# vpc-ccg/circminer

Hardware: AMD Instinct MI355X
Metric: paired reads/sec (whole node), hg38 k=20, 2x150 bp; circ_report bit-exact (higher is better)
Workload: dtype int32/u8 (chain scores f64)

## Files before the change

circminer_amd/_build.py:

```python
from __future__ import annotations

import os
import subprocess
import sys

HERE = os.path.dirname(os.path.abspath(__file__))
CSRC = os.path.join(HERE, "csrc")
INC = os.path.join(HERE, "..", "include")
OUT = os.path.join(CSRC, "libcmhot.so")
SOURCES = ["cm_hot.hip", "cm_dispatch.cpp", "host_index.cpp", "host_annot.cpp", "host_index_io.cpp", "host_fastq.cpp", "host_mapping.cpp", "host_circ.cpp",
           "host_circ_call.cpp"]
DEPS = SOURCES + sorted(f for f in os.listdir(CSRC) if f.endswith(".h")) + [os.path.join("..", "..", "include", "circminer_hot.h")]
KERNEL_EXPORTS = ['cm_create', 'cm_destroy', 'cm_last_error', 'cm_load_contig', 'cm_load_contig_raw', 'cm_build_contig', 'cm_index_download', 'cm_load_annotation', 'cm_unload_contig', 'cm_reads_upload', 'cm_reads_stage', 'cm_reads_swap', 'cm_map_rounds', 'cm_map_round', 'cm_sync', 'cm_reads_reset', 'cm_collect_active', 'cm_collect_records', 'cm_collect_records_device', 'cm_host_alloc', 'cm_host_free', 'cm_host_register', 'cm_host_unregister', 'cm_type_histogram', 'cm_reads_download', 'cm_map_batch', 'cm_seed_batch', 'cm_chain_batch', 'cm_debug_lane_clk', 'cm_debug_counters', 'cm_prof_enable', 'cm_prof_reset', 'cm_prof_get', 'cm_prof_counters', 'cm_ctx', 'cm_chain']
VARIANTS = (("k16", []), ("k24", ["-DCM_MAX_CHAIN_FRAGS=24"]))


def needs_build(out: str = OUT) -> bool:
    if not os.path.exists(out):
        return True
    t = os.path.getmtime(out)
    return any(os.path.getmtime(os.path.join(CSRC, d)) > t for d in DEPS)


def build(force: bool = False, verbose: bool = False, tag: str = "", flags=()) -> str:
    OUT = os.path.join(CSRC, f"libcmhot_{tag}.so") if tag else globals()["OUT"]
    if not force and not needs_build(OUT):
        return OUT
    hipcc = os.environ.get("HIPCC", "/opt/rocm/bin/hipcc")
    extra = os.environ.get("CM_EXTRA_FLAGS", "").split() + list(flags)
    sfx = ("_" + tag) if tag else ""
    objs = []
    jobs = []
    for s in SOURCES:
        base = [hipcc, "-c", "-O3", "-std=c++17", "-fPIC", "-ffp-contract=off", *extra, "-I", INC, "-I", CSRC]
        if s.endswith(".hip"):
            arch = ["--offload-arch=gfx950", "-Rpass-analysis=kernel-resource-usage"] if verbose else ["--offload-arch=gfx950"]
            for vtag, vflags in VARIANTS:
                o = os.path.join(CSRC, s.rsplit(".", 1)[0] + "_" + vtag + sfx + ".o")
                ren = [f"-D{n}={n}_{vtag}" for n in KERNEL_EXPORTS + ["cmc"]]
                jobs.append((s + " [" + vtag + "]", [base[0]] + arch + base[1:] + vflags + ren + [os.path.join(CSRC, s), "-o", o]))
                objs.append(o)
        else:
            o = os.path.join(CSRC, s.rsplit(".", 1)[0] + sfx + ".o")
            jobs.append((s, [base[0], "-x", "c++"] + base[1:] + [os.path.join(CSRC, s), "-o", o]))
            objs.append(o)
    procs = [(name, subprocess.Popen(cmd, stdout=subprocess.PIPE, stderr=subprocess.STDOUT, text=True)) for name, cmd in jobs]
    failed = []
    for name, pr in procs:
        out, _ = pr.communicate()
        if verbose or pr.returncode != 0:
            sys.stderr.write(out)
        if pr.returncode != 0:
            failed.append(name)
    if failed:
        raise RuntimeError(f"hipcc failed on {failed}")
    r = subprocess.run([hipcc, "--offload-arch=gfx950", "-shared", "-fPIC", "-o", OUT] + objs + ["-lpthread", "-lz"],
                       capture_output=True, text=True)
    if r.returncode != 0:
        sys.stderr.write(r.stdout + r.stderr)
        raise RuntimeError("link failed")
    return OUT


if __name__ == "__main__":
    print(build(force="--force" in sys.argv, verbose="-v" in sys.argv))
```

circminer_amd/csrc/cm_dispatch.cpp:

```cpp
#include <cstdlib>

#include "circminer_hot.h"

struct cm_ctx {
    int wide;
    void *inner;
};

#define CM_VARIANTS(ret, name, params) extern "C" ret name##_k16 params; extern "C" ret name##_k24 params;
CM_VARIANTS(int, cm_create, (const cm_params *, void **))
CM_VARIANTS(void, cm_destroy, (void *))
CM_VARIANTS(const char *, cm_last_error, (const void *))
CM_VARIANTS(int, cm_load_contig, (void *, int, const cm_index_view *))
CM_VARIANTS(int, cm_load_annotation, (void *, int, const cm_annot_view *))
CM_VARIANTS(int, cm_unload_contig, (void *, int))
CM_VARIANTS(int, cm_reads_upload, (void *, const cm_reads *, const cm_mapped_read *))
CM_VARIANTS(int, cm_reads_stage, (void *, const cm_reads *, const cm_mapped_read *))
CM_VARIANTS(int, cm_reads_swap, (void *))
CM_VARIANTS(int, cm_map_rounds, (void *, const int *, int, int))
CM_VARIANTS(int, cm_map_round, (void *, int, int))
CM_VARIANTS(int, cm_sync, (void *))
CM_VARIANTS(int, cm_reads_reset, (void *))
CM_VARIANTS(int, cm_collect_active, (void *, uint64_t, uint64_t *, cm_mapped_read *, uint64_t *))
CM_VARIANTS(int, cm_collect_records, (void *, uint64_t, uint64_t, cm_record *, uint64_t *))
CM_VARIANTS(int, cm_collect_records_device, (void *, uint64_t, uint64_t, void *, uint64_t *))
CM_VARIANTS(int, cm_host_alloc, (void *, uint64_t, void **))
CM_VARIANTS(int, cm_host_free, (void *, void *))
CM_VARIANTS(int, cm_load_contig_raw, (void *, int, const cm_index_raw *))
CM_VARIANTS(int, cm_build_contig, (void *, int, int32_t, const uint8_t *, uint32_t, cm_build_stats *))
CM_VARIANTS(int, cm_index_download, (void *, int, uint32_t *, uint16_t *, uint32_t *, uint64_t, uint64_t *))
CM_VARIANTS(int, cm_host_register, (void *, void *, uint64_t))
CM_VARIANTS(int, cm_host_unregister, (void *, void *))
CM_VARIANTS(int, cm_type_histogram, (void *, uint64_t *))
CM_VARIANTS(int, cm_reads_download, (void *, cm_mapped_read *, int32_t *, uint8_t *))
CM_VARIANTS(int, cm_map_batch, (void *, int, int, const cm_reads *, const cm_mapped_read *, cm_mapped_read *, int32_t *))
CM_VARIANTS(int, cm_seed_batch, (void *, int, uint32_t *, uint32_t *, uint32_t *, uint32_t, uint32_t *))
CM_VARIANTS(int, cm_chain_batch, (void *, int, void *, int32_t *, int32_t *))
CM_VARIANTS(int, cm_debug_lane_clk, (void *, unsigned long long *))
CM_VARIANTS(int, cm_debug_counters, (void *, unsigned long long *))
CM_VARIANTS(int, cm_prof_enable, (void *, int))
CM_VARIANTS(int, cm_prof_reset, (void *))
CM_VARIANTS(int, cm_prof_get, (void *, double *, uint64_t *))
CM_VARIANTS(int, cm_prof_counters, (void *, uint64_t *))

#define GO(name, ...) (ctx->wide ? name##_k24(ctx->inner, ##__VA_ARGS__) : name##_k16(ctx->inner, ##__VA_ARGS__))

extern "C" {

int cm_create(const cm_params *p, cm_ctx **out) {
    if (!p || !out) return CM_EINVAL;
    *out = nullptr;
    if (p->kmer < CM_WINDOW_SIZE) return CM_EINVAL;
    const int seeds = p->max_read_len / p->kmer;
    cm_ctx *c = new cm_ctx{seeds > 16 ? 1 : 0, nullptr};
    const int rc = c->wide ? cm_create_k24(p, &c->inner) : cm_create_k16(p, &c->inner);
    if (rc != CM_OK) {
        delete c;
        return rc;
    }
    *out = c;
    return CM_OK;
}
void cm_destroy(cm_ctx *ctx) {
    if (!ctx) return;
    if (ctx->wide) cm_destroy_k24(ctx->inner);
    else cm_destroy_k16(ctx->inner);
    delete ctx;
}
const char *cm_last_error(const cm_ctx *ctx) { return !ctx ? "null context" : (ctx->wide ? cm_last_error_k24(ctx->inner) : cm_last_error_k16(ctx->inner)); }
int cm_load_contig(cm_ctx *ctx, int slot, const cm_index_view *iv) { return ctx ? GO(cm_load_contig, slot, iv) : CM_EINVAL; }
int cm_load_annotation(cm_ctx *ctx, int slot, const cm_annot_view *av) { return ctx ? GO(cm_load_annotation, slot, av) : CM_EINVAL; }
int cm_unload_contig(cm_ctx *ctx, int slot) { return ctx ? GO(cm_unload_contig, slot) : CM_EINVAL; }
int cm_reads_upload(cm_ctx *ctx, const cm_reads *r, const cm_mapped_read *prior) { return ctx ? GO(cm_reads_upload, r, prior) : CM_EINVAL; }
int cm_reads_stage(cm_ctx *ctx, const cm_reads *r, const cm_mapped_read *prior) { return ctx ? GO(cm_reads_stage, r, prior) : CM_EINVAL; }
int cm_reads_swap(cm_ctx *ctx) { return ctx ? GO(cm_reads_swap) : CM_EINVAL; }
int cm_map_rounds(cm_ctx *ctx, const int *slots, int n, int last) { return ctx ? GO(cm_map_rounds, slots, n, last) : CM_EINVAL; }
int cm_map_round(cm_ctx *ctx, int slot, int is_last) { return ctx ? GO(cm_map_round, slot, is_last) : CM_EINVAL; }
int cm_sync(cm_ctx *ctx) { return ctx ? GO(cm_sync) : CM_EINVAL; }
int cm_reads_reset(cm_ctx *ctx) { return ctx ? GO(cm_reads_reset) : CM_EINVAL; }
int cm_collect_active(cm_ctx *ctx, uint64_t cap, uint64_t *idx, cm_mapped_read *st, uint64_t *n) { return ctx ? GO(cm_collect_active, cap, idx, st, n) : CM_EINVAL; }
int cm_collect_records(cm_ctx *ctx, uint64_t base, uint64_t cap, cm_record *out, uint64_t *n) { return ctx ? GO(cm_collect_records, base, cap, out, n) : CM_EINVAL; }
int cm_collect_records_device(cm_ctx *ctx, uint64_t base, uint64_t cap, void *d_out, uint64_t *n) {
    return ctx ? GO(cm_collect_records_device, base, cap, d_out, n) : CM_EINVAL;
}
int cm_host_alloc(cm_ctx *ctx, uint64_t bytes, void **out) { return ctx ? GO(cm_host_alloc, bytes, out) : CM_EINVAL; }
int cm_host_free(cm_ctx *ctx, void *p) { return ctx ? GO(cm_host_free, p) : CM_EINVAL; }
int cm_load_contig_raw(cm_ctx *ctx, int slot, const cm_index_raw *raw) { return ctx ? GO(cm_load_contig_raw, slot, raw) : CM_EINVAL; }
int cm_build_contig(cm_ctx *ctx, int slot, int32_t contig_num, const uint8_t *genome, uint32_t ref_len, cm_build_stats *stats) {
    return ctx ? GO(cm_build_contig, slot, contig_num, genome, ref_len, stats) : CM_EINVAL;
}
int cm_index_download(cm_ctx *ctx, int slot, uint32_t *bucket_off, uint16_t *checksum, uint32_t *pos, uint64_t cap, uint64_t *n) {
    return ctx ? GO(cm_index_download, slot, bucket_off, checksum, pos, cap, n) : CM_EINVAL;
}
int cm_host_register(cm_ctx *ctx, void *p, uint64_t bytes) { return ctx ? GO(cm_host_register, p, bytes) : CM_EINVAL; }
int cm_host_unregister(cm_ctx *ctx, void *p) { return ctx ? GO(cm_host_unregister, p) : CM_EINVAL; }
int cm_type_histogram(cm_ctx *ctx, uint64_t out[14]) { return ctx ? GO(cm_type_histogram, out) : CM_EINVAL; }
int cm_reads_download(cm_ctx *ctx, cm_mapped_read *st, int32_t *cat, uint8_t *act) { return ctx ? GO(cm_reads_download, st, cat, act) : CM_EINVAL; }
int cm_map_batch(cm_ctx *ctx, int slot, int is_last, const cm_reads *reads, const cm_mapped_read *prior, cm_mapped_read *st, int32_t *cat) {
    return ctx ? GO(cm_map_batch, slot, is_last, reads, prior, st, cat) : CM_EINVAL;
}
int cm_seed_batch(cm_ctx *ctx, int slot, uint32_t *a, uint32_t *b, uint32_t *c, uint32_t cap, uint32_t *n_slots) {
    return ctx ? GO(cm_seed_batch, slot, a, b, c, cap, n_slots) : CM_EINVAL;
}
int cm_chain_batch(cm_ctx *ctx, int slot, cm_chain *out, int32_t *nchain, int32_t *high) {
    if (!ctx) return CM_EINVAL;
    if (ctx->wide) return CM_ELIMIT;
    return cm_chain_batch_k16(ctx->inner, slot, out, nchain, high);
}
int cm_debug_lane_clk(cm_ctx *ctx, unsigned long long *out) { return ctx ? GO(cm_debug_lane_clk, out) : CM_EINVAL; }
int cm_debug_counters(cm_ctx *ctx, unsigned long long *out) { return ctx ? GO(cm_debug_counters, out) : CM_EINVAL; }
int cm_prof_enable(cm_ctx *ctx, int on) { return ctx ? GO(cm_prof_enable, on) : CM_EINVAL; }
int cm_prof_reset(cm_ctx *ctx) { return ctx ? GO(cm_prof_reset) : CM_EINVAL; }
int cm_prof_get(cm_ctx *ctx, double ms[8], uint64_t launches[8]) { return ctx ? GO(cm_prof_get, ms, launches) : CM_EINVAL; }
int cm_prof_counters(cm_ctx *ctx, uint64_t c[8]) { return ctx ? GO(cm_prof_counters, c) : CM_EINVAL; }

}
```

circminer_amd/csrc/cm_hot.hip:

```cpp
#include <chrono>
#include <hip/hip_runtime.h>
#include <rocprim/device/device_radix_sort.hpp>

#include <algorithm>
#include <atomic>
#include <cstdarg>
#include <cstdio>
#include <cstdlib>
#include <cstring>
#include <string>
#include <functional>
#include <thread>
#include <vector>

#include "circminer_hot.h"
#include "cm_core.h"
#include "cm_aos.h"
#include "cm_index_build.h"

using cmc::Core;
using cmc::KCore;

namespace {

// ... 275 lines not shown
    if (lane_clk) lane_clk[slot] = ((wall_clock64() - it0) & 0xFFFFFFFFull) | ((unsigned long long)t << 32);
#endif
    }
}


__global__ void __launch_bounds__(BLK_PAIR, CM_PAIR_WAVES) k_pair(KCore kc, ReadsDev rd, uint64_t pair0, uint32_t n_tile, const cm_chain *chains, const int32_t *nchain,
                                                   const int32_t *high, cm_mapped_read *state, uint8_t *active, int32_t *cat, int is_last,
                                                   int *err, unsigned long long *counters, int str_cap, unsigned long long *lane_clk,
                                                   const uint32_t *perm, const unsigned int *n_light, unsigned int *next_chunk,
                                                   RetryArgs ra) {
    pair_kernel<true>(kc, rd, pair0, n_tile, chains, nchain, high, state, active, cat, is_last, err, counters, str_cap, lane_clk, perm, n_light, next_chunk, ra);
}
__global__ void __launch_bounds__(BLK_PAIR, CM_PAIR_WAVES) k_pair_rerun(KCore kc, ReadsDev rd, uint64_t pair0, uint32_t n_tile, const cm_chain *chains,
                                                         const int32_t *nchain, const int32_t *high, cm_mapped_read *state, uint8_t *active, int32_t *cat,
                                                         int is_last, int *err, unsigned long long *counters, int str_cap,
                                                         unsigned long long *lane_clk, const uint32_t *perm, const unsigned int *n_light,
                                                         unsigned int *next_chunk, RetryArgs ra) {
    pair_kernel<false>(kc, rd, pair0, n_tile, chains, nchain, high, state, active, cat, is_last, err, counters, str_cap, lane_clk, perm, n_light, next_chunk, ra);
}

template <class T> __device__ inline T wave_excl_scan(T v, int lane, T &total) {
    T x = v;
    for (int o = 1; o < 64; o <<= 1) {
        const T y = __shfl_up(x, o);
        if (lane >= o) x += y;
    }
    total = __shfl(x, 63);
    return x - v;
}
struct HeavyChainCtx {
#if defined(CM_CHAIN_DIAG)
    unsigned long long *tk;
#endif
    const Core *c;
    CM_L const uint32_t *LP;
    CM_L const uint32_t *NB;
    const uint32_t *base, *cnt;
    int kc, seq_len;
    CM_G double *dps;
    CM_G int32_t *dpp;
};
__device__ inline uint32_t heavy_cell(const HeavyChainCtx &h, int ii, uint32_t i, CM_G cmc::Event *ev, double &out_score, int32_t &out_prev,
                                     double &e0, double &e1) {
    const Core &c = *h.c;
    const int kmer = c.P.kmer;
    const uint32_t read_remain = (uint32_t)(h.seq_len - ii * kmer - kmer);
    const int32_t cur_info = (int32_t)h.LP[h.base[ii] + i];
    const uint32_t seg_start = (uint32_t)cur_info, seg_end = (uint32_t)cur_info + kmer - 1;
    uint32_t max_lpos_lim = cmc::MAXUB, max_exon_end = 0;
    int ol = -1;
    double my_score = (double)kmer;
    int32_t my_prev = -1;
    uint32_t n = 0;
    const uint32_t cell = h.base[ii] + i;
    const bool near = (h.NB[cell >> 5] >> (cell & 31)) & 1u;
    uint2 parked = make_uint2(0u, 0u);
    int parked_ol = -1;
    if (near) {
        parked = *(CM_G const uint2 *)(h.dps + cell);
        parked_ol = h.dpp[cell];
    }
#if defined(CM_CHAIN_DIAG)
    if (!ev) h.tk[3] += 1;
#define CD_T0 const unsigned long long cd_t = wall_clock64()
#define CD_ADD(k) h.tk[k] += wall_clock64() - cd_t
#else
#define CD_T0
#define CD_ADD(k)
#endif
    for (int jj = ii + 1; jj < h.kc; ++jj) {
        const uint32_t pcn = h.cnt[jj];
        if (pcn == 0) continue;
        CM_L const uint32_t *pp = h.LP + h.base[jj];
        uint32_t lo = 0, hi = pcn;
        {
            CD_T0;
            while (lo < hi) {
                const uint32_t mid = (lo + hi) >> 1;
                if ((int32_t)pp[mid] <= cur_info) lo = mid + 1;
                else hi = mid;
            }
            CD_ADD(0);
        }
        if (lo >= pcn) continue;
        if (cur_info + c.P.max_intron < (int32_t)pp[lo]) continue;
        if (max_lpos_lim == cmc::MAXUB) {
            CD_T0;
            if (near) {
                max_lpos_lim = parked.x;
                max_exon_end = parked.y;
                ol = parked_ol;
            } else {
                max_exon_end = 0;
                ol = -1;
                max_lpos_lim = seg_start + read_remain + (uint32_t)c.P.max_ed;
            }
            CD_ADD(1);
        }
        const int distr = (jj - ii) * kmer - kmer;
        CD_T0;
        for (uint32_t j = lo; j < pcn && pp[j] <= max_lpos_lim; ++j) {
#if defined(CM_CHAIN_DIAG)
            if (!ev) h.tk[4] += 1;
#endif
            const uint32_t pinfo = pp[j];
            int genome_dist, distt, trans_dist;
            if (max_exon_end == 0 || (pinfo + kmer - 1) <= max_exon_end) genome_dist = (int)(pinfo - seg_end - 1);
            else genome_dist = cmc::INF_I;
            if (cmc::cabs(genome_dist - distr) <= c.P.max_ed) distt = genome_dist;
            else if (cmc::check_junction(c, seg_start, pinfo, ol, kmer, distr, trans_dist)) distt = trans_dist;
            else continue;
            const int maxd = distr < distt ? distt : distr, mind = distr < distt ? distr : distt;
            const double beta = 0.1 * (double)(maxd - mind);
            const double alpha = 2e4 * (double)kmer;
            const double t1 = h.dps[h.base[jj] + j] + alpha;
            const double temp_score = t1 - beta;
            if (temp_score > my_score) {
                my_score = temp_score;
                my_prev = (int32_t)(((uint32_t)jj << 16) | j);
                if (ev) {
                    ev[n].score = temp_score;
                    ev[n].cell = ((uint32_t)ii << 16) | i;
                }
                if (n == 0) e0 = temp_score;
                else if (n == 1) e1 = temp_score;
                ++n;
            }
        }
        CD_ADD(2);
    }
    out_score = my_score;
    out_prev = my_prev;
    return n;
}

struct HeavyBackTrack {
    uint32_t base[cmc::MAX_SEEDS + 1];
    uint32_t cand[CM_BESTCHAINLIM + 2];
    uint16_t cidx[CM_BESTCHAINLIM][CM_MAX_CHAIN_FRAGS];
    uint8_t cbl[CM_BESTCHAINLIM][CM_MAX_CHAIN_FRAGS];
    uint8_t clen[CM_BESTCHAINLIM + 2];
    uint8_t emit[CM_BESTCHAINLIM + 2];
    uint32_t rep[CM_BESTCHAINLIM * (CM_MAX_CHAIN_FRAGS - 1)];
};

#ifndef CM_CHEAVY_WAVES
#define CM_CHEAVY_WAVES 3
#endif
__global__ void __launch_bounds__(64, CM_CHEAVY_WAVES) k_chain_heavy(KCore kc_, ReadsDev rd, uint64_t pair0, int S, const uint32_t *sstart, const uint32_t *scnt,
                                                    const unsigned long long *celloff, double *dp_score, int32_t *dp_prev, uint8_t *pool,
                                                    unsigned long long pool_bytes, unsigned long long *pool_cursor, cm_chain *chains, int32_t *nchain,
                                                    int *err, uint16_t *resid, const uint32_t *perm, const unsigned int *n_perm, unsigned int *next_problem,
                                                    unsigned long long *counters) {
    extern __shared__ uint32_t lds_words[];
    CM_L uint32_t *LP = (CM_L uint32_t *)lds_words;
    __shared__ HeavyBackTrack BT;
    const int lane = threadIdx.x;
    const Core c = cmc::to_core(kc_);
    const int kmer = c.P.kmer;
    const uint32_t max_best = (uint32_t)c.P.max_chain_len;
    const unsigned int n_heavy = *n_perm;
    auto take = [&]() { return (unsigned int)__shfl((int)(lane == 0 ? atomicAdd(next_problem, 1u) : 0u), 0); };
    for (unsigned int hidx = take(); hidx < n_heavy; hidx = take()) {
        const uint32_t r = perm[hidx];
        const uint64_t p = pair0 + (r >> 2);
        const int mate = (int)((r >> 1) & 1u);
        const int len = (int)(mate ? rd.off2[p + 1] - rd.off2[p] : rd.off1[p + 1] - rd.off1[p]);
#if defined(CM_CHAIN_DIAG)
        const unsigned long long dg0 = wall_clock64();
#endif
        uint32_t st[cmc::MAX_SEEDS], cn[cmc::MAX_SEEDS], base[cmc::MAX_SEEDS + 1];
        int kc = S;
        for (int s = 0; s < S; ++s) {
            st[s] = sstart[(uint64_t)r * S + s];
            cn[s] = scnt[(uint64_t)r * S + s];
        }
        while (kc >= 1 && cn[kc - 1] == 0) --kc;
        base[0] = 0;
        for (int s = 0; s < kc; ++s) base[s + 1] = base[s] + cn[s];
        const uint32_t ncell = base[kc];
        CM_G double *dps = (CM_G double *)(dp_score + celloff[r]);
        CM_G int32_t *dpp = (CM_G int32_t *)(dp_prev + celloff[r]);
        for (int s = 0; s < kc; ++s)
            for (uint32_t i = lane; i < cn[s]; i += 64) LP[base[s] + i] = c.X.pos[st[s] + i];
        for (uint32_t x = lane; x < ncell; x += 64) {
            dps[x] = (double)kmer;
            dpp[x] = -1;
        }
        __threadfence_block();
        __syncthreads();
        CM_L uint32_t *NB = LP + ncell;
        CM_L uint16_t *Q = (CM_L uint16_t *)(NB + 2 * ((ncell + 63) >> 6));
        {
            const uint32_t n_pre = kc >= 1 ? base[kc - 1] : 0u;
            const unsigned long long lt = (1ull << lane) - 1ull;
            uint32_t qn = 0;
            auto look_up = [&](uint32_t cnt) {
                if ((uint32_t)lane < cnt) {
                    const uint32_t x = Q[lane];
                    int ii = 0;
                    for (int s = 1; s < kc; ++s) ii += x >= base[s] ? 1 : 0;
                    const uint32_t read_remain = (uint32_t)(len - ii * kmer - kmer);
                    uint32_t mx = 0;
                    int ol = -1;
                    const uint32_t lim = cmc::upper_bound_lookup(c, LP[x], (uint32_t)kmer, read_remain, mx, ol);
                    *(CM_G uint2 *)(dps + x) = make_uint2(lim, mx);
                    dpp[x] = ol;
                }
            };
            for (uint32_t x0 = 0; x0 < n_pre; x0 += 256) {
                bool nr[4];
#pragma unroll
                for (int u = 0; u < 4; ++u) {
                    const uint32_t x = x0 + 64 * u + lane;
                    nr[u] = x < n_pre && cmc::bit_at(c.A.near_border_bits, c.A.n_bits, LP[x]);
                }
#pragma unroll
                for (int u = 0; u < 4; ++u) {
                    const uint32_t xb = x0 + 64 * u;
                    if (xb >= n_pre) break;
                    const unsigned long long m = __ballot(nr[u]);
                    if (lane == 0) NB[xb >> 5] = (uint32_t)m;
                    if (lane == 32) NB[(xb >> 5) + 1] = (uint32_t)(m >> 32);
                    if (nr[u]) Q[qn + __popcll(m & lt)] = (uint16_t)(xb + lane);
                    qn += (uint32_t)__popcll(m);
                }
                __syncthreads();
                while (qn >= 64) {
                    look_up(64);
                    uint16_t keep[4];
#pragma unroll
                    for (int u = 0; u < 4; ++u) keep[u] = 64u * u + (uint32_t)lane < qn - 64 ? Q[64 + 64 * u + lane] : (uint16_t)0;
                    __syncthreads();
#pragma unroll
                    for (int u = 0; u < 4; ++u)
                        if (64u * u + (uint32_t)lane < qn - 64) Q[64 * u + lane] = keep[u];
                    qn -= 64;
                    __syncthreads();
                }
            }
            if (qn) look_up(qn);
        }
        __threadfence_block();
        __syncthreads();
#if defined(CM_CHAIN_DIAG)
        const unsigned long long dg1 = wall_clock64();
#endif
#if defined(CM_CHAIN_DIAG)
        unsigned long long tk[5] = {0, 0, 0, 0, 0};
        unsigned long long wv[4] = {0, 0, 0, 0};
        HeavyChainCtx H{tk, &c, LP, NB, base, cn, kc, len, dps, dpp};
#else
        HeavyChainCtx H{&c, LP, NB, base, cn, kc, len, dps, dpp};
#endif
        CM_G cmc::Event *ev = nullptr;
        uint32_t n_ev = 0, cap_ev = 0;
        bool lost = false;
        for (int ii = kc - 2; ii >= 0; --ii) {
            for (uint32_t i0 = 0; i0 < cn[ii]; i0 += 64) {
                const uint32_t i = i0 + lane;
                const bool on = i < cn[ii];
                double sc = 0, e0 = 0, e1 = 0;
                int32_t pv = -1;
#if defined(CM_CHAIN_DIAG)
                const unsigned long long w0 = wall_clock64();
#endif
                const uint32_t mine = on ? heavy_cell(H, ii, i, (CM_G cmc::Event *)nullptr, sc, pv, e0, e1) : 0u;
#if defined(CM_CHAIN_DIAG)
                const unsigned long long w1 = wall_clock64();
#endif
                uint32_t total;
                const uint32_t off = wave_excl_scan(mine, lane, total);
                if (n_ev + total > cap_ev && !lost) {
                    uint32_t ncap = cap_ev ? cap_ev : 256u;
                    while (ncap < n_ev + total) ncap *= 4u;
                    const unsigned long long bytes = (unsigned long long)ncap * sizeof(cmc::Event);
                    unsigned long long o = 0;
                    if (lane == 0) o = atomicAdd(pool_cursor, bytes);
                    o = ((unsigned long long)__shfl((unsigned int)(o >> 32), 0) << 32) | (unsigned long long)__shfl((unsigned int)o, 0);
                    if (o + bytes > pool_bytes) {
                        lost = true;
                        if (lane == 0) atomicOr(err, cmc::ERR_POOL);
                    } else {
                        CM_G cmc::Event *ne = (CM_G cmc::Event *)((CM_G uint8_t *)pool + o);
                        for (uint32_t q = lane; q < n_ev; q += 64) ne[q] = ev[q];
                        ev = ne;
                        cap_ev = ncap;
                    }
                }
                if (on) {
                    if (mine && !lost) {
                        CM_G cmc::Event *dst = ev + n_ev + off;
                        if (mine <= 2) {
                            dst[0].score = e0;
                            dst[0].cell = ((uint32_t)ii << 16) | i;
                            if (mine == 2) {
                                dst[1].score = e1;
                                dst[1].cell = ((uint32_t)ii << 16) | i;
                            }
                        } else heavy_cell(H, ii, i, dst, sc, pv, e0, e1);
                    }
                    dps[base[ii] + i] = sc;
                    dpp[base[ii] + i] = pv;
                }
                if (!lost) n_ev += total;
#if defined(CM_CHAIN_DIAG)
                const unsigned long long w3 = wall_clock64();
                wv[0] += w1 - w0;
                wv[2] += w3 - w1;
#endif
            }
#if defined(CM_CHAIN_DIAG)
            const unsigned long long w4 = wall_clock64();
#endif
            __threadfence_block();
            __syncthreads();
#if defined(CM_CHAIN_DIAG)
            wv[3] += wall_clock64() - w4;
#endif
        }
#if defined(CM_CHAIN_DIAG)
        for (int k = 0; k < 5; ++k) atomicAdd(&counters[8 + k], tk[k]);
        if (lane == 0)
            for (int k = 0; k < 4; ++k) atomicAdd(&counters[16 + k], wv[k]);
#endif
        CM_G cm_chain *out = (CM_G cm_chain *)(chains + (uint64_t)r * CM_BESTCHAINLIM);
        uint32_t best_count = 0;
        int first_q0 = 0, first_qlast = 0;
        if (lane <= kc) BT.base[lane] = base[lane];
        __threadfence_block();
        __syncthreads();
#if defined(CM_CHAIN_DIAG)
        const unsigned long long dg2 = wall_clock64();
#endif
        if (n_ev > 0) {
            double best_score = -1.0;
            for (uint32_t q = lane; q < n_ev; q += 64) best_score = ev[q].score > best_score ? ev[q].score : best_score;
            for (int o = 32; o >= 1; o >>= 1) {
                const double u = __shfl_xor(best_score, o);
                best_score = u > best_score ? u : best_score;
            }
            double cur = best_score;
            bool have = true;
            uint32_t n_rep = 0;
#if defined(CM_CHAIN_DIAG)
            unsigned long long dg_levels = 0;
#endif
            while (have && best_count < max_best) {
#if defined(CM_CHAIN_DIAG)
                ++dg_levels;
#endif
                uint32_t n_c = 0;
                double nxt = -1.0;
                bool hv = false;
                for (uint32_t q0 = 0; q0 < n_ev; q0 += 64) {
                    const uint32_t q = q0 + lane;
                    const double v = q < n_ev ? ev[q].score : 0.0;
                    const bool hit = q < n_ev && v == cur;
                    if (q < n_ev && v < cur && (!hv || v > nxt)) {
                        nxt = v;
                        hv = true;
                    }
                    const unsigned long long m = __ballot(hit);
                    if (m && n_c < max_best) {
                        const uint32_t rank = n_c + (uint32_t)__popcll(m & ((1ull << lane) - 1ull));
                        if (hit && rank < max_best) BT.cand[rank] = ev[q].cell;
                        n_c += (uint32_t)__popcll(m);
                        if (n_c > max_best) n_c = max_best;
// ... 591 lines not shown
                        if (cmc::fold_task(c, r1, r2, res[y - b0].is_left != 0, res[y - b0].ok != 0, res[y - b0].row, res[y - b0].pair_type, r1_fwd, mr)) {
                            early = true;
                            S[lane].done = 1;
                            break;
                        }
                        min_ret1 = r1.type < min_ret1 ? r1.type : min_ret1;
                        min_ret2 = r2.type < min_ret2 ? r2.type : min_ret2;
                        g1 = (r1.exons_spos >= 0) || (r1.exons_epos >= 0);
                        g2 = (r2.exons_spos >= 0) || (r2.exons_epos >= 0);
                    }
                }
                __syncthreads();
                CM_TICK(sm, 31);
            }
            int a = -1;
            bool do_f = false, do_b = false;
            if (on) {
                CM_L HSlot &s = S[lane];
                if (early) a = CM_CONCRD;
                else if (mr.type == CM_CONCRD || mr.type == CM_DISCRD || mr.type == CM_CHIORF || mr.type == CM_CHIBSJ || mr.type == CM_CHI2BSJ) a = mr.type;
                else {
                    const uint32_t fun = ~s.fp & (s.nf >= 32 ? 0xffffffffu : ((1u << s.nf) - 1u));
                    const uint32_t bun = ~s.bp & (s.nb >= 32 ? 0xffffffffu : ((1u << s.nb) - 1u));
                    do_f = min_ret1 != CM_CONCRD && fun != 0;
                    do_b = min_ret2 != CM_CONCRD && bun != 0;
                    if (!cmc::leftovers_matter(mr.type, min_ret1, do_f, min_ret2, do_b)) a = mr.type;
                    else {
                        s.fun = fun;
                        s.bun = bun;
                        s.nfu = (int16_t)(do_f ? __popc(fun) : 0);
                        s.nbu = (int16_t)(do_b ? __popc(bun) : 0);
                        s.exf = 99;
                        s.exb = 99;
                        s.gf = 0;
                        s.gb = 0;
                    }
                }
            }
            __syncthreads();
            pre[0] = 0;
#pragma unroll
            for (int g = 0; g < HG; ++g) pre[g + 1] = pre[g] + S[g].nfu + S[g].nbu;
            for (int x = lane; x < pre[HG]; x += 64) {
                int g, u;
                locate(pre, x, g, u);
                CM_L HSlot &s = S[g];
                const bool back = u >= s.nfu;
                const int k = back ? u - s.nfu : u;
                const int ci = nth_set_bit(back ? s.bun : s.fun, k);
                const cmc::CH ch{(back ? slot_bch(s, chains) : slot_fch(s, chains)) + ci, kmer};
                const cmc::Read frd{s.fseq, s.flen, 0}, brd{s.bseq, s.blen, 1};
                cmc::MM m = cmc::mm_init(c);
                sm.err = slot_perr(s, ra.pair_err);
                const int ex = ext.chain_both_sides(ch, back ? brd : frd, m, back ? -1 : 1);
                atomicMin((int *)(back ? &s.exb : &s.exf), ex);
                if (k == 0) {
                    cmc::overlap_to_spos(c, m);
                    cmc::overlap_to_epos(c, m);
                    (back ? s.gb : s.gf) = (int8_t)((m.exons_spos >= 0) || (m.exons_epos >= 0));
                }
            }
            __syncthreads();
            CM_TICK(sm, 15);
            if (on) {
                if (a < 0) {
                    CM_L HSlot &s = S[lane];
                    if (do_f) {
                        min_ret1 = s.exf < min_ret1 ? s.exf : min_ret1;
                        g1 = s.gf;
                    }
                    if (do_b) {
                        min_ret2 = s.exb < min_ret2 ? s.exb : min_ret2;
                        g2 = s.gb;
                    }
                    cmc::mr_update_type(mr, cmc::leftover_type(min_ret1, min_ret2, g1 != 0, g2 != 0));
                    a = mr.type;
                }
                if (c.P.scan_level == 0 && a == CM_CONCRD) st = CM_CONCRD;
            }
            __syncthreads();
        }
        __threadfence_block();
        if (owner) {
            if (st < 0) st = mr.type;
            if (__hip_atomic_load(ra.pair_err + t, __ATOMIC_RELAXED, __HIP_MEMORY_SCOPE_AGENT) != 0u) {
                ra.list[atomicAdd(ra.count, 1u)] = t;
                active[p] = 1;
            } else {
                uint8_t act = 1;
                cmc::finish_round(c, st, is_last, len1, len2, mr, act);
                state[p] = mr;
                active[p] = act;
                cat[p] = st;
                atomicAdd(&counters[3], 1ull);
            }
        }
        __syncthreads();
        CM_TICK(sm, 13);
    }
#if defined(CM_DIAG)
    if (dbg_rows && lane == 0)
        for (int i = 0; i < 64; ++i) dbg_rows[(size_t)blockIdx.x * 64 + i] = tick_w[1 + i];
#endif
}

#include "cm_heavy_pipe.h"

__global__ void __launch_bounds__(BLK) k_active_cls(const uint8_t *active, uint64_t n, int8_t *cls) {
    const uint64_t i = (uint64_t)blockIdx.x * BLK + threadIdx.x;
    if (i < n) cls[i] = active[i] ? 0 : -2;
}
__global__ void __launch_bounds__(BLK) k_gather_active(const uint32_t *perm, const unsigned int *count, unsigned long long cap, const cm_mapped_read *state,
                                                       unsigned long long *out_idx, cm_mapped_read *out_state) {
    const uint64_t i = (uint64_t)blockIdx.x * BLK + threadIdx.x;
    if (i >= *count || i >= cap) return;
    const uint32_t p = perm[i];
    out_idx[i] = p;
    out_state[i] = state[p];
}

__global__ void __launch_bounds__(BLK) k_gather_records(const uint32_t *perm, const unsigned int *count, unsigned long long cap, const cm_mapped_read *state,
                                                        unsigned long long index_base, cm_record *out) {
    const uint64_t i = (uint64_t)blockIdx.x * BLK + threadIdx.x;
    if (i >= *count || i >= cap) return;
    const uint32_t p = perm[i];
    out[i].pair = index_base + p;
    out[i].state = state[p];
}

__global__ void __launch_bounds__(BLK) k_type_hist(const cm_mapped_read *state, uint64_t n, unsigned long long *hist) {
    __shared__ unsigned int h[16];
    if (threadIdx.x < 16) h[threadIdx.x] = 0;
    __syncthreads();
    for (uint64_t i = (uint64_t)blockIdx.x * BLK + threadIdx.x; i < n; i += (uint64_t)gridDim.x * BLK) {
        const int t = state[i].type;
        if (t >= 0 && t < 14) atomicAdd(&h[t], 1u);
    }
    __syncthreads();
    if (threadIdx.x < 14 && h[threadIdx.x]) atomicAdd(&hist[threadIdx.x], (unsigned long long)h[threadIdx.x]);
}
__global__ void k_err_clear(int *err, int mask) {
    if (threadIdx.x == 0 && blockIdx.x == 0) atomicAnd(err, ~mask);
}
__global__ void __launch_bounds__(BLK) k_build_desc(const uint32_t *bucket_off, const uint16_t *checksum, uint64_t n_buckets, int kmer, uint32_t *desc) {
    const uint64_t hv = (uint64_t)blockIdx.x * BLK + threadIdx.x;
    if (hv >= n_buckets) return;
    const uint32_t b0 = bucket_off[hv], n = bucket_off[hv + 1] - b0;
    uint32_t out[cmc::DESC_WORDS];
    cmc::desc_pack(b0, n, [&](uint32_t i) { return (uint32_t)checksum[b0 + i]; }, kmer, out);
    uint4 v;
    v.x = out[0]; v.y = out[1]; v.z = out[2]; v.w = out[3];
    ((uint4 *)desc)[hv] = v;
}
constexpr int S32_T = 1024, S32_E = 8, S32_B = S32_T * S32_E;
__global__ void __launch_bounds__(S32_T) k_scan32_a(const uint32_t *in, uint64_t n, uint32_t *out, uint32_t *bsum, uint32_t add, int inclusive) {
    __shared__ uint32_t wsum[S32_T / 64];
    const uint64_t base = (uint64_t)blockIdx.x * S32_B + (uint64_t)threadIdx.x * S32_E;
    uint32_t v[S32_E], run = 0;
#pragma unroll
    for (int k = 0; k < S32_E; ++k) {
        const uint64_t i = base + k;
        v[k] = i < n ? in[i] + add : 0u;
        run += v[k];
    }
    const int lane = threadIdx.x & 63, wave = threadIdx.x >> 6;
    uint32_t incl = run;
    for (int o = 1; o < 64; o <<= 1) {
        const uint32_t y = __shfl_up(incl, o);
        if (lane >= o) incl += y;
    }
    if (lane == 63) wsum[wave] = incl;
    __syncthreads();
    uint32_t wbase = 0;
    for (int w = 0; w < wave; ++w) wbase += wsum[w];
    uint32_t pre = wbase + incl - run;
#pragma unroll
    for (int k = 0; k < S32_E; ++k) {
        const uint64_t i = base + k;
        if (i < n) out[i] = inclusive ? pre + v[k] : pre;
        pre += v[k];
    }
    if (threadIdx.x == S32_T - 1) bsum[blockIdx.x] = pre;
}
__global__ void __launch_bounds__(1024) k_scan32_b(uint32_t *bsum, uint32_t nb) {
    __shared__ uint32_t part[1024];
    const uint32_t t = threadIdx.x, chunk = (nb + 1023u) / 1024u;
    const uint32_t a = t * chunk, b = (a + chunk < nb) ? a + chunk : nb;
    uint32_t sum = 0;
    for (uint32_t i = a; i < b; ++i) sum += bsum[i];
    part[t] = sum;
    __syncthreads();
    for (uint32_t d = 1; d < 1024; d <<= 1) {
        const uint32_t v = (t >= d) ? part[t - d] : 0u;
        __syncthreads();
        part[t] += v;
        __syncthreads();
    }
    uint32_t run = t ? part[t - 1] : 0u;
    for (uint32_t i = a; i < b; ++i) {
        const uint32_t x = bsum[i];
        bsum[i] = run;
        run += x;
    }
}
__global__ void __launch_bounds__(S32_T) k_scan32_c(uint32_t *out, uint64_t n, const uint32_t *bsum) {
    const uint32_t add = bsum[blockIdx.x];
    const uint64_t base = (uint64_t)blockIdx.x * S32_B + (uint64_t)threadIdx.x * S32_E;
    if (add)
#pragma unroll
        for (int k = 0; k < S32_E; ++k)
            if (base + k < n) out[base + k] += add;
}
struct RawEntry { uint16_t checksum, pad; int32_t info; };
__global__ void __launch_bounds__(BLK) k_raw_counts(const RawEntry *tab, const uint32_t *start, const uint32_t *hv, const uint32_t *cnt14, uint32_t n_b,
                                                   uint64_t n_buckets_all, uint32_t *counts, int *bad) {
    const uint32_t i = blockIdx.x * BLK + threadIdx.x;
    if (i >= n_b) return;
    const int32_t c = tab[start[i]].info;
    if (c < 0 || (uint32_t)c > cnt14[i] || (uint64_t)hv[i] >= n_buckets_all || (i && hv[i] <= hv[i - 1])) {
        atomicOr(bad, 1);
        return;
    }
    counts[hv[i] + 1] = (uint32_t)c;
}
__global__ void __launch_bounds__(BLK) k_raw_scatter(const RawEntry *tab, const uint32_t *start, const uint32_t *hv, uint32_t n_b, const uint32_t *bucket_off,
                                                    uint16_t *checksum, uint32_t *pos) {
    const uint32_t i = blockIdx.x * BLK + threadIdx.x;
    if (i >= n_b) return;
    const uint32_t h = hv[i], w = bucket_off[h], c = bucket_off[h + 1] - w;
    const RawEntry *e = tab + start[i] + 1;
    for (uint32_t k = 0; k < c; ++k) {
        const RawEntry x = e[k];
        checksum[w + k] = x.checksum;
        pos[w + k] = (uint32_t)x.info;
    }
}

constexpr int IB_PER = 8, IB_TILE = BLK * IB_PER;
constexpr int IB_HALO = CM_WINDOW_SIZE + 8 - 1;
static_assert(cmc::CM_STAGE_PAD >= 4, "k_ib_positions reads whole words up to 3 bytes past the contig");
template <bool SCATTER>
__global__ void __launch_bounds__(BLK) k_ib_positions(const uint8_t *genome, uint32_t ref_len, uint32_t n_pos, int k, int c, uint32_t *cursor,
                                                      uint16_t *checksum, uint32_t *pos) {
    __shared__ uint8_t codes[IB_TILE + IB_HALO + 3];
    const uint64_t t0 = (uint64_t)blockIdx.x * IB_TILE;
    if (t0 >= n_pos) return;
    const uint32_t tile_pos = (uint32_t)(n_pos - t0 < (uint64_t)IB_TILE ? n_pos - t0 : (uint64_t)IB_TILE);
    const uint32_t n_codes = tile_pos + (uint32_t)k - 1;
    const uint32_t *gw = (const uint32_t *)(genome + t0);
    for (uint32_t w = threadIdx.x; w * 4 < n_codes; w += BLK) {
        const uint32_t x = gw[w];
#pragma unroll
        for (int b = 0; b < 4; ++b) codes[w * 4 + b] = (uint8_t)cmib::base_code((uint8_t)(x >> (8 * b)));
    }
    __syncthreads();
    const uint32_t first = threadIdx.x * IB_PER;
    if (first >= tile_pos) return;
    const uint32_t mine = tile_pos - first < (uint32_t)IB_PER ? tile_pos - first : (uint32_t)IB_PER;
    cmib::scan_positions(codes + first, n_codes - first, mine, k, c, [&](uint32_t j, uint32_t hv, uint32_t ck) {
        if (SCATTER) {
            const uint32_t at = atomicSub(&cursor[hv], 1u) - 1u;
            checksum[at] = (uint16_t)ck;
            pos[at] = (uint32_t)(t0 + first + j) + 1u;
        } else {
            atomicAdd(&cursor[hv], 1u);
        }
    });
}
enum { IB_ST_PATH = 0, IB_ST_MAX = 3, IB_ST_NMED = 4, IB_ST_NOVER = 5, IB_ST_WORDS = 6 };
__global__ void __launch_bounds__(BLK) k_ib_order_lane(const uint32_t *bucket_off, uint64_t n_buckets, uint16_t *checksum, uint32_t *pos, uint32_t lane_max,
                                                       uint32_t wg_max, uint32_t *med_list, uint32_t *over_list, unsigned long long *st) {
    __shared__ unsigned int cnt[4];
    if (threadIdx.x < 4) cnt[threadIdx.x] = 0;
    __syncthreads();
    const uint64_t hv = (uint64_t)blockIdx.x * BLK + threadIdx.x;
    if (hv < n_buckets) {
        const uint32_t b0 = bucket_off[hv], n = bucket_off[hv + 1] - b0;
        const int path = cmib::bucket_path(n, lane_max, wg_max);
        if (path >= 0) {
            atomicAdd(&cnt[path], 1u);
            atomicMax(&cnt[3], n);
            if (path == 0) cmib::lane_sort(checksum + b0, pos + b0, n);
            else if (path == 1) med_list[atomicAdd(&st[IB_ST_NMED], 1ull)] = (uint32_t)hv;
            else over_list[atomicAdd(&st[IB_ST_NOVER], 1ull)] = (uint32_t)hv;
        }
    }
    __syncthreads();
    if (threadIdx.x < 3 && cnt[threadIdx.x]) atomicAdd(&st[IB_ST_PATH + threadIdx.x], (unsigned long long)cnt[threadIdx.x]);
    if (threadIdx.x == 3 && cnt[3]) atomicMax(&st[IB_ST_MAX], (unsigned long long)cnt[3]);
}
constexpr uint32_t IB_WG_CAP = cmib::WG_MAX;
__global__ void __launch_bounds__(BLK) k_ib_order_wg(const uint32_t *bucket_off, const uint32_t *list, uint32_t n_list, uint16_t *checksum, uint32_t *pos) {
    __shared__ uint64_t keys[IB_WG_CAP];
    for (uint32_t b = blockIdx.x; b < n_list; b += gridDim.x) {
        const uint32_t hv = list[b], b0 = bucket_off[hv], n = bucket_off[hv + 1] - b0;
        if (n > IB_WG_CAP) continue;
        const uint32_t np2 = cmib::pow2_at_least(n);
        for (uint32_t i = threadIdx.x; i < np2; i += BLK) keys[i] = i < n ? cmib::pack_key(checksum[b0 + i], pos[b0 + i]) : ~0ull;
        __syncthreads();
        for (uint32_t size = 2; size <= np2; size <<= 1)
            for (uint32_t stride = size >> 1; stride > 0; stride >>= 1) {
                for (uint32_t i = threadIdx.x; i < np2; i += BLK) cmib::bitonic_step(keys, i, size, stride);
                __syncthreads();
            }
        for (uint32_t i = threadIdx.x; i < n; i += BLK) {
            checksum[b0 + i] = cmib::key_checksum(keys[i]);
            pos[b0 + i] = cmib::key_pos(keys[i]);
        }
        __syncthreads();
    }
}
__global__ void __launch_bounds__(BLK) k_ib_over_sizes(const uint32_t *bucket_off, const uint32_t *list, uint32_t n_list, uint32_t *sizes) {
    const uint32_t i = blockIdx.x * BLK + threadIdx.x;
    if (i < n_list) sizes[i] = bucket_off[list[i] + 1] - bucket_off[list[i]];
}
__global__ void __launch_bounds__(BLK) k_ib_over_pack(const uint32_t *bucket_off, const uint32_t *list, const uint32_t *start, uint32_t r0, uint32_t r1,
                                                      const uint16_t *checksum, const uint32_t *pos, uint64_t *keys) {
    const uint32_t base = start[r0];
    for (uint32_t r = r0 + blockIdx.x; r < r1; r += gridDim.x) {
        const uint32_t b0 = bucket_off[list[r]], n = start[r + 1] - start[r], at = start[r] - base;
        for (uint32_t i = threadIdx.x; i < n; i += BLK) keys[at + i] = cmib::over_key(r - r0, checksum[b0 + i], pos[b0 + i]);
    }
}
__global__ void __launch_bounds__(BLK) k_ib_over_unpack(const uint32_t *bucket_off, const uint32_t *list, const uint32_t *start, uint32_t r0, uint32_t r1,
                                                        const uint64_t *keys, uint16_t *checksum, uint32_t *pos) {
    const uint32_t base = start[r0];
    for (uint32_t r = r0 + blockIdx.x; r < r1; r += gridDim.x) {
        const uint32_t b0 = bucket_off[list[r]], n = start[r + 1] - start[r], at = start[r] - base;
        for (uint32_t i = threadIdx.x; i < n; i += BLK) {
            const uint64_t x = keys[at + i];
            checksum[b0 + i] = cmib::key_checksum(x);
            pos[b0 + i] = cmib::key_pos(x);
        }
    }
}

__global__ void k_init_state(KCore kc, cm_mapped_read *state, uint8_t *active, int32_t *cat, uint64_t n) {
    const uint64_t i = (uint64_t)blockIdx.x * BLK + threadIdx.x;
    if (i >= n) return;
    Core c;
    c.P = kc.P;
    cmc::default_mr(c, state[i]);
    active[i] = 1;
    cat[i] = -1;
}

struct Slot {
    bool loaded = false, has_annot = false;
    uint64_t gen = 0;
    uint32_t *d_desc = nullptr;
    bool chain_parallel_ok = false;
    cm_index_view X{};
    cmc::AnnotDev A{};
    std::vector<void *> idx_allocs, ann_allocs;
};

struct ProfRec { hipEvent_t a, b; int cls; };

enum Life { BATCH = 0, CONTEXT = 1 };
struct DevMem {
    void *p = nullptr;
    size_t cap = 0;
    std::vector<DevMem *> *listed = nullptr;
    DevMem() = default;
    DevMem(const DevMem &) = delete;
    DevMem &operator=(const DevMem &) = delete;
};
inline void swap(DevMem &a, DevMem &b) {
    std::swap(a.p, b.p);
    std::swap(a.cap, b.cap);
    if (!a.listed && b.listed) (a.listed = b.listed)->push_back(&a);
    if (!b.listed && a.listed) (b.listed = a.listed)->push_back(&b);
}
template <class T, Life L>
struct DevBuf : DevMem {
    operator T *() const { return (T *)p; }
};
template <class T> using BatchBuf = DevBuf<T, BATCH>;
template <class T> using CtxBuf = DevBuf<T, CONTEXT>;

struct ReadBufs {
    BatchBuf<uint8_t> seq1_base, seq2_base;
    BatchBuf<uint64_t> off1, off2;
};
inline void swap(ReadBufs &a, ReadBufs &b) {
    swap(a.seq1_base, b.seq1_base);
    swap(a.seq2_base, b.seq2_base);
    swap(a.off1, b.off1);
    swap(a.off2, b.off2);
}

struct SeedSet {
    BatchBuf<uint32_t> sstart, scnt, sraw;
    BatchBuf<unsigned long long> celloff, bsum;
    BatchBuf<unsigned int> bmax;
    BatchBuf<int8_t> cls4;
    BatchBuf<unsigned int> cblk, cctr;
    BatchBuf<uint32_t> perm4;
    BatchBuf<int32_t> thigh;
    bool cls_deferred = false;
};
struct ChainRecs {
    BatchBuf<cm_chain> chains;
    BatchBuf<int32_t> nchain, high;
    BatchBuf<uint16_t> resid;
};
struct PairSet {
    uint32_t *perm = nullptr, *hlist = nullptr;
    unsigned int *cls_ctr = nullptr;
    uint32_t *pair_err = nullptr, *retry_list = nullptr;
    unsigned int *retry_ctr = nullptr;
    uint32_t *hp_fall = nullptr;
    unsigned int *hp_fallctr = nullptr;
};
struct PairSetMem {
    BatchBuf<uint32_t> perm, hlist;
    BatchBuf<unsigned int> cls_ctr;
    BatchBuf<uint32_t> pair_err, retry_list;
    BatchBuf<unsigned int> retry_ctr;
    BatchBuf<uint32_t> hp_fall;
    BatchBuf<unsigned int> hp_fallctr;
};
struct PairSort {
    BatchBuf<int8_t> cls, sub, sub2;
    BatchBuf<uint32_t> perm1, perm0;
    BatchBuf<unsigned int> ctr2, ctr3, blk_cnt;
};
struct HeavyPipe {
    BatchBuf<HPair> pairs;
    BatchBuf<uint32_t> list2, q, q2;
    BatchBuf<HTask> T;
    BatchBuf<int8_t> tcls;
    BatchBuf<uint32_t> tperm;
    BatchBuf<unsigned int> tblk, tctr;
    BatchBuf<HUnp> U;
    BatchBuf<cmc::PreDP> pre, pre2;
    BatchBuf<HRes> res;
    BatchBuf<uint16_t> lists;
    BatchBuf<unsigned int> ctr;
    uint32_t tasks_cap = 0, unp_cap = 0;
};
struct ChainWork {
    BatchBuf<double> score;
    BatchBuf<int32_t> prev;
    unsigned long long cells_cap = 0;
    BatchBuf<uint8_t> pool;
    unsigned long long pool_bytes = 0;
};
struct Collect {
    BatchBuf<int8_t> cls;
    BatchBuf<uint32_t> perm;
    BatchBuf<unsigned int> blk, ctr;
    CtxBuf<unsigned long long> idx;
    CtxBuf<cm_mapped_read> st;
    CtxBuf<cm_record> rec;
};

struct Streams {
    hipStream_t B = nullptr;
    hipStream_t B2 = nullptr;
    hipStream_t C = nullptr;
    hipStream_t P = nullptr, P2 = nullptr;
    hipStream_t R = nullptr;
    hipStream_t O = nullptr;
    hipStream_t S = nullptr;
};
enum StreamKind { BLOCKING, NON_BLOCKING, NON_BLOCKING_LOWEST };
struct StreamDef {
    hipStream_t Streams::*st;
    const char *name;
    StreamKind kind;
};
constexpr StreamDef STREAMS[] = {
    {&Streams::B, "main", BLOCKING},           {&Streams::B2, "heavy chains", BLOCKING},     {&Streams::C, "copy", NON_BLOCKING},
    {&Streams::P, "pairs", NON_BLOCKING_LOWEST}, {&Streams::P2, "heavy pairs", NON_BLOCKING}, {&Streams::R, "re-run", NON_BLOCKING},
    {&Streams::O, "pair ordering", NON_BLOCKING}, {&Streams::S, "seeding", NON_BLOCKING},
};
struct Events {
    hipEvent_t fork = nullptr, join = nullptr;
    hipEvent_t join_p = nullptr, tail = nullptr;
    hipEvent_t flags = nullptr;
    hipEvent_t staged = nullptr, retired = nullptr;
    hipEvent_t order[2] = {nullptr, nullptr};
    hipEvent_t seed[2] = {nullptr, nullptr};
    hipEvent_t first[2] = {nullptr, nullptr};
    hipEvent_t prep[2] = {nullptr, nullptr}, pair[2] = {nullptr, nullptr};
    hipEvent_t *begin() { return &fork; }
    hipEvent_t *end() { return begin() + sizeof(Events) / sizeof(hipEvent_t); }
};
static_assert(sizeof(Events) == 17 * sizeof(hipEvent_t), "Events holds events only");

}

struct cm_ctx {
    cm_params P{};
    unsigned id = 0;
    int teardown_errors = 0;
    Streams st;
    Events ev;
    std::vector<DevMem *> bufs[2];
    struct Rerun {
        bool deferred = false;
        cmc::KCore core;
// ... 99 lines not shown
    for (void *p : v) report_hip(ctx, "hipFree", hipFree(p));
    v.clear();
}
void dfree(cm_ctx *c, DevMem &m) {
    if (m.p) report_hip(c, "hipFree", hipFree(m.p));
    m.p = nullptr;
    m.cap = 0;
}
template <class T, Life L>
hipError_t ensure(cm_ctx *c, DevBuf<T, L> &m, size_t bytes) {
    if (m.p && m.cap >= bytes) return hipSuccess;
    dfree(c, m);
    const hipError_t e = hipMalloc(&m.p, bytes ? bytes : 1);
    if (e != hipSuccess) return e;
    m.cap = bytes;
    if (!m.listed) (m.listed = &c->bufs[L])->push_back(&m);
    return e;
}
void release(cm_ctx *c, Life l) {
    for (DevMem *m : c->bufs[l]) {
        dfree(c, *m);
        m->listed = nullptr;
    }
    c->bufs[l].clear();
}

void free_reads(cm_ctx *c) {
    if (c->st.C) report_hip(c, "hipStreamSynchronize(copy stream)", hipStreamSynchronize(c->st.C));
    release(c, BATCH);
    c->pset[0] = c->pset[1] = PairSet{};
    c->ones_cap = 0;
    c->pre_launched = c->pre_ready = false;
    c->staged = false;
    c->st_n_pairs = 0;
    c->n_pairs = 0;
    c->tile = 0;
}

static hipEvent_t take_event(cm_ctx *c) {
    hipEvent_t e = nullptr;
    if (!c->ev_free.empty()) {
        e = c->ev_free.back();
        c->ev_free.pop_back();
    } else (void)hipEventCreate(&e);
    return e;
}
struct Timer {
    cm_ctx *c;
    int cls;
    ProfRec r{};
    bool on;
    hipStream_t st;
    Timer(cm_ctx *ctx, int k, hipStream_t stream = nullptr) : c(ctx), cls(k), on(ctx->prof), st(stream ? stream : ctx->st.B) {
        if (on) {
            r.a = take_event(c);
            r.b = take_event(c);
            r.cls = cls;
            (void)hipEventRecord(r.a, st);
        }
    }
    ~Timer() {
        if (on) {
            (void)hipEventRecord(r.b, st);
            c->recs.push_back(r);
        }
    }
};

KCore make_core(const cm_ctx *c, const Slot &s) {
    KCore k;
    k.P = c->P;
    k.X = s.X;
    k.A = s.A;
    k.desc = s.d_desc;
    return k;
}

int check_slot(cm_ctx *ctx, int slot, bool need_annot) {
    if (slot < 0 || slot >= MAX_SLOTS) return fail(ctx, CM_EINVAL, "slot %d out of range", slot);
    if (!ctx->slots[slot].loaded) return fail(ctx, CM_ESTATE, "contig slot %d not loaded", slot);
    if (need_annot && !ctx->slots[slot].has_annot) return fail(ctx, CM_ESTATE, "annotation of slot %d not loaded", slot);
    return CM_OK;
}

ReadsDev reads_dev(const ReadBufs &r) { return ReadsDev{r.seq1_base + cmc::CM_STAGE_PAD, r.seq2_base + cmc::CM_STAGE_PAD, r.off1, r.off2}; }
ReadsDev current_reads(const cm_ctx *ctx) { return reads_dev(ctx->rd); }

constexpr unsigned HP_PLAN_GRID = 2048;
static bool heavy_pipeline() {
    static const bool v = !(getenv("CM_HEAVY_PIPELINE") && getenv("CM_HEAVY_PIPELINE")[0] == '0');
    return v;
}
static unsigned long long chain_light_w() {
    static const unsigned long long v = getenv("CM_CHAIN_LIGHT_W") ? strtoull(getenv("CM_CHAIN_LIGHT_W"), nullptr, 10) : 256ull;
    return v;
}
static unsigned int chain_light_cells() {
    static const unsigned int v = getenv("CM_CHAIN_LIGHT_CELLS") ? (unsigned)atoi(getenv("CM_CHAIN_LIGHT_CELLS")) : 96u;
    return v;
}

static int seed_classes(cm_ctx *ctx, uint64_t pair0, uint32_t n_tile, const uint8_t *act, int s, hipStream_t st, const ChainRecs *rb, bool defer = false) {
    const int S = ctx->n_seeds;
    const uint32_t n_prob = n_tile * 4u;
    if ((uint64_t)n_prob * (uint64_t)S == 0) return CM_OK;
    const SeedSet &sb = ctx->seed[s];
    Timer t(ctx, 5, st);
    const uint32_t nbk = (n_prob + CLS_T - 1) / CLS_T;
    hipLaunchKernelGGL(k_chain_cls, dim3((n_prob + BLK - 1) / BLK), dim3(BLK), 0, st, sb.scnt, sb.sraw, S, n_prob, sb.cls4, defer ? sb.thigh : rb->high,
                       chain_light_w(), chain_light_cells(), defer ? (int32_t *)nullptr : rb->nchain, defer ? (uint16_t *)nullptr : rb->resid, act, pair0);
    ctx->seed[s].cls_deferred = defer;
    hipLaunchKernelGGL(k_cls_hist, dim3(nbk), dim3(CLS_W), 0, st, sb.cls4, n_prob, sb.cblk, nbk, (const uint32_t *)nullptr,
                       (const unsigned int *)nullptr);
    hipLaunchKernelGGL(k_cls_scan, dim3(1), dim3(SCAN_CLS_T), 0, st, sb.cblk, nbk, sb.cctr, -1, N_CLS);
    hipLaunchKernelGGL(k_cls_place, dim3(nbk), dim3(CLS_W), 0, st, sb.cls4, n_prob, sb.cblk, nbk, sb.cctr, sb.perm4,
                       (uint32_t *)nullptr, (const uint32_t *)nullptr, (const unsigned int *)nullptr);
    ctx->launches[5] += 4;
    HIPCHK(ctx, hipMemsetAsync(ctx->pool_cursor(s), 0, sizeof(unsigned long long), st));
    HIPCHK(ctx, hipMemsetAsync(sb.cctr + 48, 0, sizeof(unsigned int), st));
    HIPCHK(ctx, hipGetLastError());
    return CM_OK;
}
int run_seed_tile(cm_ctx *ctx, const KCore &core, const ReadsDev &rd, uint64_t pair0, uint32_t n_tile, const uint8_t *act, int s, hipStream_t st,
                  const ChainRecs *rb, bool defer_rb = false) {
    const int S = ctx->n_seeds;
    const uint64_t total = (uint64_t)n_tile * 4u * (uint64_t)S;
    if (total == 0) return CM_OK;
    const SeedSet &sb = ctx->seed[s];
    {
        Timer t(ctx, 0, st);
        hipLaunchKernelGGL(k_seed, dim3((unsigned)((total + BLK - 1) / BLK)), dim3(BLK), 0, st, core, rd, act, pair0, n_tile, S,
                           sb.sstart, sb.scnt, sb.sraw, ctx->d_counters);
        ++ctx->launches[0];
    }
    const uint32_t n_prob = n_tile * 4u;
    {
        Timer t(ctx, 3, st);
        const uint32_t nb = (n_prob + SCAN_ELEMS - 1) / SCAN_ELEMS;
        hipLaunchKernelGGL(k_scan_a, dim3(nb), dim3(SCAN_T), 0, st, sb.scnt, S, n_prob, sb.celloff, sb.bsum, sb.bmax);
        hipLaunchKernelGGL(k_scan_b, dim3(1), dim3(1024), 0, st, sb.bsum, nb, sb.celloff + n_prob, (const unsigned int *)sb.bmax);
        hipLaunchKernelGGL(k_scan_c, dim3((n_prob + SCAN_T - 1) / SCAN_T), dim3(SCAN_T), 0, st, sb.celloff, sb.bsum, n_prob);
        ctx->launches[3] += 3;
    }
    HIPCHK(ctx, hipMemcpyAsync(ctx->h_pin + 8 + 2 * s, sb.celloff + n_prob, 2 * sizeof(unsigned long long), hipMemcpyDeviceToHost, st));
    if (rb) {
        const int rc = seed_classes(ctx, pair0, n_tile, act, s, st, rb, defer_rb);
        if (rc) return rc;
    }
    HIPCHK(ctx, hipEventRecord(ctx->ev.seed[s], st));
    HIPCHK(ctx, hipGetLastError());
    return CM_OK;
}

int run_chain_tile(cm_ctx *ctx, const KCore &core, const ReadsDev &rd, uint64_t pair0, uint32_t n_tile, bool parallel_ok, const uint8_t *act,
                   const ChainRecs &rb, int s, const std::function<int()> &after_launch = {}) {
    const int S = ctx->n_seeds;
    const uint32_t n_prob = n_tile * 4u;
    if (n_prob == 0 || S == 0) return after_launch ? after_launch() : CM_OK;
    const SeedSet &sb = ctx->seed[s];
    HIPCHK(ctx, hipStreamWaitEvent(ctx->st.B, ctx->ev.seed[s], 0));
    HIPCHK(ctx, hipEventSynchronize(ctx->ev.seed[s]));
    if (ctx->seed[s].cls_deferred) {
        hipLaunchKernelGGL(k_chain_apply, dim3((n_prob + BLK - 1) / BLK), dim3(BLK), 0, ctx->st.B, n_prob, (const int8_t *)sb.cls4, (const int32_t *)sb.thigh,
                           rb.high, rb.nchain, rb.resid);
        ctx->seed[s].cls_deferred = false;
    }
    const unsigned long long total = ctx->h_pin[8 + 2 * s];
    const unsigned long long max_cells = ctx->h_pin[9 + 2 * s];
    std::vector<std::pair<uint32_t, uint32_t>> ranges;
    if (total <= ctx->dp.cells_cap) {
        ranges.push_back({0u, n_prob});
    } else {
        ctx->h_celloff.resize((size_t)n_prob + 1);
        HIPCHK(ctx, hipMemcpyAsync(ctx->h_celloff.data(), sb.celloff, ((size_t)n_prob + 1) * sizeof(unsigned long long), hipMemcpyDeviceToHost,
                                   ctx->st.B));
        HIPCHK(ctx, hipStreamSynchronize(ctx->st.B));
        uint32_t a = 0;
        while (a < n_prob) {
            uint32_t b = a;
            while (b < n_prob && ctx->h_celloff[b + 1] - ctx->h_celloff[a] <= ctx->dp.cells_cap) ++b;
            if (b == a) return fail(ctx, CM_ELIMIT, "one chaining problem needs %llu DP cells (> workspace %llu)",
                                    ctx->h_celloff[a + 1] - ctx->h_celloff[a], ctx->dp.cells_cap);
            ranges.push_back({a, b});
            a = b;
        }
    }
    const size_t lds_extra = ((size_t)max_cells / 64 + 2) * 8 + 640;
    const size_t heavy_lds = std::min<size_t>((size_t)S * (size_t)ctx->P.seed_lim * sizeof(uint32_t),
                                              ((size_t)max_cells * sizeof(uint32_t) + 2047) / 2048 * 2048 + 2048) + (lds_extra + 255) / 256 * 256;
    const bool split = ranges.size() == 1 && parallel_ok && heavy_lds <= 152u * 1024u;
    bool fresh = true;
    auto launch_group = [&](uint32_t a, uint32_t b, unsigned long long base, bool use_split) -> int {
        const uint32_t n = b - a;
        if (!fresh) {
            HIPCHK(ctx, hipMemsetAsync(ctx->pool_cursor(s), 0, sizeof(unsigned long long), ctx->st.B));
            HIPCHK(ctx, hipMemsetAsync(sb.cctr + 48, 0, sizeof(unsigned int), ctx->st.B));
        }
        fresh = false;
        if (use_split) {
            HIPCHK(ctx, hipEventRecord(ctx->ev.fork, ctx->st.B));
            HIPCHK(ctx, hipStreamWaitEvent(ctx->st.B2, ctx->ev.fork, 0));
            {
            Timer t(ctx, 6, ctx->st.B2);
            static std::atomic<size_t> heavy_attr{64u * 1024u};
            if (heavy_lds > heavy_attr.load()) {
                HIPCHK(ctx, hipFuncSetAttribute((const void *)k_chain_heavy, hipFuncAttributeMaxDynamicSharedMemorySize, (int)heavy_lds));
                heavy_attr.store(heavy_lds);
            }
            const uint32_t hb = n < 8192u ? n : 8192u;
            hipLaunchKernelGGL(k_chain_heavy, dim3(hb), dim3(64), heavy_lds, ctx->st.B2, core, rd, pair0, S, sb.sstart, sb.scnt, sb.celloff,
                               ctx->dp.score, ctx->dp.prev, ctx->dp.pool, ctx->dp.pool_bytes, ctx->pool_cursor(s), rb.chains, rb.nchain, ctx->d_err,
                               rb.resid, sb.perm4, sb.cctr + CTR_BASE + CHAIN_LIGHT_CLS - 1, sb.cctr + 48, ctx->d_counters);
            ++ctx->launches[6];
            }
            HIPCHK(ctx, hipEventRecord(ctx->ev.join, ctx->st.B2));
        }
        Timer t(ctx, 1);
        hipLaunchKernelGGL(k_chain, dim3((n + BLK_CHAIN - 1) / BLK_CHAIN), dim3(BLK_CHAIN), 0, ctx->st.B, core, rd, act, pair0, a, b, S,
                           sb.sstart, sb.scnt, sb.sraw, sb.celloff, base, ctx->dp.score, ctx->dp.prev, ctx->dp.pool,
                           ctx->dp.pool_bytes, ctx->pool_cursor(s), rb.chains, rb.nchain, rb.high, ctx->d_err, rb.resid,
                           use_split ? sb.perm4 : (const uint32_t *)nullptr, sb.cctr + CTR_BASE + CHAIN_LIGHT_CLS - 1, sb.cctr + CTR_SUM);
        if (use_split) HIPCHK(ctx, hipStreamWaitEvent(ctx->st.B, ctx->ev.join, 0));
        ++ctx->launches[1];
        HIPCHK(ctx, hipGetLastError());
        return CM_OK;
    };
    auto pool_lost = [&](bool *lost) -> int {
        HIPCHK(ctx, hipMemcpyAsync(ctx->h_pin + 2, ctx->d_err, sizeof(int), hipMemcpyDeviceToHost, ctx->st.B));
        HIPCHK(ctx, hipStreamSynchronize(ctx->st.B));
        const int e = *(const int *)(ctx->h_pin + 2);
        *lost = (e & cmc::ERR_POOL) != 0;
        if (*lost) {
            hipLaunchKernelGGL(k_err_clear, dim3(1), dim3(64), 0, ctx->st.B, ctx->d_err, (int)cmc::ERR_POOL);
            HIPCHK(ctx, hipStreamSynchronize(ctx->st.B));
        }
        return CM_OK;
    };
    const unsigned long long pool_max = getenv("CM_POOL_MAX") ? strtoull(getenv("CM_POOL_MAX"), nullptr, 10) : (48ull << 30);
    bool told = false;
    for (auto &rg : ranges) {
        unsigned long long base = 0;
        if (rg.first != 0) base = ctx->h_celloff[rg.first];
        int rc = launch_group(rg.first, rg.second, base, split);
        if (rc) return rc;
        if (!told && after_launch && (rc = after_launch())) return rc;
        told = true;
        bool lost = false;
        if ((rc = pool_lost(&lost))) return rc;
        while (lost && ctx->dp.pool_bytes < pool_max) {
            unsigned long long want = ctx->dp.pool_bytes * 4ull;
            if (want > pool_max) want = pool_max;
            HIPCHK(ctx, hipStreamSynchronize(ctx->st.B2));
            if (ensure(ctx, ctx->dp.pool, want) != hipSuccess) {
                (void)hipGetLastError();
                HIPCHK(ctx, ensure(ctx, ctx->dp.pool, ctx->dp.pool_bytes));
                break;
            }
            ctx->dp.pool_bytes = want;
            if ((rc = launch_group(rg.first, rg.second, base, split))) return rc;
            if ((rc = pool_lost(&lost))) return rc;
        }
        if (lost) {
            std::vector<std::pair<uint32_t, uint32_t>> todo{{rg.first, rg.second}};
            while (!todo.empty()) {
                const auto pc = todo.back();
                todo.pop_back();
                if ((rc = launch_group(pc.first, pc.second, base, false))) return rc;
                if ((rc = pool_lost(&lost))) return rc;
                if (!lost) continue;
                if (pc.second - pc.first <= 1)
                    return fail(ctx, CM_ELIMIT, "one chaining problem's improvement log does not fit %llu bytes", ctx->dp.pool_bytes);
                const uint32_t mid = pc.first + (pc.second - pc.first) / 2;
                todo.push_back({mid, pc.second});
                todo.push_back({pc.first, mid});
            }
        }
    }
    return CM_OK;
}

int check_dev_err(cm_ctx *ctx) {
    HIPCHK(ctx, hipMemcpyAsync(ctx->h_pin, ctx->d_err, sizeof(int), hipMemcpyDeviceToHost, ctx->st.B));
    HIPCHK(ctx, hipStreamSynchronize(ctx->st.B));
    const int e = *(const int *)ctx->h_pin;
    if (e) {
        (void)hipMemsetAsync(ctx->d_err, 0, sizeof(int), ctx->st.B);
        return fail(ctx, CM_ELIMIT, "device capacity limit hit:%s%s%s", (e & cmc::ERR_POOL) ? " chain improvement-log pool exhausted;" : "",
                    (e & (cmc::ERR_SEEDS | cmc::ERR_BAND)) ? " DP string longer than the staging buffer;" : "",
                    (e & cmc::ERR_MEMO) ? " extension memo overflowed where the reference's memo would have served a colliding key" : "");
    }
    return CM_OK;
}

}

extern "C" {

int cm_create(const cm_params *p, cm_ctx **out) {
    if (!p || !out) return CM_EINVAL;
    *out = nullptr;
    const int c = p->kmer - CM_WINDOW_SIZE;
    if (p->kmer < CM_WINDOW_SIZE || c > 8) return CM_EINVAL;
    if (p->max_chain_len < 1 || p->max_chain_len > CM_BESTCHAINLIM) return CM_EINVAL;
    if (p->band < 0 || p->band > cmc::MAX_BAND) return CM_EINVAL;
    if (p->seed_lim < 1 || p->seed_lim > 65535) return CM_EINVAL;
    if (p->max_ed < 0 || p->max_sc < 0 || p->max_read_len < p->kmer) return CM_EINVAL;
    const char *hwq = getenv("GPU_MAX_HW_QUEUES");
    const bool hwq_low = !hwq || atoi(hwq) < 16;
    setenv("GPU_MAX_HW_QUEUES", "16", 0);
    int ndev = 0;
    if (hipGetDeviceCount(&ndev) != hipSuccess || ndev <= 0) return CM_ENODEV;
    if (p->device < 0 || p->device >= ndev) return CM_ENODEV;
    if (hipSetDevice(p->device) != hipSuccess) return CM_ENODEV;
    cm_ctx *ctx = new cm_ctx();
    ctx->P = *p;
    {
        static std::atomic<unsigned> serial{0};
        ctx->id = ++serial;
    }
    int prio_lo = 0, prio_hi = 0;
    (void)hipDeviceGetStreamPriorityRange(&prio_lo, &prio_hi);
    for (const StreamDef &d : STREAMS) {
        hipStream_t *st = &(ctx->st.*d.st);
        if ((d.kind == BLOCKING              ? hipStreamCreate(st)
             : d.kind == NON_BLOCKING_LOWEST ? hipStreamCreateWithPriority(st, hipStreamNonBlocking, prio_lo)
                                             : hipStreamCreateWithFlags(st, hipStreamNonBlocking)) != hipSuccess) {
            cm_destroy(ctx);
            return CM_EHIP;
        }
    }
    for (hipEvent_t &e : ctx->ev)
        if (hipEventCreateWithFlags(&e, hipEventDisableTiming) != hipSuccess) {
            cm_destroy(ctx);
            return CM_EHIP;
        }
    if (ensure(ctx, ctx->d_pool_cursor, 2 * sizeof(unsigned long long)) != hipSuccess ||
        ensure(ctx, ctx->d_err, sizeof(int)) != hipSuccess ||
        ensure(ctx, ctx->d_counters, 32 * sizeof(unsigned long long)) != hipSuccess ||
        hipHostMalloc((void **)&ctx->h_pin, 128, hipHostMallocDefault) != hipSuccess) {
        cm_destroy(ctx);
        return CM_ENOMEM;
    }
    memset(ctx->h_pin, 0, 128);
    (void)hipMemsetAsync(ctx->d_err, 0, sizeof(int), ctx->st.B);
    (void)hipMemsetAsync(ctx->d_counters, 0, 32 * sizeof(unsigned long long), ctx->st.B);
    if (hwq_low) {
        ctx->err = "note: GPU_MAX_HW_QUEUES was " + std::string(hwq ? hwq : "unset") +
                   " when this context was created; if HIP was initialised earlier in this process the seven streams of a context share the "
                   "default 4 hardware queues (pipelined rounds run slower). Export GPU_MAX_HW_QUEUES=16 before the first HIP call.";
        static std::atomic<bool> said{false};
        if (hwq && !said.exchange(true) && !getenv("CM_QUIET")) fprintf(stderr, "[cmhot] %s\n", ctx->err.c_str());
    }
    *out = ctx;
    return CM_OK;
}

void cm_destroy(cm_ctx *ctx) {
    if (!ctx) return;
    report_hip(ctx, "hipSetDevice", hipSetDevice(ctx->P.device));
    for (const StreamDef &d : STREAMS)
        if (ctx->st.*d.st) report_hip(ctx, (std::string("hipStreamSynchronize(") + d.name + ")").c_str(), hipStreamSynchronize(ctx->st.*d.st));
    report_hip(ctx, "hipGetLastError at teardown", hipGetLastError());
    for (auto e : ctx->ev_free) report_hip(ctx, "hipEventDestroy", hipEventDestroy(e));
    ctx->ev_free.clear();
    for (auto &r : ctx->recs) {
        report_hip(ctx, "hipEventDestroy", hipEventDestroy(r.a));
        report_hip(ctx, "hipEventDestroy", hipEventDestroy(r.b));
    }
    ctx->recs.clear();
    free_reads(ctx);
    for (auto &s : ctx->slots) {
        free_all(ctx, s.idx_allocs);
        free_all(ctx, s.ann_allocs);
    }
    release(ctx, CONTEXT);
    if (ctx->h_pin) report_hip(ctx, "hipHostFree", hipHostFree(ctx->h_pin));
    for (hipEvent_t e : ctx->ev)
        if (e) report_hip(ctx, "hipEventDestroy", hipEventDestroy(e));
    for (const StreamDef &d : STREAMS)
        if (ctx->st.*d.st) report_hip(ctx, "hipStreamDestroy", hipStreamDestroy(ctx->st.*d.st));
    delete ctx;
}

const char *cm_last_error(const cm_ctx *ctx) { return ctx ? ctx->err.c_str() : "null context"; }

static int finish_contig(cm_ctx *ctx, Slot &s) {
    const size_t nb = ((size_t)1 << (2 * CM_WINDOW_SIZE)) + 1;
    s.d_desc = nullptr;
    static const bool use_desc = !(getenv("CM_SEED_DESC") && getenv("CM_SEED_DESC")[0] == '0');
    if (use_desc) {
        const uint64_t n_buckets = nb - 1;
        uint32_t *d = nullptr;
        if (hipMalloc((void **)&d, n_buckets * cmc::DESC_WORDS * sizeof(uint32_t)) == hipSuccess) {
            s.idx_allocs.push_back(d);
            hipLaunchKernelGGL(k_build_desc, dim3((unsigned)((n_buckets + BLK - 1) / BLK)), dim3(BLK), 0, ctx->st.B, s.X.bucket_off, s.X.checksum, n_buckets,
                               ctx->P.kmer, d);
            HIPCHK(ctx, hipGetLastError());
            s.d_desc = d;
        } else (void)hipGetLastError();
    }
    HIPCHK(ctx, hipStreamSynchronize(ctx->st.B));
    s.loaded = true;
    return CM_OK;
}

int cm_load_contig(cm_ctx *ctx, int slot, const cm_index_view *iv) {
    if (!ctx || !iv) return CM_EINVAL;
    if (slot < 0 || slot >= MAX_SLOTS) return fail(ctx, CM_EINVAL, "slot %d out of range", slot);
    if (!iv->genome || !iv->bucket_off || !iv->checksum || !iv->pos) return fail(ctx, CM_EINVAL, "null index array");
    HIPCHK(ctx, hipSetDevice(ctx->P.device));
    Slot &s = ctx->slots[slot];
    free_all(ctx, s.idx_allocs);
    s.d_desc = nullptr;
    s.loaded = false;
    ++s.gen;
    const size_t nb = ((size_t)1 << (2 * CM_WINDOW_SIZE)) + 1;
    s.X = *iv;
    int rc;
    {
        uint8_t *g = nullptr;
        const size_t pad = cmc::CM_STAGE_PAD;
        HIPCHK(ctx, hipMalloc((void **)&g, (size_t)iv->ref_len + 2 * pad));
        s.idx_allocs.push_back(g);
        HIPCHK(ctx, hipMemsetAsync(g, 0, (size_t)iv->ref_len + 2 * pad, ctx->st.B));
        HIPCHK(ctx, hipMemcpyAsync(g + pad, iv->genome, (size_t)iv->ref_len, hipMemcpyHostToDevice, ctx->st.B));
        s.X.genome = g + pad;
    }
    if ((rc = up(ctx, s.idx_allocs, iv->bucket_off, nb, &s.X.bucket_off))) return rc;
    if ((rc = up(ctx, s.idx_allocs, iv->checksum, (size_t)iv->n_entries, &s.X.checksum))) return rc;
    if ((rc = up(ctx, s.idx_allocs, iv->pos, (size_t)iv->n_entries, &s.X.pos))) return rc;
    return finish_contig(ctx, s);
}

static int scan32(cm_ctx *ctx, const uint32_t *in, uint64_t n, uint32_t *out, uint32_t *tmp, uint32_t add, int inclusive) {
    const uint32_t nb = (uint32_t)((n + S32_B - 1) / S32_B);
    if (nb == 0) return CM_OK;
    hipLaunchKernelGGL(k_scan32_a, dim3(nb), dim3(S32_T), 0, ctx->st.B, in, n, out, tmp, add, inclusive);
    hipLaunchKernelGGL(k_scan32_b, dim3(1), dim3(1024), 0, ctx->st.B, tmp, nb);
    hipLaunchKernelGGL(k_scan32_c, dim3(nb), dim3(S32_T), 0, ctx->st.B, out, n, (const uint32_t *)tmp);
    HIPCHK(ctx, hipGetLastError());
    return CM_OK;
}

int cm_load_contig_raw(cm_ctx *ctx, int slot, const cm_index_raw *raw) {
    if (!ctx || !raw) return CM_EINVAL;
    if (slot < 0 || slot >= MAX_SLOTS) return fail(ctx, CM_EINVAL, "slot %d out of range", slot);
    if (!raw->genome || (raw->n_buckets && (!raw->hv || !raw->count14 || !raw->table))) return fail(ctx, CM_EINVAL, "null array in the raw record");
    if (raw->table_slots > 0xffffffffull) return fail(ctx, CM_ELIMIT, "table of %llu slots", (unsigned long long)raw->table_slots);
    HIPCHK(ctx, hipSetDevice(ctx->P.device));
    Slot &s = ctx->slots[slot];
    free_all(ctx, s.idx_allocs);
    s.d_desc = nullptr;
    s.loaded = false;
    ++s.gen;
    const uint64_t n_all = (uint64_t)1 << (2 * CM_WINDOW_SIZE);
    const uint32_t n_b = raw->n_buckets;
    s.X = cm_index_view{};
    s.X.contig_num = raw->contig_num;
    s.X.ref_len = raw->ref_len;
    int rc;
    {
        uint8_t *g = nullptr;
        const size_t pad = cmc::CM_STAGE_PAD;
        HIPCHK(ctx, hipMalloc((void **)&g, (size_t)raw->ref_len + 2 * pad));
        s.idx_allocs.push_back(g);
        HIPCHK(ctx, hipMemsetAsync(g, 0, (size_t)raw->ref_len + 2 * pad, ctx->st.B));
        HIPCHK(ctx, hipMemcpyAsync(g + pad, raw->genome, (size_t)raw->ref_len, hipMemcpyHostToDevice, ctx->st.B));
        s.X.genome = g + pad;
    }
    std::vector<void *> tmp;
    struct FreeTmp {
        cm_ctx *c;
        std::vector<void *> &v;
        ~FreeTmp() { free_all(c, v); }
    } free_tmp{ctx, tmp};
    const RawEntry *d_tab = nullptr;
    const uint32_t *d_hv = nullptr, *d_cnt = nullptr;
    if ((rc = up(ctx, tmp, (const RawEntry *)raw->table, (size_t)raw->table_slots, &d_tab))) return rc;
    if ((rc = up(ctx, tmp, raw->hv, (size_t)n_b, &d_hv))) return rc;
    if ((rc = up(ctx, tmp, raw->count14, (size_t)n_b, &d_cnt))) return rc;
    uint32_t *d_start = nullptr, *d_bs = nullptr, *d_off = nullptr;
    int *d_bad = nullptr;
    HIPCHK(ctx, hipMalloc((void **)&d_start, ((size_t)n_b + 1) * sizeof(uint32_t)));
    tmp.push_back(d_start);
    HIPCHK(ctx, hipMalloc((void **)&d_bs, ((size_t)(n_all / S32_B) + 4) * sizeof(uint32_t)));
    tmp.push_back(d_bs);
    HIPCHK(ctx, hipMalloc((void **)&d_bad, sizeof(int)));
    tmp.push_back(d_bad);
    HIPCHK(ctx, hipMemsetAsync(d_bad, 0, sizeof(int), ctx->st.B));
    HIPCHK(ctx, hipMalloc((void **)&d_off, (n_all + 1) * sizeof(uint32_t)));
    s.idx_allocs.push_back(d_off);
    HIPCHK(ctx, hipMemsetAsync(d_off, 0, (n_all + 1) * sizeof(uint32_t), ctx->st.B));
    if ((rc = scan32(ctx, d_cnt, n_b, d_start, d_bs, 1u, 0))) return rc;
    if (n_b) {
        hipLaunchKernelGGL(k_raw_counts, dim3((n_b + BLK - 1) / BLK), dim3(BLK), 0, ctx->st.B, d_tab, (const uint32_t *)d_start, d_hv, d_cnt, n_b, n_all, d_off, d_bad);
        HIPCHK(ctx, hipGetLastError());
    }
    if ((rc = scan32(ctx, d_off, n_all + 1, d_off, d_bs, 0u, 1))) return rc;
    unsigned long long landing[2] = {0, 0};
    HIPCHK(ctx, hipMemcpyAsync(&landing[0], d_off + n_all, sizeof(uint32_t), hipMemcpyDeviceToHost, ctx->st.B));
    HIPCHK(ctx, hipMemcpyAsync(&landing[1], d_bad, sizeof(int), hipMemcpyDeviceToHost, ctx->st.B));
    HIPCHK(ctx, hipStreamSynchronize(ctx->st.B));
    if ((int)landing[1]) return fail(ctx, CM_EINVAL, "malformed index table: a bucket header is out of range");
    const uint64_t total = (uint32_t)landing[0];
    uint16_t *d_cs = nullptr;
    uint32_t *d_ps = nullptr;
    HIPCHK(ctx, hipMalloc((void **)&d_cs, (total ? total : 1) * sizeof(uint16_t)));
    s.idx_allocs.push_back(d_cs);
    HIPCHK(ctx, hipMalloc((void **)&d_ps, (total ? total : 1) * sizeof(uint32_t)));
    s.idx_allocs.push_back(d_ps);
    if (n_b) {
        hipLaunchKernelGGL(k_raw_scatter, dim3((n_b + BLK - 1) / BLK), dim3(BLK), 0, ctx->st.B, d_tab, (const uint32_t *)d_start, d_hv, n_b, (const uint32_t *)d_off, d_cs, d_ps);
        HIPCHK(ctx, hipGetLastError());
    }
    s.X.bucket_off = d_off;
    s.X.checksum = d_cs;
    s.X.pos = d_ps;
    s.X.n_entries = total;
    return finish_contig(ctx, s);
}

static int ib_order(cm_ctx *ctx, const uint32_t *d_off, uint16_t *d_cs, uint32_t *d_ps, uint64_t total, uint32_t *d_bs, std::vector<void *> &tmp,
                    unsigned long long st_host[IB_ST_WORDS], size_t *tmp_bytes) {
    const uint64_t n_all = (uint64_t)1 << (2 * CM_WINDOW_SIZE);
    static const uint32_t wg_lim = std::max<uint32_t>(1u, std::min<uint32_t>(getenv("CM_IB_WG_MAX") ? (uint32_t)atoi(getenv("CM_IB_WG_MAX")) : cmib::WG_MAX, IB_WG_CAP));
    static const uint32_t lane_max = std::max<uint32_t>(1u, std::min<uint32_t>(getenv("CM_IB_LANE_MAX") ? (uint32_t)atoi(getenv("CM_IB_LANE_MAX")) : cmib::LANE_MAX, wg_lim));
    unsigned long long *d_st = nullptr;
    uint32_t *d_med = nullptr, *d_over = nullptr;
    const size_t med_cap = (size_t)(total / ((uint64_t)lane_max + 1)) + 1, over_cap = (size_t)(total / ((uint64_t)wg_lim + 1)) + 1;
    HIPCHK(ctx, hipMalloc((void **)&d_st, IB_ST_WORDS * sizeof(unsigned long long)));
    tmp.push_back(d_st);
    HIPCHK(ctx, hipMalloc((void **)&d_med, med_cap * sizeof(uint32_t)));
    tmp.push_back(d_med);
    HIPCHK(ctx, hipMalloc((void **)&d_over, over_cap * sizeof(uint32_t)));
    tmp.push_back(d_over);
    *tmp_bytes += (med_cap + over_cap) * sizeof(uint32_t);
    HIPCHK(ctx, hipMemsetAsync(d_st, 0, IB_ST_WORDS * sizeof(unsigned long long), ctx->st.B));
    hipLaunchKernelGGL(k_ib_order_lane, dim3((unsigned)(n_all / BLK)), dim3(BLK), 0, ctx->st.B, d_off, n_all, d_cs, d_ps, lane_max, wg_lim, d_med, d_over, d_st);
    HIPCHK(ctx, hipGetLastError());
    HIPCHK(ctx, hipMemcpyAsync(st_host, d_st, IB_ST_WORDS * sizeof(unsigned long long), hipMemcpyDeviceToHost, ctx->st.B));
    HIPCHK(ctx, hipStreamSynchronize(ctx->st.B));
    const uint32_t n_med = (uint32_t)st_host[IB_ST_NMED], n_over = (uint32_t)st_host[IB_ST_NOVER];
    if (n_med) {
        hipLaunchKernelGGL(k_ib_order_wg, dim3(std::min<uint32_t>(n_med, 1u << 16)), dim3(BLK), 0, ctx->st.B, d_off, (const uint32_t *)d_med, n_med, d_cs, d_ps);
        HIPCHK(ctx, hipGetLastError());
    }
    if (!n_over) return CM_OK;
    uint32_t *d_start = nullptr;
    HIPCHK(ctx, hipMalloc((void **)&d_start, ((size_t)n_over + 1) * sizeof(uint32_t)));
    tmp.push_back(d_start);
    HIPCHK(ctx, hipMemsetAsync(d_start + n_over, 0, sizeof(uint32_t), ctx->st.B));
    hipLaunchKernelGGL(k_ib_over_sizes, dim3((n_over + BLK - 1) / BLK), dim3(BLK), 0, ctx->st.B, d_off, (const uint32_t *)d_over, n_over, d_start);
    int rc;
    if ((rc = scan32(ctx, d_start, (uint64_t)n_over + 1, d_start, d_bs, 0u, 0))) return rc;
    std::vector<uint32_t> start((size_t)n_over + 1);
    HIPCHK(ctx, hipMemcpyAsync(start.data(), d_start, start.size() * sizeof(uint32_t), hipMemcpyDeviceToHost, ctx->st.B));
    HIPCHK(ctx, hipStreamSynchronize(ctx->st.B));
    auto rank_bits_of = [](uint32_t n_ranks) {
        unsigned b = 1;
        while ((1u << b) < n_ranks) ++b;
        return b;
    };
    uint64_t *d_k0 = nullptr, *d_k1 = nullptr;
    void *d_sort = nullptr;
    uint32_t largest = 0;
    size_t sort_bytes = 0;
    for (uint32_t r0 = 0; r0 < n_over; r0 += cmib::OVER_CHUNK) {
        const uint32_t r1 = std::min(n_over, r0 + cmib::OVER_CHUNK), m = start[r1] - start[r0];
        size_t need = 0;
        HIPCHK(ctx, rocprim::radix_sort_keys(nullptr, need, d_k0, d_k1, (size_t)m, 0u, 48u + rank_bits_of(r1 - r0), ctx->st.B));
        largest = std::max(largest, m);
        sort_bytes = std::max(sort_bytes, need);
    }
    HIPCHK(ctx, hipMalloc((void **)&d_k0, (size_t)largest * sizeof(uint64_t)));
    tmp.push_back(d_k0);
    HIPCHK(ctx, hipMalloc((void **)&d_k1, (size_t)largest * sizeof(uint64_t)));
    tmp.push_back(d_k1);
    HIPCHK(ctx, hipMalloc(&d_sort, sort_bytes ? sort_bytes : 1));
    tmp.push_back(d_sort);
    *tmp_bytes += 2 * (size_t)largest * sizeof(uint64_t) + sort_bytes + ((size_t)n_over + 1) * sizeof(uint32_t);
    for (uint32_t r0 = 0; r0 < n_over; r0 += cmib::OVER_CHUNK) {
        const uint32_t r1 = std::min(n_over, r0 + cmib::OVER_CHUNK), m = start[r1] - start[r0];
        const unsigned rank_bits = rank_bits_of(r1 - r0);
        size_t have = sort_bytes;
        const dim3 grid(std::min<uint32_t>(r1 - r0, 1u << 16));
        hipLaunchKernelGGL(k_ib_over_pack, grid, dim3(BLK), 0, ctx->st.B, d_off, (const uint32_t *)d_over, (const uint32_t *)d_start, r0, r1, (const uint16_t *)d_cs,
                           (const uint32_t *)d_ps, d_k0);
        HIPCHK(ctx, hipGetLastError());
        HIPCHK(ctx, rocprim::radix_sort_keys(d_sort, have, d_k0, d_k1, (size_t)m, 0u, 48u + rank_bits, ctx->st.B));
        hipLaunchKernelGGL(k_ib_over_unpack, grid, dim3(BLK), 0, ctx->st.B, d_off, (const uint32_t *)d_over, (const uint32_t *)d_start, r0, r1, (const uint64_t *)d_k1,
                           d_cs, d_ps);
        HIPCHK(ctx, hipGetLastError());
    }
    return CM_OK;
}

static int build_contig_arrays(cm_ctx *ctx, Slot &s, const uint8_t *genome, uint32_t ref_len, cm_build_stats *stats, hipEvent_t ev_a, hipEvent_t ev_b) {
    const uint64_t n_all = (uint64_t)1 << (2 * CM_WINDOW_SIZE);
    const int k = ctx->P.kmer, c = k - CM_WINDOW_SIZE;
    {
        uint8_t *g = nullptr;
        const size_t pad = cmc::CM_STAGE_PAD;
        HIPCHK(ctx, hipMalloc((void **)&g, (size_t)ref_len + 2 * pad));
        s.idx_allocs.push_back(g);
        HIPCHK(ctx, hipMemsetAsync(g, 0, (size_t)ref_len + 2 * pad, ctx->st.B));
        if (ref_len) HIPCHK(ctx, hipMemcpyAsync(g + pad, genome, (size_t)ref_len, hipMemcpyHostToDevice, ctx->st.B));
        s.X.genome = g + pad;
    }
    std::vector<void *> tmp;
    struct FreeTmp {
        cm_ctx *c;
        std::vector<void *> &v;
        ~FreeTmp() { free_all(c, v); }
    } free_tmp{ctx, tmp};
    size_t tmp_bytes = ((size_t)(n_all / S32_B) + 4) * sizeof(uint32_t);
    uint32_t *d_bs = nullptr, *d_off = nullptr;
    HIPCHK(ctx, hipMalloc((void **)&d_bs, tmp_bytes));
    tmp.push_back(d_bs);
    HIPCHK(ctx, hipMalloc((void **)&d_off, (n_all + 1) * sizeof(uint32_t)));
    s.idx_allocs.push_back(d_off);
    HIPCHK(ctx, hipEventRecord(ev_a, ctx->st.B));
    HIPCHK(ctx, hipMemsetAsync(d_off, 0, (n_all + 1) * sizeof(uint32_t), ctx->st.B));
    const uint32_t n_pos = ref_len >= (uint32_t)k ? ref_len - (uint32_t)k + 1u : 0u;
    const dim3 pgrid((unsigned)(((uint64_t)n_pos + IB_TILE - 1) / IB_TILE));
    if (n_pos) {
        hipLaunchKernelGGL(k_ib_positions<false>, pgrid, dim3(BLK), 0, ctx->st.B, s.X.genome, ref_len, n_pos, k, c, d_off, (uint16_t *)nullptr, (uint32_t *)nullptr);
        HIPCHK(ctx, hipGetLastError());
    }
    int rc;
    if ((rc = scan32(ctx, d_off, n_all + 1, d_off, d_bs, 0u, 1))) return rc;
    uint32_t total32 = 0;
    HIPCHK(ctx, hipMemcpyAsync(&total32, d_off + n_all, sizeof(uint32_t), hipMemcpyDeviceToHost, ctx->st.B));
    HIPCHK(ctx, hipStreamSynchronize(ctx->st.B));
    const uint64_t total = total32;
    if (total > (uint64_t)n_pos) return fail(ctx, CM_ELIMIT, "%llu entries from %u k-mer starts", (unsigned long long)total, n_pos);
    uint16_t *d_cs = nullptr;
    uint32_t *d_ps = nullptr;
    HIPCHK(ctx, hipMalloc((void **)&d_cs, (total ? total : 1) * sizeof(uint16_t)));
    s.idx_allocs.push_back(d_cs);
    HIPCHK(ctx, hipMalloc((void **)&d_ps, (total ? total : 1) * sizeof(uint32_t)));
    s.idx_allocs.push_back(d_ps);
    unsigned long long st[IB_ST_WORDS] = {0, 0, 0, 0, 0, 0};
    if (total) {
        hipLaunchKernelGGL(k_ib_positions<true>, pgrid, dim3(BLK), 0, ctx->st.B, s.X.genome, ref_len, n_pos, k, c, d_off, d_cs, d_ps);
        HIPCHK(ctx, hipGetLastError());
        if ((rc = ib_order(ctx, d_off, d_cs, d_ps, total, d_bs, tmp, st, &tmp_bytes))) return rc;
    }
    HIPCHK(ctx, hipEventRecord(ev_b, ctx->st.B));
    s.X.bucket_off = d_off;
    s.X.checksum = d_cs;
    s.X.pos = d_ps;
    s.X.n_entries = total;
    if ((rc = finish_contig(ctx, s))) return rc;
    if (stats) {
        float ms = 0.f;
        HIPCHK(ctx, hipEventElapsedTime(&ms, ev_a, ev_b));
        memset(stats, 0, sizeof *stats);
        stats->n_entries = total;
        stats->max_bucket = (uint32_t)st[IB_ST_MAX];
        stats->reserved = (uint32_t)std::min<size_t>(tmp_bytes >> 20, 0xffffffffu);
        for (int i = 0; i < 3; ++i) stats->buckets_by_path[i] = st[IB_ST_PATH + i];
        stats->ms_device = ms;
    }
    return CM_OK;
}

int cm_build_contig(cm_ctx *ctx, int slot, int32_t contig_num, const uint8_t *genome, uint32_t ref_len, cm_build_stats *stats) {
    if (!ctx) return CM_EINVAL;
    if (slot < 0 || slot >= MAX_SLOTS) return fail(ctx, CM_EINVAL, "slot %d out of range", slot);
    if (!genome && ref_len) return fail(ctx, CM_EINVAL, "null genome");
    HIPCHK(ctx, hipSetDevice(ctx->P.device));
    Slot &s = ctx->slots[slot];
    free_all(ctx, s.idx_allocs);
    s.d_desc = nullptr;
    s.loaded = false;
    ++s.gen;
    s.X = cm_index_view{};
    s.X.contig_num = contig_num;
    s.X.ref_len = ref_len;
    hipEvent_t ev_a = take_event(ctx), ev_b = take_event(ctx);
    if (!ev_a || !ev_b) return fail(ctx, CM_EHIP, "hipEventCreate failed");
    const int rc = build_contig_arrays(ctx, s, genome, ref_len, stats, ev_a, ev_b);
    if (rc != CM_OK) {
        (void)hipStreamSynchronize(ctx->st.B);
        (void)hipGetLastError();
        free_all(ctx, s.idx_allocs);
        s.d_desc = nullptr;
        s.loaded = false;
        s.X = cm_index_view{};
    }
    ctx->ev_free.push_back(ev_a);
    ctx->ev_free.push_back(ev_b);
    return rc;
}

int cm_index_download(cm_ctx *ctx, int slot, uint32_t *bucket_off, uint16_t *checksum, uint32_t *pos, uint64_t cap_entries, uint64_t *n_entries) {
    if (!ctx) return CM_EINVAL;
    int rc;
    if ((rc = check_slot(ctx, slot, false))) return rc;
    const Slot &s = ctx->slots[slot];
    const uint64_t n = s.X.n_entries;
    if (n_entries) *n_entries = n;
    if (!bucket_off && !checksum && !pos) return CM_OK;
    if ((checksum || pos) && cap_entries < n) return fail(ctx, CM_ELIMIT, "slot %d holds %llu entries, the buffers %llu", slot, (unsigned long long)n, (unsigned long long)cap_entries);
    HIPCHK(ctx, hipSetDevice(ctx->P.device));
    const size_t nb = ((size_t)1 << (2 * CM_WINDOW_SIZE)) + 1;
    if (bucket_off) HIPCHK(ctx, hipMemcpyAsync(bucket_off, s.X.bucket_off, nb * sizeof(uint32_t), hipMemcpyDeviceToHost, ctx->st.B));
    if (checksum && n) HIPCHK(ctx, hipMemcpyAsync(checksum, s.X.checksum, (size_t)n * sizeof(uint16_t), hipMemcpyDeviceToHost, ctx->st.B));
    if (pos && n) HIPCHK(ctx, hipMemcpyAsync(pos, s.X.pos, (size_t)n * sizeof(uint32_t), hipMemcpyDeviceToHost, ctx->st.B));
    HIPCHK(ctx, hipStreamSynchronize(ctx->st.B));
    return CM_OK;
}

int cm_load_annotation(cm_ctx *ctx, int slot, const cm_annot_view *av) {
    if (!ctx || !av) return CM_EINVAL;
    if (slot < 0 || slot >= MAX_SLOTS) return fail(ctx, CM_EINVAL, "slot %d out of range", slot);
    if (av->n_iv == 0 || av->n_chr == 0) return fail(ctx, CM_EINVAL, "annotation needs >= 1 interval and >= 1 chromosome");
    HIPCHK(ctx, hipSetDevice(ctx->P.device));
    Slot &s = ctx->slots[slot];
    free_all(ctx, s.ann_allocs);
    s.has_annot = false;
    ++s.gen;
    cmc::AnnotAosHost aos;
    cmc::build_annot_aos(*av, aos);
    cmc::AnnotDev &A = s.A;
    A = cmc::AnnotDev{};
    A.n_iv = av->n_iv; A.n_seg = av->n_seg; A.n_trans = av->n_trans; A.n_gene = av->n_gene; A.n_chr = av->n_chr; A.n_bits = av->n_bits;
    A.pair_reach = aos.pair_reach;
    int rc;
    auto &al = s.ann_allocs;
    if ((rc = up(ctx, al, aos.iv.data(), aos.iv.size(), &A.iv))) return rc;
    if ((rc = up(ctx, al, av->iv_seg, (size_t)av->iv_seg_off[av->n_iv], &A.iv_seg))) return rc;
    if ((rc = up(ctx, al, aos.seg.data(), aos.seg.size(), &A.seg))) return rc;
    if ((rc = up(ctx, al, av->seg_tid, (size_t)av->seg_tid_off[av->n_seg], &A.seg_tid))) return rc;
    if ((rc = up(ctx, al, aos.tr.data(), aos.tr.size(), &A.tr))) return rc;
    if ((rc = up(ctx, al, av->t2s, (size_t)av->t2s_off[av->n_trans], &A.t2s))) return rc;
    if ((rc = up(ctx, al, aos.gene.data(), aos.gene.size(), &A.gene))) return rc;
    if ((rc = up(ctx, al, av->near_border_bits, (size_t)(av->n_bits / 64), &A.near_border_bits))) return rc;
    if ((rc = up(ctx, al, av->intronic_bits, (size_t)(av->n_bits / 64), &A.intronic_bits))) return rc;
    if ((rc = up(ctx, al, av->chr_shift, (size_t)av->n_chr, &A.chr_shift))) return rc;
    if ((rc = up(ctx, al, av->chr_id, (size_t)av->n_chr, &A.chr_id))) return rc;
    if (av->iv_bucket && av->n_iv_bucket >= 2) {
        if ((rc = up(ctx, al, av->iv_bucket, (size_t)av->n_iv_bucket, &A.iv_bucket))) return rc;
        A.iv_bucket_shift = av->iv_bucket_shift;
        A.n_iv_bucket = av->n_iv_bucket;
    }
    HIPCHK(ctx, hipStreamSynchronize(ctx->st.B));
    {
        const long long mi = ctx->P.max_intron;
        bool ok = mi >= (long long)ctx->P.max_read_len + ctx->P.max_ed && mi < (1ll << 30);
        for (uint32_t i = 0; i < av->n_iv && ok; ++i) {
            if (av->iv_seg_off[i + 1] == av->iv_seg_off[i]) continue;
            const long long far = std::max<long long>((long long)av->iv_max_next_exon[i] + ctx->P.kmer, (long long)av->iv_max_end[i]);
            if (far - (long long)av->iv_spos[i] > mi) ok = false;
        }
        s.chain_parallel_ok = ok;
    }
    s.has_annot = true;
    return CM_OK;
}

int cm_unload_contig(cm_ctx *ctx, int slot) {
    if (!ctx || slot < 0 || slot >= MAX_SLOTS) return CM_EINVAL;
    (void)hipSetDevice(ctx->P.device);
    (void)hipStreamSynchronize(ctx->st.B);
    free_all(ctx, ctx->slots[slot].idx_allocs);
    free_all(ctx, ctx->slots[slot].ann_allocs);
    ctx->slots[slot].loaded = ctx->slots[slot].has_annot = false;
    ctx->slots[slot].d_desc = nullptr;
    ++ctx->slots[slot].gen;
    return CM_OK;
}

static int check_reads(cm_ctx *ctx, const cm_reads *rd, int *max_len_out) {
    const uint64_t n = rd->n_pairs;
    if (n > 0x3fffffffull) return fail(ctx, CM_ELIMIT, "more than 2^30 pairs in one batch");
    if (!rd->seq1 || !rd->seq2 || !rd->off1 || !rd->off2) return fail(ctx, CM_EINVAL, "null read arrays");
    int max_len = 0;
    const uint64_t lim = (uint64_t)ctx->P.max_read_len;
    uint64_t bad = 0, longest = 0;
    auto scan = [&](uint64_t lo, uint64_t hi, uint64_t *bad_o, uint64_t *long_o) {
        uint64_t bd = 0, lg = 0;
        for (uint64_t i = lo; i < hi; ++i) {
            const uint64_t l1 = rd->off1[i + 1] - rd->off1[i], l2 = rd->off2[i + 1] - rd->off2[i];
            const uint64_t m = l1 > l2 ? l1 : l2;
            if (m > lim && !bd) bd = i + 1;
            if (m > lg) lg = m;
        }
        *bad_o = bd;
        *long_o = lg;
    };
    const unsigned hw = std::thread::hardware_concurrency();
    const unsigned n_thr = n < (1u << 18) ? 1u : std::min(8u, hw ? hw : 1u);
    if (n_thr <= 1) {
        scan(0, n, &bad, &longest);
    } else {
        uint64_t bd[8] = {0}, lg[8] = {0};
        std::thread th[8];
        unsigned started = 1;
        try {
            for (; started < n_thr; ++started) th[started] = std::thread(scan, n * started / n_thr, n * (started + 1) / n_thr, &bd[started], &lg[started]);
        } catch (...) {
        }
        scan(0, n / n_thr, &bd[0], &lg[0]);
        for (unsigned k = started; k < n_thr; ++k) scan(n * k / n_thr, n * (k + 1) / n_thr, &bd[k], &lg[k]);
        for (unsigned k = 1; k < started; ++k) th[k].join();
        for (unsigned k = 0; k < n_thr; ++k) {
            if (bd[k] && !bad) bad = bd[k];
            if (lg[k] > longest) longest = lg[k];
        }
    }
    if (bad) {
        const uint64_t i = bad - 1;
        if (rd->off1[i + 1] < rd->off1[i] || rd->off2[i + 1] < rd->off2[i]) return fail(ctx, CM_EINVAL, "read offsets not monotone at pair %llu", (unsigned long long)i);
        return fail(ctx, CM_EINVAL, "pair %llu longer than max_read_len %d", (unsigned long long)i, ctx->P.max_read_len);
    }
    max_len = (int)longest;
    if (max_len / ctx->P.kmer > cmc::MAX_SEEDS) return fail(ctx, CM_ELIMIT, "%d seeds per read > %d supported", max_len / ctx->P.kmer, cmc::MAX_SEEDS);
    *max_len_out = max_len;
    return CM_OK;
}

static uint32_t tile_for(uint64_t n) {
    uint32_t tile_cap = TILE_PAIRS;
    if (n > 2ull * TILE_PAIRS) {
        const uint64_t half = ((n + 1) / 2 + 65535) / 65536 * 65536;
        tile_cap = (uint32_t)std::min<uint64_t>(half, TILE_PAIRS_MAX);
    }
    if (const char *e = getenv("CM_TILE_PAIRS")) {
        const long v = atol(e);
        if (v >= 64 && v <= (1l << 24)) tile_cap = (uint32_t)v;
    }
    return (uint32_t)(n < tile_cap ? n : tile_cap);
}

static int prepare_resident(cm_ctx *ctx, uint64_t n, int max_len) {
    ctx->n_seeds = max_len / ctx->P.kmer;
    ctx->max_len = max_len;
    HIPCHK(ctx, ensure(ctx, ctx->d_state, n * sizeof(cm_mapped_read)));
    HIPCHK(ctx, ensure(ctx, ctx->d_active, n));
    HIPCHK(ctx, ensure(ctx, ctx->d_active_b, n));
    HIPCHK(ctx, ensure(ctx, ctx->d_cat, n * sizeof(int32_t)));
    const uint32_t tile = tile_for(n);
    ctx->tile = tile;
    const size_t nprob = (size_t)tile * 4, nprobe = nprob * (size_t)(ctx->n_seeds ? ctx->n_seeds : 1);
    for (SeedSet &sd : ctx->seed) {
        HIPCHK(ctx, ensure(ctx, sd.sstart, nprobe * 4));
        HIPCHK(ctx, ensure(ctx, sd.scnt, nprobe * 4));
        HIPCHK(ctx, ensure(ctx, sd.sraw, nprobe * 4));
        HIPCHK(ctx, ensure(ctx, sd.celloff, (nprob + 2) * 8));
        HIPCHK(ctx, ensure(ctx, sd.bmax, (nprob / SCAN_ELEMS + 2) * 4));
        HIPCHK(ctx, ensure(ctx, sd.bsum, (nprob / SCAN_ELEMS + 2) * 8));
        HIPCHK(ctx, ensure(ctx, sd.cctr, CTR_WORDS * sizeof(unsigned int)));
        HIPCHK(ctx, ensure(ctx, sd.cblk, (size_t)N_CLS * (4 * (size_t)tile / CLS_T + 2) * sizeof(unsigned int)));
        HIPCHK(ctx, ensure(ctx, sd.cls4, (size_t)tile * 4));
        HIPCHK(ctx, ensure(ctx, sd.perm4, (size_t)tile * 4 * 4));
        HIPCHK(ctx, ensure(ctx, sd.thigh, (size_t)tile * 4 * sizeof(int32_t)));
    }
    for (ChainRecs &cr : ctx->rec) {
        HIPCHK(ctx, ensure(ctx, cr.chains, nprob * CM_BESTCHAINLIM * sizeof(cm_chain)));
        HIPCHK(ctx, ensure(ctx, cr.nchain, nprob * 4));
        HIPCHK(ctx, ensure(ctx, cr.high, nprob * 4));
        HIPCHK(ctx, ensure(ctx, cr.resid, (size_t)tile * 4 * sizeof(uint16_t)));
    }
    unsigned long long cap = (unsigned long long)nprob * 64ull;
    const unsigned long long worst = (unsigned long long)ctx->P.seed_lim * (unsigned long long)(ctx->n_seeds ? ctx->n_seeds : 1);
    if (cap < (8ull << 20)) cap = 8ull << 20;
    if (cap < worst) cap = worst;
    if (cap > ctx->dp.cells_cap || !ctx->dp.score) ctx->dp.cells_cap = cap;
    HIPCHK(ctx, ensure(ctx, ctx->dp.score, ctx->dp.cells_cap * sizeof(double)));
    HIPCHK(ctx, ensure(ctx, ctx->dp.prev, ctx->dp.cells_cap * sizeof(int32_t)));
    HIPCHK(ctx, ensure(ctx, ctx->sort.cls, (size_t)tile));
    PairSetMem &pm = ctx->pair_mem;
    HIPCHK(ctx, ensure(ctx, pm.perm, (size_t)tile * 4 * 2));
    HIPCHK(ctx, ensure(ctx, pm.hlist, (size_t)tile * 4 * 2));
    HIPCHK(ctx, ensure(ctx, ctx->d_hres, (size_t)HEAVY_GRID_MAX * (64 * sizeof(HRes) + HEAVY_SCRATCH)));
    if (heavy_pipeline()) {
        const size_t tc = getenv("CM_HP_TASKS_CAP") ? (size_t)std::max(1, atoi(getenv("CM_HP_TASKS_CAP"))) : std::max<size_t>((size_t)tile * 6, 4096);
        const size_t uc = getenv("CM_HP_UNP_CAP") ? (size_t)std::max(1, atoi(getenv("CM_HP_UNP_CAP"))) : std::max<size_t>((size_t)tile * 4, 4096);
        ctx->hp.tasks_cap = (uint32_t)tc;
        ctx->hp.unp_cap = (uint32_t)uc;
        HIPCHK(ctx, ensure(ctx, ctx->hp.pairs, (size_t)tile * sizeof(HPair)));
        HIPCHK(ctx, ensure(ctx, ctx->hp.list2, (size_t)tile * 4));
        HIPCHK(ctx, ensure(ctx, pm.hp_fall, (size_t)tile * 4 * 2));
        HIPCHK(ctx, ensure(ctx, pm.hp_fallctr, 2 * sizeof(unsigned int)));
        HIPCHK(ctx, ensure(ctx, ctx->hp.T, tc * sizeof(HTask)));
        HIPCHK(ctx, ensure(ctx, ctx->hp.tcls, tc));
        HIPCHK(ctx, ensure(ctx, ctx->hp.tperm, tc * 4));
        HIPCHK(ctx, ensure(ctx, ctx->hp.tblk, (size_t)N_CLS * (tc / CLS_T + 2) * sizeof(unsigned int)));
        HIPCHK(ctx, ensure(ctx, ctx->hp.tctr, CTR_WORDS * sizeof(unsigned int)));
        HIPCHK(ctx, ensure(ctx, ctx->hp.pre, tc * 4 * sizeof(cmc::PreDP)));
        HIPCHK(ctx, ensure(ctx, ctx->hp.q, tc * 4 * 4));
        HIPCHK(ctx, ensure(ctx, ctx->hp.res, tc * sizeof(HRes)));
        HIPCHK(ctx, ensure(ctx, ctx->hp.U, uc * sizeof(HUnp)));
        HIPCHK(ctx, ensure(ctx, ctx->hp.pre2, uc * 2 * sizeof(cmc::PreDP)));
        HIPCHK(ctx, ensure(ctx, ctx->hp.q2, uc * 2 * 4));
        HIPCHK(ctx, ensure(ctx, ctx->hp.lists, (size_t)HP_PLAN_GRID * HEAVY_LIST * 2));
        HIPCHK(ctx, ensure(ctx, ctx->hp.ctr, HC_WORDS * sizeof(unsigned int)));
    }
    {
        const uint32_t *before = pm.pair_err;
        HIPCHK(ctx, ensure(ctx, pm.pair_err, (size_t)tile * 4 * 2));
        if (pm.pair_err != before) HIPCHK(ctx, hipMemsetAsync(pm.pair_err, 0, (size_t)tile * 4 * 2, ctx->st.P));
    }
    HIPCHK(ctx, ensure(ctx, pm.retry_list, (size_t)tile * 4 * 2));
    HIPCHK(ctx, ensure(ctx, pm.retry_ctr, 4 * sizeof(unsigned int)));
    HIPCHK(ctx, ensure(ctx, ctx->d_heavy_load, sizeof(unsigned long long)));
    HIPCHK(ctx, ensure(ctx, ctx->d_spill, (size_t)RETRY_GRID * BLK_PAIR * RETRY_SPILL * sizeof(cmc::MemoSpill)));
    HIPCHK(ctx, ensure(ctx, pm.cls_ctr, 2 * CTR_WORDS * sizeof(unsigned int)));
    HIPCHK(ctx, ensure(ctx, ctx->sort.ctr2, CTR_WORDS * sizeof(unsigned int)));
    HIPCHK(ctx, ensure(ctx, ctx->sort.sub, (size_t)tile));
    HIPCHK(ctx, ensure(ctx, ctx->sort.perm1, (size_t)tile * 4));
    HIPCHK(ctx, ensure(ctx, ctx->sort.ctr3, CTR_WORDS * sizeof(unsigned int)));
    HIPCHK(ctx, ensure(ctx, ctx->sort.sub2, (size_t)tile));
    HIPCHK(ctx, ensure(ctx, ctx->sort.perm0, (size_t)tile * 4));
    HIPCHK(ctx, ensure(ctx, ctx->sort.blk_cnt, (size_t)N_CLS * (4 * (size_t)tile / CLS_T + 2) * sizeof(unsigned int)));
    if (getenv("CM_LANE_CLK")) {
#if defined(CM_DIAG)
        const size_t clk_words = 16 * 2 + 1;
#else
        const size_t clk_words = 1;
#endif
// ... 273 lines not shown
                                   (const int32_t *)rb.nchain, hp, pair_err, str_cap, (task_order && attempt == 0) ? (const uint32_t *)ctx->hp.tperm : (const uint32_t *)nullptr,
                                   (const unsigned int *)(ctx->hp.tctr + CTR_SUM));
                hipLaunchKernelGGL(k_hp_fold, dim3(pipe_grid), dim3(BLK_PAIR), 0, sp2, core, p0, (const uint32_t *)ctx->hp.list2, n_list2, n_heavy, attempt, hp,
                                   ctx->d_counters);
                hipLaunchKernelGGL(k_hp_unp_req, dim3(pipe_grid), dim3(BLK_PAIR), 0, sp2, core, rd, p0, attempt, (const cm_chain *)rb.chains, hp, str_cap);
                hipLaunchKernelGGL(k_hp_dp, dim3(pipe_grid), dim3(BLK_PAIR), lds_bytes, sp2, core, rd, p0, attempt, hp, 1, str_cap);
                hipLaunchKernelGGL(k_hp_unp, dim3(pipe_grid), dim3(BLK_PAIR), lds_bytes, sp2, core, rd, p0, attempt, (const cm_chain *)rb.chains, hp, pair_err,
                                   str_cap);
                hipLaunchKernelGGL(k_hp_finish, dim3(pipe_grid), dim3(BLK_PAIR), 0, sp2, core, p0, (const uint32_t *)ctx->hp.list2, n_list2, n_heavy, attempt, hp,
                                   ctx->d_state, act_out, ctx->d_cat, is_last_round, ctx->d_counters, ra1, (const int32_t *)rb.nchain, n_attempts == 1 ? 1 : 0);
            }
            HIPCHK(ctx, hipMemcpyAsync((void *)(ctx->h_pin + 14 + b), ps.hp_fallctr, sizeof(unsigned int), hipMemcpyDeviceToHost, sp2));
            {
                cm_ctx::Rerun &q = ctx->rerun[b];
                q.fall = true;
                q.lds_heavy = lds_heavy;
                q.str_cap = str_cap;
                q.fall_grid = std::min(heavy_grid, 256u);
            }
            if (!defer) {
                int rc;
                if ((rc = launch_fall_back(ctx, b, sp2))) return rc;
                ctx->rerun[b].fall = false;
            }
            ctx->launches[4] += 9 * n_attempts;
        } else {
        hipLaunchKernelGGL(k_pair_heavy, dim3(heavy_grid), dim3(BLK_PAIR), lds_heavy, sp2, core, rd, p0, hlist, cls_ctr + HEAVY_CLS, rb.chains,
                           rb.nchain, rb.high, ctx->d_state, act_out, ctx->d_cat, is_last_round, ctx->d_err, ctx->d_counters, str_cap,
                           ctx->d_lane_clk ? ctx->d_lane_clk + (size_t)nt * 16 + (size_t)(nt / 64 + 1) * 64 : nullptr, ctx->d_hres,
                           cls_ctr + CTR_NEXT + 1, ra1);
        ++ctx->launches[4];
        }
    }
    HIPCHK(ctx, hipEventRecord(ctx->ev.join_p, sp2));
    {
        Timer t(ctx, 2, sp);
        const unsigned want = (nt + BLK_PAIR - 1) / BLK_PAIR, cap = (heavy_pipeline() && ctx->P.band == 3) ? 2048u
                                                                                                           : 256u * 4u * slots_per_simd;
        hipLaunchKernelGGL(k_pair, dim3(want < cap ? want : cap), dim3(BLK_PAIR), lds_bytes, sp, core, rd, p0, nt, rb.chains, rb.nchain, rb.high,
                           ctx->d_state, act_out, ctx->d_cat, is_last_round, ctx->d_err, ctx->d_counters, str_cap, ctx->d_lane_clk, perm,
                           cls_ctr + CTR_SUM, cls_ctr + CTR_NEXT, ra1);
        HIPCHK(ctx, hipStreamWaitEvent(sp, ctx->ev.join_p, 0));
        ++ctx->launches[2];
    }
    HIPCHK(ctx, hipMemcpyAsync((void *)(ctx->h_pin + 12 + b), retry_ctr, sizeof(unsigned int), hipMemcpyDeviceToHost, sp));
    HIPCHK(ctx, hipEventRecord(ctx->ev.first[b], sp));
    ctx->rerun[b].deferred = defer;
    if (!defer) {
        HIPCHK(ctx, hipStreamWaitEvent(sp3, ctx->ev.first[b], 0));
        int rc;
        if ((rc = launch_rerun(ctx, b))) return rc;
        HIPCHK(ctx, hipEventRecord(ctx->ev.pair[b], sp3));
    }
    ctx->pair_pending[b] = true;
    HIPCHK(ctx, hipGetLastError());
    return CM_OK;
}

static int map_rounds_issue(cm_ctx *ctx, const int *slots, int n_rounds, int last_is_final, int *items_done, int *rounds_done) {
    int rc;
    const bool prefetch = last_is_final && ctx->staged && ctx->st_n_pairs <= ctx->n_pairs && ctx->st_max_len <= ctx->max_len;
    if (prefetch && ctx->ones_cap < ctx->st_n_pairs) {
        HIPCHK(ctx, ensure(ctx, ctx->d_ones, ctx->n_pairs));
        HIPCHK(ctx, hipMemsetAsync(ctx->d_ones, 1, ctx->n_pairs, ctx->st.B));
        ctx->ones_cap = ctx->n_pairs;
    }
    HIPCHK(ctx, hipEventRecord(ctx->ev.tail, ctx->st.B));
    HIPCHK(ctx, hipStreamWaitEvent(ctx->st.P, ctx->ev.tail, 0));
    HIPCHK(ctx, hipStreamWaitEvent(ctx->st.S, ctx->ev.tail, 0));
    HIPCHK(ctx, hipStreamWaitEvent(ctx->st.O, ctx->ev.tail, 0));
    HIPCHK(ctx, hipEventRecord(ctx->ev.flags, ctx->st.B));
    uint8_t *A[2] = {ctx->d_active, ctx->d_active_b};
    struct Item { uint64_t p0; uint32_t nt; int r; };
    std::vector<Item> items;
    const uint64_t n_tiles = (ctx->n_pairs + ctx->tile - 1) / ctx->tile;
    const bool round_major = n_tiles >= 2;
    auto tile_nt = [&](uint64_t t) { return (uint32_t)((ctx->n_pairs - t * ctx->tile < ctx->tile) ? ctx->n_pairs - t * ctx->tile : ctx->tile); };
    if (round_major) {
        for (int r = 0; r < n_rounds; ++r)
            for (uint64_t t = 0; t < n_tiles; ++t) items.push_back(Item{t * ctx->tile, tile_nt(t), r});
    } else {
        for (uint64_t t = 0; t < n_tiles; ++t)
            for (int r = 0; r < n_rounds; ++r) items.push_back(Item{t * ctx->tile, tile_nt(t), r});
    }
    const int n_items = (int)items.size();
    std::vector<int> tiles_of_round((size_t)n_rounds, 0);
    const bool use_pre = ctx->pre_ready && slots[0] == ctx->pre_slot && ctx->slots[slots[0]].gen == ctx->pre_gen && ctx->n_pairs == ctx->pre_n &&
                         items[0].nt == ctx->pre_nt && (ctx->item_base & 1) == ctx->pre_b;
    ctx->pre_ready = ctx->pre_launched = false;
    if (use_pre) ++ctx->launches[7];
    const ReadsDev rd_cur = current_reads(ctx);
    auto prep_flags = [&](int i) -> const uint8_t * {
        const int r = items[i].r;
        return round_major ? A[r & 1] : ((r == 0) ? A[0] : A[(r - 1) & 1]);
    };
    std::vector<char> seeded((size_t)n_items, 0);
    bool pre_seeded = false;
    const bool early_ok = round_major;
    auto issue_seed_early = [&](int i) -> int {
        HIPCHK(ctx, hipStreamWaitEvent(ctx->st.S, ctx->ev.flags, 0));
        if (n_tiles == 2 && i >= 2) HIPCHK(ctx, hipStreamWaitEvent(ctx->st.S, ctx->ev.first[(ctx->item_base + i) & 1], 0));
        const ChainRecs &rbe = ctx->rec[(ctx->item_base + i) & 1];
        const int e = run_seed_tile(ctx, make_core(ctx, ctx->slots[slots[items[i].r]]), rd_cur, items[i].p0, items[i].nt, prep_flags(i), i & 1, ctx->st.S, &rbe, true);
        seeded[(size_t)i] = 1;
        return e;
    };
    auto issue_seed = [&](int i, hipStream_t st) -> int {
        const int b = (ctx->item_base + i) & 1;
        int e;
        if ((e = settle_pair(ctx, b))) return e;
        if (ctx->pair_pending[b]) HIPCHK(ctx, hipStreamWaitEvent(st, ctx->ev.pair[b], 0));
        const ChainRecs &rbi = ctx->rec[b];
        e = run_seed_tile(ctx, make_core(ctx, ctx->slots[slots[items[i].r]]), rd_cur, items[i].p0, items[i].nt, prep_flags(i), i & 1, st, &rbi);
        seeded[(size_t)i] = 1;
        return e;
    };
    for (int i = 0; i < n_items; ++i) {
        const uint64_t p0 = items[i].p0;
        const uint32_t nt = items[i].nt;
        const int r = items[i].r, b = (ctx->item_base + i) & 1;
        const Slot &sl = ctx->slots[slots[r]];
        const KCore core = make_core(ctx, sl);
        const ChainRecs &rb = ctx->rec[b];
        const uint8_t *act_prep = prep_flags(i);
        auto ahead = [&]() -> int {
            if (i + 1 >= n_items || seeded[(size_t)i + 1]) return CM_OK;
            if (early_ok) return issue_seed_early(i + 1);
            const int bn = (ctx->item_base + i + 1) & 1;
            if (ctx->rerun[bn].deferred && hipEventQuery(ctx->ev.first[bn]) != hipSuccess) {
                (void)hipGetLastError();
                return CM_OK;
            }
            return issue_seed(i + 1, ctx->st.S);
        };
        auto late = [&]() -> int { return (i + 1 < n_items && !seeded[(size_t)i + 1]) ? issue_seed(i + 1, ctx->st.S) : CM_OK; };
        if (i == n_items - 1 && prefetch && !pre_seeded) {
            const Slot &sl0 = ctx->slots[slots[0]];
            const uint32_t nt0 = tile_for(ctx->st_n_pairs);
            const ReadsDev rd_next = reads_dev(ctx->st_rd);
            HIPCHK(ctx, hipStreamWaitEvent(ctx->st.S, ctx->ev.staged, 0));
            if ((rc = run_seed_tile(ctx, make_core(ctx, sl0), rd_next, 0, nt0, ctx->d_ones, n_items & 1, ctx->st.S, nullptr))) return rc;
            pre_seeded = true;
        }
        if (use_pre && i == 0) {
            if ((rc = ahead())) return rc;
        } else {
            if (!seeded[(size_t)i] && (rc = issue_seed(i, ctx->st.B))) return rc;
            if ((rc = settle_pair(ctx, b))) return rc;
            if (ctx->pair_pending[b]) {
                HIPCHK(ctx, hipStreamWaitEvent(ctx->st.B, ctx->ev.pair[b], 0));
                ctx->pair_pending[b] = false;
            }
            HIPCHK(ctx, hipEventRecord(ctx->ev.flags, ctx->st.B));
            if ((rc = run_chain_tile(ctx, core, rd_cur, p0, nt, sl.chain_parallel_ok, act_prep, rb, i & 1, ahead))) return rc;
            HIPCHK(ctx, hipEventRecord(ctx->ev.prep[b], ctx->st.B));
        }
        const int is_last = (r == n_rounds - 1) ? (last_is_final != 0) : 0;
        const bool same_tile = i > 0 && items[i - 1].p0 == p0;
        if ((rc = run_pair_tile(ctx, core, p0, nt, is_last, A[r & 1], A[(r + 1) & 1], rb, b, same_tile, round_major))) return rc;
        if ((rc = late())) return rc;
        ++*items_done;
        if (++tiles_of_round[(size_t)r] == (int)n_tiles) ++*rounds_done;
    }
    ctx->item_base = (ctx->item_base + n_items) & 1;
    *items_done = 0;
    if (prefetch) {
        const int b = ctx->item_base;
        const Slot &sl = ctx->slots[slots[0]];
        const KCore core = make_core(ctx, sl);
        const uint32_t nt = tile_for(ctx->st_n_pairs);
        HIPCHK(ctx, hipStreamWaitEvent(ctx->st.B, ctx->ev.staged, 0));
        if ((rc = settle_pair(ctx, b))) return rc;
        if (ctx->pair_pending[b]) {
            HIPCHK(ctx, hipStreamWaitEvent(ctx->st.B, ctx->ev.pair[b], 0));
            ctx->pair_pending[b] = false;
        }
        const ChainRecs &rbn = ctx->rec[b];
        const ReadsDev rd_next = reads_dev(ctx->st_rd);
        if (pre_seeded) {
            HIPCHK(ctx, hipStreamWaitEvent(ctx->st.B, ctx->ev.seed[n_items & 1], 0));
            if ((rc = seed_classes(ctx, 0, nt, ctx->d_ones, n_items & 1, ctx->st.B, &rbn))) return rc;
        } else if ((rc = run_seed_tile(ctx, core, rd_next, 0, nt, ctx->d_ones, n_items & 1, ctx->st.B, &rbn))) return rc;
        if ((rc = run_chain_tile(ctx, core, rd_next, 0, nt, sl.chain_parallel_ok, ctx->d_ones, rbn, n_items & 1))) return rc;
        HIPCHK(ctx, hipEventRecord(ctx->ev.prep[b], ctx->st.B));
        ctx->pre_launched = true;
        ctx->pre_slot = slots[0];
        ctx->pre_gen = sl.gen;
        ctx->pre_b = b;
        ctx->pre_nt = nt;
    }
    if ((rc = settle_pair(ctx, ctx->item_base, false)) || (rc = settle_pair(ctx, ctx->item_base ^ 1, false))) return rc;
    HIPCHK(ctx, hipEventRecord(ctx->ev.tail, ctx->st.R));
    HIPCHK(ctx, hipStreamWaitEvent(ctx->st.B, ctx->ev.tail, 0));
    ctx->pair_pending[0] = ctx->pair_pending[1] = false;
    if (n_rounds & 1) swap(ctx->d_active, ctx->d_active_b);
    *rounds_done = 0;
    return CM_OK;
}

int cm_map_rounds(cm_ctx *ctx, const int *slots, int n_rounds, int last_is_final) {
    if (!ctx || (n_rounds > 0 && !slots) || n_rounds < 0) return CM_EINVAL;
    int rc;
    for (int r = 0; r < n_rounds; ++r)
        if ((rc = check_slot(ctx, slots[r], true))) return rc;
    HIPCHK(ctx, hipSetDevice(ctx->P.device));
    if (ctx->n_pairs == 0 || n_rounds == 0) return CM_OK;
    int items_done = 0, rounds_done = 0;
    rc = map_rounds_issue(ctx, slots, n_rounds, last_is_final, &items_done, &rounds_done);
    if (rc == CM_OK) return rc;
    for (const StreamDef &d : STREAMS)
        if (d.st != &Streams::C) (void)hipStreamSynchronize(ctx->st.*d.st);
    ctx->rerun[0].deferred = ctx->rerun[1].deferred = false;
    ctx->seed[0].cls_deferred = ctx->seed[1].cls_deferred = false;
    ctx->item_base = (ctx->item_base + items_done) & 1;
    if (rounds_done & 1) swap(ctx->d_active, ctx->d_active_b);
    ctx->pair_pending[0] = ctx->pair_pending[1] = false;
    ctx->pre_ready = ctx->pre_launched = false;
    return rc;
}

int cm_map_round(cm_ctx *ctx, int slot, int is_last_round) { return cm_map_rounds(ctx, &slot, 1, is_last_round); }

int cm_sync(cm_ctx *ctx) {
    if (!ctx) return CM_EINVAL;
    HIPCHK(ctx, hipSetDevice(ctx->P.device));
    HIPCHK(ctx, hipStreamSynchronize(ctx->st.B));
    HIPCHK(ctx, hipStreamSynchronize(ctx->st.C));
    return check_dev_err(ctx);
}

int cm_reads_reset(cm_ctx *ctx) {
    if (!ctx) return CM_EINVAL;
    HIPCHK(ctx, hipSetDevice(ctx->P.device));
    if (ctx->n_pairs == 0) return CM_OK;
    KCore k{};
    k.P = ctx->P;
    hipLaunchKernelGGL(k_init_state, dim3((unsigned)((ctx->n_pairs + BLK - 1) / BLK)), dim3(BLK), 0, ctx->st.B, k, ctx->d_state, ctx->d_active,
                       ctx->d_cat, ctx->n_pairs);
    HIPCHK(ctx, hipGetLastError());
    return CM_OK;
}

#ifdef CM_TRACE_HOST
#define TRACE_T0 auto tr_t = std::chrono::steady_clock::now()
#define TRACE_PT(name) do { auto n_ = std::chrono::steady_clock::now(); fprintf(stderr, "[trace] %s %.1f us\n", name, std::chrono::duration<double, std::micro>(n_ - tr_t).count()); tr_t = n_; } while (0)
#else
#define TRACE_T0
#define TRACE_PT(name)
#endif
static int compact_active(cm_ctx *ctx) {
    const uint64_t n = ctx->n_pairs;
    if (n > 0xfffffff0ull) return fail(ctx, CM_ELIMIT, "cm_collect_*: too many pairs");
    const uint32_t nbk = (uint32_t)((n + CLS_T - 1) / CLS_T);
    HIPCHK(ctx, ensure(ctx, ctx->col.cls, n));
    HIPCHK(ctx, ensure(ctx, ctx->col.perm, n * 4));
    HIPCHK(ctx, ensure(ctx, ctx->col.blk, (size_t)N_CLS * (nbk + 2) * sizeof(unsigned int)));
    HIPCHK(ctx, ensure(ctx, ctx->col.ctr, CTR_WORDS * sizeof(unsigned int)));
    hipLaunchKernelGGL(k_active_cls, dim3((unsigned)((n + BLK - 1) / BLK)), dim3(BLK), 0, ctx->st.B, ctx->d_active, n, ctx->col.cls);
    hipLaunchKernelGGL(k_cls_hist, dim3(nbk), dim3(CLS_W), 0, ctx->st.B, ctx->col.cls, (uint32_t)n, ctx->col.blk, nbk, (const uint32_t *)nullptr,
                       (const unsigned int *)nullptr);
    hipLaunchKernelGGL(k_cls_scan, dim3(1), dim3(SCAN_CLS_T), 0, ctx->st.B, ctx->col.blk, nbk, ctx->col.ctr, -1, 1);
    hipLaunchKernelGGL(k_cls_place, dim3(nbk), dim3(CLS_W), 0, ctx->st.B, ctx->col.cls, (uint32_t)n, ctx->col.blk, nbk, ctx->col.ctr,
                       ctx->col.perm, (uint32_t *)nullptr, (const uint32_t *)nullptr, (const unsigned int *)nullptr);
    return CM_OK;
}
static int read_count(cm_ctx *ctx, uint64_t cap, unsigned int *cnt, const char *what) {
    HIPCHK(ctx, hipMemcpyAsync(ctx->h_pin, ctx->col.ctr, sizeof(unsigned int), hipMemcpyDeviceToHost, ctx->st.B));
    HIPCHK(ctx, hipMemcpyAsync(ctx->h_pin + 1, ctx->d_err, sizeof(int), hipMemcpyDeviceToHost, ctx->st.B));
    HIPCHK(ctx, hipStreamSynchronize(ctx->st.B));
    *cnt = *(const unsigned int *)ctx->h_pin;
    if (*(const int *)(ctx->h_pin + 1)) return check_dev_err(ctx);
    if (*cnt > cap) return fail(ctx, CM_ELIMIT, "%s: %u active pairs > cap %llu", what, *cnt, (unsigned long long)cap);
    return CM_OK;
}

int cm_collect_active(cm_ctx *ctx, uint64_t cap, uint64_t *out_idx, cm_mapped_read *out_state, uint64_t *out_n) {
    if (!ctx || !out_n || (cap && (!out_idx || !out_state))) return CM_EINVAL;
    HIPCHK(ctx, hipSetDevice(ctx->P.device));
    *out_n = 0;
    if (ctx->n_pairs == 0) return CM_OK;
    int rc = compact_active(ctx);
    if (rc) return rc;
    if (cap) {
        HIPCHK(ctx, ensure(ctx, ctx->col.idx, cap * sizeof(unsigned long long)));
        HIPCHK(ctx, ensure(ctx, ctx->col.st, cap * sizeof(cm_mapped_read)));
    }
    if (cap)
        hipLaunchKernelGGL(k_gather_active, dim3((unsigned)((cap + BLK - 1) / BLK)), dim3(BLK), 0, ctx->st.B, ctx->col.perm, ctx->col.ctr,
                           (unsigned long long)cap, ctx->d_state, ctx->col.idx, ctx->col.st);
    unsigned int cnt = 0;
    rc = read_count(ctx, cap, &cnt, "cm_collect_active");
    *out_n = cnt;
    if (rc) return rc;
    if (cnt) {
        HIPCHK(ctx, hipMemcpyAsync(out_idx, ctx->col.idx, (size_t)cnt * sizeof(unsigned long long), hipMemcpyDeviceToHost, ctx->st.B));
        HIPCHK(ctx, hipMemcpyAsync(out_state, ctx->col.st, (size_t)cnt * sizeof(cm_mapped_read), hipMemcpyDeviceToHost, ctx->st.B));
        HIPCHK(ctx, hipStreamSynchronize(ctx->st.B));
    }
    return CM_OK;
}

static int collect_records_into(cm_ctx *ctx, uint64_t index_base, uint64_t cap, cm_record *d_dst, uint64_t *out_n, const char *what) {
    *out_n = 0;
    if (ctx->n_pairs == 0) return CM_OK;
    int rc = compact_active(ctx);
    if (rc) return rc;
    if (cap)
        hipLaunchKernelGGL(k_gather_records, dim3((unsigned)((cap + BLK - 1) / BLK)), dim3(BLK), 0, ctx->st.B, ctx->col.perm, ctx->col.ctr,
                           (unsigned long long)cap, ctx->d_state, (unsigned long long)index_base, d_dst);
    unsigned int cnt = 0;
    rc = read_count(ctx, cap, &cnt, what);
    *out_n = cnt;
    return rc;
}

int cm_collect_records(cm_ctx *ctx, uint64_t index_base, uint64_t cap, cm_record *out, uint64_t *out_n) {
    if (!ctx || !out_n || (cap && !out)) return CM_EINVAL;
    HIPCHK(ctx, hipSetDevice(ctx->P.device));
    if (cap) HIPCHK(ctx, ensure(ctx, ctx->col.rec, cap * sizeof(cm_record)));
    int rc = collect_records_into(ctx, index_base, cap, ctx->col.rec, out_n, "cm_collect_records");
    if (rc) return rc;
    if (*out_n) {
        HIPCHK(ctx, hipMemcpyAsync(out, ctx->col.rec, (size_t)*out_n * sizeof(cm_record), hipMemcpyDeviceToHost, ctx->st.B));
        HIPCHK(ctx, hipStreamSynchronize(ctx->st.B));
    }
    return CM_OK;
}

int cm_collect_records_device(cm_ctx *ctx, uint64_t index_base, uint64_t cap, void *d_out, uint64_t *out_n) {
    if (!ctx || !out_n || (cap && !d_out)) return CM_EINVAL;
    HIPCHK(ctx, hipSetDevice(ctx->P.device));
    if (cap) {
        hipPointerAttribute_t at;
        if (hipPointerGetAttributes(&at, d_out) != hipSuccess || at.type != hipMemoryTypeDevice || at.device != ctx->P.device) {
            (void)hipGetLastError();
            return fail(ctx, CM_EINVAL, "cm_collect_records_device: d_out is not memory of device %d", ctx->P.device);
        }
    }
    return collect_records_into(ctx, index_base, cap, (cm_record *)d_out, out_n, "cm_collect_records_device");
}

int cm_host_alloc(cm_ctx *ctx, uint64_t bytes, void **out) {
    if (!ctx || !out) return CM_EINVAL;
    *out = nullptr;
    HIPCHK(ctx, hipSetDevice(ctx->P.device));
    HIPCHK(ctx, hipHostMalloc(out, bytes ? bytes : 1, hipHostMallocDefault));
    return CM_OK;
}

int cm_host_free(cm_ctx *ctx, void *p) {
    if (!ctx) return CM_EINVAL;
    if (p) HIPCHK(ctx, hipHostFree(p));
    return CM_OK;
}

int cm_host_register(cm_ctx *ctx, void *p, uint64_t bytes) {
    if (!ctx || !p || !bytes) return CM_EINVAL;
    HIPCHK(ctx, hipSetDevice(ctx->P.device));
    HIPCHK(ctx, hipHostRegister(p, bytes, hipHostRegisterDefault));
    return CM_OK;
}

int cm_host_unregister(cm_ctx *ctx, void *p) {
    if (!ctx) return CM_EINVAL;
    if (p) HIPCHK(ctx, hipHostUnregister(p));
    return CM_OK;
}

int cm_type_histogram(cm_ctx *ctx, uint64_t out[14]) {
    if (!ctx || !out) return CM_EINVAL;
    HIPCHK(ctx, hipSetDevice(ctx->P.device));
    for (int i = 0; i < 14; ++i) out[i] = 0;
    if (ctx->n_pairs == 0) return CM_OK;
    HIPCHK(ctx, ensure(ctx, ctx->d_type_hist, 16 * sizeof(unsigned long long)));
    HIPCHK(ctx, hipMemsetAsync(ctx->d_type_hist, 0, 16 * sizeof(unsigned long long), ctx->st.B));
    const unsigned grid = (unsigned)std::min<uint64_t>((ctx->n_pairs + BLK - 1) / BLK, 1024);
    hipLaunchKernelGGL(k_type_hist, dim3(grid), dim3(BLK), 0, ctx->st.B, ctx->d_state, ctx->n_pairs, ctx->d_type_hist);
    unsigned long long h[16];
    HIPCHK(ctx, hipMemcpyAsync(h, ctx->d_type_hist, sizeof h, hipMemcpyDeviceToHost, ctx->st.B));
    HIPCHK(ctx, hipStreamSynchronize(ctx->st.B));
    for (int i = 0; i < 14; ++i) out[i] = h[i];
    return check_dev_err(ctx);
}

int cm_reads_download(cm_ctx *ctx, cm_mapped_read *out_state, int32_t *out_category, uint8_t *out_active) {
    if (!ctx) return CM_EINVAL;
    HIPCHK(ctx, hipSetDevice(ctx->P.device));
    const uint64_t n = ctx->n_pairs;
    if (n) {
        if (out_state) HIPCHK(ctx, hipMemcpyAsync(out_state, ctx->d_state, n * sizeof(cm_mapped_read), hipMemcpyDeviceToHost, ctx->st.B));
        if (out_category) HIPCHK(ctx, hipMemcpyAsync(out_category, ctx->d_cat, n * sizeof(int32_t), hipMemcpyDeviceToHost, ctx->st.B));
        if (out_active) HIPCHK(ctx, hipMemcpyAsync(out_active, ctx->d_active, n, hipMemcpyDeviceToHost, ctx->st.B));
    }
    HIPCHK(ctx, hipStreamSynchronize(ctx->st.B));
    return check_dev_err(ctx);
}

int cm_map_batch(cm_ctx *ctx, int slot, int is_last_round, const cm_reads *reads, const cm_mapped_read *prior, cm_mapped_read *out_state,
                 int32_t *out_category) {
    int rc = cm_reads_upload(ctx, reads, prior);
    if (rc) return rc;
    if ((rc = cm_map_round(ctx, slot, is_last_round))) return rc;
    return cm_reads_download(ctx, out_state, out_category, nullptr);
}

int cm_seed_batch(cm_ctx *ctx, int slot, uint32_t *out_start, uint32_t *out_cnt, uint32_t *out_raw, uint32_t cap_probes, uint32_t *out_n_slots) {
    if (!ctx || !out_start || !out_cnt || !out_raw || !out_n_slots) return CM_EINVAL;
    int rc = check_slot(ctx, slot, false);
    if (rc) return rc;
    HIPCHK(ctx, hipSetDevice(ctx->P.device));
    *out_n_slots = (uint32_t)ctx->n_seeds;
    const uint64_t need = ctx->n_pairs * 4ull * (uint64_t)ctx->n_seeds;
    if (need > cap_probes) return fail(ctx, CM_EINVAL, "cm_seed_batch: need room for %llu probes", (unsigned long long)need);
    const KCore core = make_core(ctx, ctx->slots[slot]);
    for (uint64_t p0 = 0; p0 < ctx->n_pairs; p0 += ctx->tile) {
        const uint32_t nt = (uint32_t)((ctx->n_pairs - p0 < ctx->tile) ? ctx->n_pairs - p0 : ctx->tile);
        if ((rc = run_seed_tile(ctx, core, current_reads(ctx), p0, nt, ctx->d_active, 0, ctx->st.B, nullptr))) return rc;
        const size_t cnt = (size_t)nt * 4 * ctx->n_seeds, o = (size_t)p0 * 4 * ctx->n_seeds;
        HIPCHK(ctx, hipMemcpyAsync(out_start + o, ctx->seed[0].sstart, cnt * 4, hipMemcpyDeviceToHost, ctx->st.B));
        HIPCHK(ctx, hipMemcpyAsync(out_cnt + o, ctx->seed[0].scnt, cnt * 4, hipMemcpyDeviceToHost, ctx->st.B));
        HIPCHK(ctx, hipMemcpyAsync(out_raw + o, ctx->seed[0].sraw, cnt * 4, hipMemcpyDeviceToHost, ctx->st.B));
        HIPCHK(ctx, hipStreamSynchronize(ctx->st.B));
    }
    return CM_OK;
}

int cm_chain_batch(cm_ctx *ctx, int slot, cm_chain *out_chains, int32_t *out_nchain, int32_t *out_high) {
    if (!ctx || !out_chains || !out_nchain || !out_high) return CM_EINVAL;
    int rc = check_slot(ctx, slot, true);
    if (rc) return rc;
    HIPCHK(ctx, hipSetDevice(ctx->P.device));
    const KCore core = make_core(ctx, ctx->slots[slot]);
    for (uint64_t p0 = 0; p0 < ctx->n_pairs; p0 += ctx->tile) {
        const uint32_t nt = (uint32_t)((ctx->n_pairs - p0 < ctx->tile) ? ctx->n_pairs - p0 : ctx->tile);
        HIPCHK(ctx, hipMemsetAsync(ctx->rec[0].chains, 0, (size_t)nt * 4 * CM_BESTCHAINLIM * sizeof(cm_chain), ctx->st.B));
        const ChainRecs &rb0 = ctx->rec[0];
        if ((rc = run_seed_tile(ctx, core, current_reads(ctx), p0, nt, ctx->d_active, 0, ctx->st.B, &rb0))) return rc;
        if ((rc = run_chain_tile(ctx, core, current_reads(ctx), p0, nt, ctx->slots[slot].chain_parallel_ok, ctx->d_active, rb0, 0))) return rc;
        const size_t np = (size_t)nt * 4, o = (size_t)p0 * 4;
        HIPCHK(ctx, hipMemcpyAsync(out_chains + o * CM_BESTCHAINLIM, ctx->rec[0].chains, np * CM_BESTCHAINLIM * sizeof(cm_chain), hipMemcpyDeviceToHost,
                                   ctx->st.B));
        HIPCHK(ctx, hipMemcpyAsync(out_nchain + o, ctx->rec[0].nchain, np * 4, hipMemcpyDeviceToHost, ctx->st.B));
        HIPCHK(ctx, hipMemcpyAsync(out_high + o, ctx->rec[0].high, np * 4, hipMemcpyDeviceToHost, ctx->st.B));
        HIPCHK(ctx, hipStreamSynchronize(ctx->st.B));
    }
    return check_dev_err(ctx);
}

int cm_debug_counters(cm_ctx *ctx, unsigned long long *out) {
    if (!ctx || !out) return CM_EINVAL;
    HIPCHK(ctx, hipSetDevice(ctx->P.device));
    HIPCHK(ctx, hipMemcpyAsync(out, ctx->d_counters, 32 * sizeof(unsigned long long), hipMemcpyDeviceToHost, ctx->st.B));
    HIPCHK(ctx, hipStreamSynchronize(ctx->st.B));
    return CM_OK;
}

int cm_debug_lane_clk(cm_ctx *ctx, unsigned long long *out) {
    if (!ctx || !out || !ctx->d_lane_clk) return CM_EINVAL;
#if defined(CM_DIAG)
    HIPCHK(ctx, hipMemcpy(out, ctx->d_lane_clk, ctx->n_pairs * 8 * 33, hipMemcpyDeviceToHost));
#else
    HIPCHK(ctx, hipMemcpy(out, ctx->d_lane_clk, ctx->n_pairs * 8, hipMemcpyDeviceToHost));
#endif
    return CM_OK;
}

int cm_prof_enable(cm_ctx *ctx, int on) {
    if (!ctx) return CM_EINVAL;
    ctx->prof = on != 0;
    return CM_OK;
}

int cm_prof_reset(cm_ctx *ctx) {
    if (!ctx) return CM_EINVAL;
    HIPCHK(ctx, hipSetDevice(ctx->P.device));
    HIPCHK(ctx, hipStreamSynchronize(ctx->st.B));
    for (auto &r : ctx->recs) {
        ctx->ev_free.push_back(r.a);
        ctx->ev_free.push_back(r.b);
    }
    ctx->recs.clear();
    for (int i = 0; i < 8; ++i) {
        ctx->ms[i] = 0;
        ctx->launches[i] = 0;
    }
    HIPCHK(ctx, hipMemsetAsync(ctx->d_counters, 0, 32 * sizeof(unsigned long long), ctx->st.B));
    HIPCHK(ctx, hipStreamSynchronize(ctx->st.B));
    return CM_OK;
}

int cm_prof_get(cm_ctx *ctx, double ms[8], uint64_t launches[8]) {
    if (!ctx || !ms || !launches) return CM_EINVAL;
    HIPCHK(ctx, hipSetDevice(ctx->P.device));
    HIPCHK(ctx, hipStreamSynchronize(ctx->st.B));
    for (auto &r : ctx->recs) {
        float t = 0;
        if (hipEventElapsedTime(&t, r.a, r.b) == hipSuccess) ctx->ms[r.cls] += (double)t;
        ctx->ev_free.push_back(r.a);
        ctx->ev_free.push_back(r.b);
    }
    ctx->recs.clear();
    for (int i = 0; i < 8; ++i) {
        ms[i] = ctx->ms[i];
        launches[i] = ctx->launches[i];
    }
    return CM_OK;
}

int cm_prof_counters(cm_ctx *ctx, uint64_t c[8]) {
    if (!ctx || !c) return CM_EINVAL;
    HIPCHK(ctx, hipSetDevice(ctx->P.device));
    unsigned long long h[8] = {0, 0, 0, 0, 0, 0, 0, 0};
    HIPCHK(ctx, hipMemcpyAsync(h, ctx->d_counters, sizeof h, hipMemcpyDeviceToHost, ctx->st.B));
    HIPCHK(ctx, hipStreamSynchronize(ctx->st.B));
    for (int i = 0; i < 8; ++i) c[i] = h[i];
    return CM_OK;
}

}
```

circminer_amd/lib.py:

```python
from __future__ import annotations

import ctypes as C
import os

import numpy as np

HERE = os.path.dirname(os.path.abspath(__file__))
LIB_PATH = os.environ.get("CM_LIB") or os.path.join(HERE, "csrc", "libcmhot.so")

CM_BESTCHAINLIM = 30
CM_MAX_CHAIN_FRAGS = 16
CM_CONTIG_SIZE = 1_100_000_000

CAT = dict(CONCRD=0, DISCRD=1, CHIORF=2, CHIBSJ=3, CHI2BSJ=4, CONGEN=5, CHIFUS=6, CONGNM=7, OEA2=8,
           CANDID=9, OEANCH=10, ORPHAN=11, NOPROC_MANYHIT=12, NOPROC_NOMATCH=13)

u8p, u16p, u32p, u64p, i32p = (C.POINTER(t) for t in (C.c_uint8, C.c_uint16, C.c_uint32, C.c_uint64, C.c_int32))


class Params(C.Structure):
    _fields_ = [(n, C.c_int32) for n in ("kmer", "seed_lim", "max_read_len", "scan_level", "max_ed", "max_sc", "band",
                                         "max_tlen", "max_intron", "max_chain_len", "device", "reserved")]


# ... 2 lines not shown
                ("reserved", C.c_int32), ("start_signal", C.c_char_p), ("end_signal", C.c_char_p), ("start_bp_ref", C.c_char_p),
                ("end_bp_ref", C.c_char_p)]


class MappingArgs(C.Structure):
    _fields_ = [("index_path", C.c_char_p), ("index_info_path", C.c_char_p), ("gtf_path", C.c_char_p), ("fastq1", C.c_char_p),
                ("fastq2", C.c_char_p), ("out_prefix", C.c_char_p), ("params", Params), ("report", C.c_int32), ("n_threads", C.c_int32),
                ("batch_pairs", C.c_uint64), ("rank", C.c_int32), ("world", C.c_int32)]


class CircStats(C.Structure):
    _fields_ = [("pairs", C.c_uint64), ("candidate_rows", C.c_uint64), ("calls", C.c_uint64), ("seconds", C.c_double)]


class MappingStats(C.Structure):
    _fields_ = [("pairs", C.c_uint64), ("bsj_pairs", C.c_uint64), ("by_type", C.c_uint64 * 14), ("rounds", C.c_int32),
                ("reserved", C.c_int32), ("seconds_load", C.c_double), ("seconds_map", C.c_double), ("seconds_parse", C.c_double),
                ("seconds_device", C.c_double), ("seconds_write", C.c_double)]


def default_params(**kw) -> Params:
    d = dict(kmer=20, seed_lim=500, max_read_len=300, scan_level=0, max_ed=4, max_sc=7, band=3, max_tlen=500,
             max_intron=2_000_000, max_chain_len=30, device=0, reserved=0)
    d.update(kw)
    return Params(**d)


class CircArgs(C.Structure):
    _fields_ = [("index_path", C.c_char_p), ("index_info_path", C.c_char_p), ("gtf_path", C.c_char_p), ("out_prefix", C.c_char_p),
                ("params", Params), ("last_round", C.c_int32), ("window_size", C.c_int32), ("n_threads", C.c_int32), ("reserved", C.c_int32)]


class IndexView(C.Structure):
    _fields_ = [("contig_num", C.c_int32), ("ref_len", C.c_uint32), ("genome", u8p), ("bucket_off", u32p),
                ("checksum", u16p), ("pos", u32p), ("n_entries", C.c_uint64)]


class IndexRaw(C.Structure):
    _fields_ = [("contig_num", C.c_int32), ("ref_len", C.c_uint32), ("genome", u8p), ("n_buckets", C.c_uint32), ("hv", u32p),
                ("count14", u32p), ("table", C.c_void_p), ("table_slots", C.c_uint64)]


class BuildStats(C.Structure):
    _fields_ = [("n_entries", C.c_uint64), ("max_bucket", C.c_uint32), ("reserved", C.c_uint32), ("buckets_by_path", C.c_uint64 * 3),
                ("ms_device", C.c_double)]


class AnnotView(C.Structure):
    _fields_ = [("n_iv", C.c_uint32), ("iv_spos", u32p), ("iv_epos", u32p), ("iv_max_end", u32p), ("iv_min_end", u32p),
                ("iv_max_next_exon", u32p), ("iv_seg_off", u32p), ("iv_seg", u32p),
                ("n_seg", C.c_uint32), ("seg_start", u32p), ("seg_end", u32p), ("seg_next_exon_beg", u32p),
                ("seg_gene_id", u32p), ("seg_tid_off", u32p), ("seg_tid", u32p),
                ("n_trans", C.c_uint32), ("trans_start_ind", i32p), ("t2s_off", u32p), ("t2s", u8p),
                ("n_gene", C.c_uint32), ("gene_start", u32p), ("gene_end", u32p),
                ("n_bits", C.c_uint64), ("near_border_bits", u64p), ("intronic_bits", u64p),
                ("n_chr", C.c_uint32), ("chr_shift", u32p), ("chr_id", i32p),
                ("iv_bucket", u32p), ("iv_bucket_shift", C.c_uint32), ("n_iv_bucket", C.c_uint32),
                ("n_giv", C.c_uint32), ("giv_spos", u32p), ("giv_epos", u32p), ("giv_gene_off", u32p), ("giv_gene", u32p)]


class MappedRead(C.Structure):
    _fields_ = [(n, C.c_uint32) for n in ("spos_r1", "spos_r2", "epos_r1", "epos_r2", "qspos_r1", "qspos_r2",
                                          "qepos_r1", "qepos_r2", "mlen_r1", "mlen_r2")] + \
               [(n, C.c_int32) for n in ("ed_r1", "ed_r2", "type", "tlen", "contig_num", "chr_id")] + \
               [("junc_num", C.c_uint16), ("r1_forward", C.c_uint8), ("r2_forward", C.c_uint8),
                ("gm_compatible", C.c_uint8), ("pad", C.c_uint8 * 3)]


MAPPED_DTYPE = np.dtype([(n, "<u4") for n in ("spos_r1", "spos_r2", "epos_r1", "epos_r2", "qspos_r1", "qspos_r2",
                                               "qepos_r1", "qepos_r2", "mlen_r1", "mlen_r2")] +
                        [(n, "<i4") for n in ("ed_r1", "ed_r2", "type", "tlen", "contig_num", "chr_id")] +
                        [("junc_num", "<u2"), ("r1_forward", "u1"), ("r2_forward", "u1"), ("gm_compatible", "u1"),
                         ("pad", "u1", (3,))])
assert MAPPED_DTYPE.itemsize == C.sizeof(MappedRead) == 72
RECORD_DTYPE = np.dtype([("pair", "<u8"), ("state", MAPPED_DTYPE)])

CHAIN_DTYPE = np.dtype([("score", "<f4"), ("chain_len", "<u4"), ("rpos", "<u4", (CM_MAX_CHAIN_FRAGS,)),
                        ("qpos", "<i4", (CM_MAX_CHAIN_FRAGS,))])
assert CHAIN_DTYPE.itemsize == 136


class Reads(C.Structure):
    _fields_ = [("n_pairs", C.c_uint64), ("seq1", u8p), ("off1", u64p), ("seq2", u8p), ("off2", u64p)]


class ChrInfo(C.Structure):
    _fields_ = [("name", C.c_char_p), ("contig_id", C.c_uint32), ("start_pos", C.c_uint32), ("len", C.c_uint32)]


class FastqBatch(C.Structure):
    _fields_ = [("reads", Reads), ("qual1", u8p), ("qual2", u8p), ("names1", C.c_void_p), ("names2", C.c_void_p),
                ("name_off1", u64p), ("name_off2", u64p), ("prior", C.c_void_p)]


def ptr(a: np.ndarray, t):
    return a.ctypes.data_as(t)


class ReadBatch:

    def __init__(self, seq1: np.ndarray, seq2: np.ndarray, len1=None, len2=None):
        if seq1.ndim == 2:
            n, L1 = seq1.shape
            L2 = seq2.shape[1]
            self.off1 = (np.arange(n + 1, dtype=np.uint64) * L1)
            self.off2 = (np.arange(n + 1, dtype=np.uint64) * L2)
            self.seq1 = np.ascontiguousarray(seq1, dtype=np.uint8).reshape(-1)
            self.seq2 = np.ascontiguousarray(seq2, dtype=np.uint8).reshape(-1)
        else:
            self.seq1 = np.ascontiguousarray(seq1, dtype=np.uint8)
            self.seq2 = np.ascontiguousarray(seq2, dtype=np.uint8)
            self.off1 = np.concatenate([[0], np.cumsum(len1)]).astype(np.uint64)
            self.off2 = np.concatenate([[0], np.cumsum(len2)]).astype(np.uint64)
            n = len(self.off1) - 1
        if self.seq1.size == 0:
            self.seq1 = np.zeros(1, np.uint8)
        if self.seq2.size == 0:
            self.seq2 = np.zeros(1, np.uint8)
        self.n = int(n)
        self.c = Reads(self.n, ptr(self.seq1, u8p), ptr(self.off1, u64p), ptr(self.seq2, u8p), ptr(self.off2, u64p))

    def max_len(self) -> int:
        if self.n == 0:
            return 0
        return int(max(np.diff(self.off1).max(), np.diff(self.off2).max()))


_lib = None


RELEASE_HOOK = C.CFUNCTYPE(None, C.c_void_p, C.c_void_p, C.c_uint64)


def load(path: str = LIB_PATH) -> C.CDLL:
    global _lib
    if _lib is not None:
        return _lib
    if not os.path.exists(path):
        raise RuntimeError(f"{path} is missing: run `python -c 'import __graft_entry__ as g; g.build()'` "
                           "(the hot path is HIP-only; there is no CPU fallback)")
    L = C.CDLL(path)
    vp = C.c_void_p
    pp = C.POINTER
    sigs = {
        "cm_create": (C.c_int, [pp(Params), pp(vp)]),
        "cm_destroy": (None, [vp]),
        "cm_last_error": (C.c_char_p, [vp]),
        "cm_load_contig": (C.c_int, [vp, C.c_int, pp(IndexView)]),
        "cm_load_annotation": (C.c_int, [vp, C.c_int, pp(AnnotView)]),
        "cm_load_contig_raw": (C.c_int, [vp, C.c_int, pp(IndexRaw)]),
        "cm_host_next_contig_raw": (C.c_int, [vp, C.c_int, pp(IndexRaw), pp(C.c_int)]),
        "cm_build_contig": (C.c_int, [vp, C.c_int, C.c_int32, u8p, C.c_uint32, pp(BuildStats)]),
        "cm_index_download": (C.c_int, [vp, C.c_int, vp, vp, vp, C.c_uint64, pp(C.c_uint64)]),
        "cm_unload_contig": (C.c_int, [vp, C.c_int]),
        "cm_reads_upload": (C.c_int, [vp, pp(Reads), vp]),
        "cm_reads_stage": (C.c_int, [vp, pp(Reads), vp]),
        "cm_reads_swap": (C.c_int, [vp]),
        "cm_map_round": (C.c_int, [vp, C.c_int, C.c_int]),
        "cm_map_rounds": (C.c_int, [vp, i32p, C.c_int, C.c_int]),
        "cm_reads_download": (C.c_int, [vp, vp, vp, vp]),
        "cm_map_batch": (C.c_int, [vp, C.c_int, C.c_int, pp(Reads), vp, vp, vp]),
        "cm_sync": (C.c_int, [vp]),
        "cm_reads_reset": (C.c_int, [vp]),
        "cm_collect_active": (C.c_int, [vp, C.c_uint64, vp, vp, pp(C.c_uint64)]),
        "cm_collect_records": (C.c_int, [vp, C.c_uint64, C.c_uint64, vp, pp(C.c_uint64)]),
        "cm_collect_records_device": (C.c_int, [vp, C.c_uint64, C.c_uint64, vp, pp(C.c_uint64)]),
        "cm_host_alloc": (C.c_int, [vp, C.c_uint64, pp(vp)]),
        "cm_host_free": (C.c_int, [vp, vp]),
        "cm_host_register": (C.c_int, [vp, vp, C.c_uint64]),
        "cm_host_unregister": (C.c_int, [vp, vp]),
        "cm_type_histogram": (C.c_int, [vp, pp(C.c_uint64)]),
        "cm_seed_batch": (C.c_int, [vp, C.c_int, vp, vp, vp, C.c_uint32, pp(C.c_uint32)]),
        "cm_chain_batch": (C.c_int, [vp, C.c_int, vp, vp, vp]),
        "cm_prof_enable": (C.c_int, [vp, C.c_int]),
        "cm_prof_reset": (C.c_int, [vp]),
        "cm_prof_get": (C.c_int, [vp, pp(C.c_double), pp(C.c_uint64)]),
        "cm_prof_counters": (C.c_int, [vp, pp(C.c_uint64)]),
        "cm_host_build_index": (C.c_int, [u8p, C.c_uint32, C.c_int32, C.c_int32, C.c_int, pp(IndexView)]),
        "cm_host_free_index": (None, [pp(IndexView)]),
        "cm_host_index_stats": (C.c_int, [pp(IndexView), C.c_int32, C.c_int, pp(C.c_uint64)]),
        "cm_host_build_annotation": (C.c_int, [C.c_char_p, pp(ChrInfo), C.c_uint32, u32p, C.c_uint32, C.c_int32,
                                               pp(AnnotView)]),
        "cm_host_free_annotation": (None, [pp(AnnotView), C.c_uint32]),
        "cm_host_pack_genome": (C.c_int, [C.c_char_p, C.c_char_p, C.c_char_p, C.c_uint32]),
        "cm_host_read_index_info": (C.c_int, [C.c_char_p, pp(pp(ChrInfo)), pp(C.c_uint32)]),
        "cm_host_free_index_info": (None, [pp(ChrInfo), C.c_uint32]),
        "cm_host_write_index": (C.c_int, [C.c_char_p, C.c_char_p, C.c_int32, C.c_int, C.c_int]),
        "cm_host_open_index": (C.c_int, [C.c_char_p, pp(vp), pp(C.c_int32), pp(C.c_int32), pp(C.c_uint32)]),
        "cm_host_next_contig": (C.c_int, [vp, C.c_int, pp(IndexView), pp(C.c_int)]),
        "cm_host_next_contig_genome": (C.c_int, [vp, pp(IndexView), pp(C.c_int)]),
        "cm_host_free_loaded_contig": (None, [pp(IndexView)]),
        "cm_host_close_index": (None, [vp]),
        "cm_fastq_open": (C.c_int, [C.c_char_p, C.c_char_p, pp(ChrInfo), C.c_uint32, C.c_int32, pp(vp)]),
        "cm_fastq_open_shard": (C.c_int, [C.c_char_p, C.c_char_p, pp(ChrInfo), C.c_uint32, C.c_int32, C.c_int32, C.c_int32, C.c_int, pp(vp),
                                          pp(C.c_uint64), pp(C.c_uint64)]),
        "cm_merge_parts": (C.c_int, [C.c_char_p, C.c_int32, C.c_int32, C.c_int32]),
        "cm_fastq_next": (C.c_int, [vp, C.c_uint64, pp(FastqBatch)]),
        "cm_fastq_close": (None, [vp]),
        "cm_fastq_set_release_hook": (None, [vp, RELEASE_HOOK, vp]),
        "cm_writer_open": (C.c_int, [C.c_char_p, C.c_char_p, pp(ChrInfo), C.c_uint32, pp(vp)]),
        "cm_write_remain": (C.c_int, [vp, pp(FastqBatch), vp, vp, C.c_uint64]),
        "cm_write_remain_records": (C.c_int, [vp, pp(FastqBatch), vp, C.c_uint64]),
        "cm_write_pam": (C.c_int, [vp, pp(FastqBatch), vp, vp, C.c_uint64]),
        "cm_host_gene_overlap": (C.c_int, [pp(AnnotView), C.c_uint32, pp(u32p), pp(C.c_uint32)]),
        "cm_sort_remain": (C.c_int, [C.c_char_p, C.c_char_p]),
        "cm_regional_table_build": (C.c_int, [vp, C.c_uint32, C.c_int32, C.c_int32, pp(u32p), pp(u32p)]),
        "cm_regional_table_free": (None, [u32p, u32p]),
        "cm_circ_report": (C.c_int, [pp(CircRes), C.c_uint64, C.c_char_p]),
        "cm_mapping_run": (C.c_int, [pp(MappingArgs), pp(MappingStats), C.c_char_p, C.c_uint64]),
        "cm_circ_call": (C.c_int, [pp(Params), C.c_int32, C.c_uint32, pp(IndexView), pp(AnnotView), pp(ChrInfo), C.c_uint32, pp(FastqBatch),
                                   C.c_char_p, C.c_char_p, pp(CircStats)]),
        "cm_circ_run": (C.c_int, [pp(CircArgs), pp(CircStats), C.c_char_p, C.c_uint64]),
        "cm_write_sam_header": (C.c_int, [vp]),
        "cm_write_sam": (C.c_int, [vp, pp(FastqBatch), vp, vp, C.c_uint64]),
        "cm_writer_flush": (C.c_int, [vp]),
        "cm_writer_close": (None, [vp]),
    }
    sigs["cm_abi_sizes"] = (C.c_int, [pp(C.c_uint32), C.c_uint32])
    for name, (res, args) in sigs.items():
        fn = getattr(L, name)
        fn.restype = res
        fn.argtypes = args
    got = (C.c_uint32 * 16)()
    n = L.cm_abi_sizes(got, 16)
    mine = [C.sizeof(t) for t in (Params, IndexView, AnnotView, MappedRead, Reads, C.c_uint8 * RECORD_DTYPE.itemsize, ChrInfo, FastqBatch, MappingArgs,
                                  MappingStats, CircRes, CircArgs, CircStats, IndexRaw, BuildStats)]
    if n != len(mine) or list(got[:n]) != mine:
        raise RuntimeError(f"circminer_amd.lib: struct sizes differ from {path}: library {list(got[:max(n, 0)])}, ctypes {mine}")
    _lib = L
    return L


EXPORTED_SYMBOLS = ["cm_create", "cm_destroy", "cm_last_error", "cm_load_contig", "cm_load_contig_raw", "cm_host_next_contig_raw", "cm_load_annotation",
                    "cm_unload_contig", "cm_reads_upload", "cm_reads_stage", "cm_reads_swap", "cm_map_round", "cm_map_rounds", "cm_reads_download", "cm_map_batch",
                    "cm_sync", "cm_reads_reset", "cm_collect_active", "cm_collect_records", "cm_collect_records_device", "cm_abi_sizes", "cm_host_alloc", "cm_host_free", "cm_host_register", "cm_host_unregister", "cm_type_histogram", "cm_write_remain_records", "cm_seed_batch", "cm_chain_batch", "cm_prof_enable", "cm_prof_reset", "cm_prof_get",
                    "cm_prof_counters", "cm_host_build_index", "cm_host_free_index", "cm_host_index_stats", "cm_host_build_annotation",
                    "cm_host_free_annotation", "cm_host_pack_genome", "cm_host_read_index_info", "cm_host_free_index_info",
                    "cm_host_write_index", "cm_host_open_index", "cm_host_next_contig", "cm_host_next_contig_genome", "cm_host_free_loaded_contig",
                    "cm_host_close_index", "cm_fastq_open", "cm_fastq_open_shard", "cm_merge_parts", "cm_fastq_next", "cm_fastq_set_release_hook", "cm_fastq_close", "cm_writer_open", "cm_write_remain",
                    "cm_write_pam", "cm_write_sam_header", "cm_write_sam", "cm_writer_flush", "cm_writer_close", "cm_mapping_run", "cm_sort_remain", "cm_circ_report", "cm_circ_call", "cm_circ_run", "cm_host_gene_overlap", "cm_regional_table_build", "cm_regional_table_free",
                    "cm_build_contig", "cm_index_download"]


class HostIndex:

    def __init__(self, contigs, chr_table, gtf_path, kmer=20, max_read_len=300, n_threads=8, index_dir=None):
        L = load()
        self.L = L
        self.contigs = [np.ascontiguousarray(c, dtype=np.uint8) for c in contigs]
        self.views = []
        self._mapped = []
        self.kmer = kmer
        for ci, g in enumerate(self.contigs):
            iv = IndexView()
            if index_dir is None:
                rc = L.cm_host_build_index(ptr(g, u8p), len(g), kmer, ci, n_threads, C.byref(iv))
                if rc != 0:
                    raise RuntimeError(f"cm_host_build_index failed: {rc}")
            else:
                arrs = [np.memmap(os.path.join(index_dir, f"c{ci}.{nm}"), dtype=dt, mode="r")
                        for nm, dt in (("off", np.uint32), ("cks", np.uint16), ("pos", np.uint32))]
                if len(arrs[0]) != (1 << 28) + 1 or len(arrs[1]) != len(arrs[2]) or int(arrs[0][-1]) != len(arrs[2]):
                    raise RuntimeError(f"index files of contig {ci} in {index_dir} are inconsistent")
                self._mapped.append(arrs)
                iv = IndexView(ci, len(g), ptr(g, u8p), C.cast(arrs[0].ctypes.data, u32p), C.cast(arrs[1].ctypes.data, u16p),
                               C.cast(arrs[2].ctypes.data, u32p), len(arrs[2]))
            self.views.append(iv)
        n_con = len(self.contigs)
        self._names = [t[0].encode() for t in chr_table]
        chrs = (ChrInfo * len(chr_table))(*[ChrInfo(self._names[i], t[1], t[2], t[3]) for i, t in enumerate(chr_table)])
        clen = np.asarray([len(c) for c in self.contigs], dtype=np.uint32)
        self.annots = (AnnotView * n_con)()
        rc = L.cm_host_build_annotation(gtf_path.encode(), chrs, len(chr_table), ptr(clen, u32p), n_con, max_read_len,
                                        self.annots)
        if rc != 0:
            raise RuntimeError(f"cm_host_build_annotation failed: {rc}")
        self.chr_table = list(chr_table)
        self.n_contigs = n_con

    def hit_stats(self, seed_lim=500, n_threads=8):
        res = []
        for iv in self.views:
            o = (C.c_uint64 * 4)()
            rc = self.L.cm_host_index_stats(C.byref(iv), seed_lim, n_threads, o)
            if rc != 0:
                raise RuntimeError(f"cm_host_index_stats failed: {rc}")
            res.append(tuple(int(x) for x in o))
        return res

    def save_index(self, index_dir):
        os.makedirs(index_dir, exist_ok=True)
        for ci, iv in enumerate(self.views):
            n = int(iv.n_entries)
            np.ctypeslib.as_array(iv.bucket_off, ((1 << 28) + 1,)).tofile(os.path.join(index_dir, f"c{ci}.off"))
            np.ctypeslib.as_array(iv.checksum, (max(n, 1),))[:n].tofile(os.path.join(index_dir, f"c{ci}.cks"))
            np.ctypeslib.as_array(iv.pos, (max(n, 1),))[:n].tofile(os.path.join(index_dir, f"c{ci}.pos"))

    def close(self):
        if self.views:
            if not self._mapped:
                for iv in self.views:
                    self.L.cm_host_free_index(C.byref(iv))
            self._mapped = []
            self.L.cm_host_free_annotation(self.annots, self.n_contigs)
            self.views = []

    def __del__(self):
        try:
            self.close()
        except Exception:
            pass


def pack_genome(fasta: str, contig_size: int = CM_CONTIG_SIZE):
    packed, info = fasta + ".packed.fa", fasta + ".packed.fa.index.info"
    rc = load().cm_host_pack_genome(fasta.encode(), packed.encode(), info.encode(), contig_size)
    if rc != 0:
        raise RuntimeError(f"cm_host_pack_genome failed ({rc})")
    return packed, info


def write_index(packed_fa: str, kmer: int = 20, compact: bool = False, n_threads: int = 8) -> str:
    idx = packed_fa + ".index"
    rc = load().cm_host_write_index(packed_fa.encode(), idx.encode(), kmer, int(compact), n_threads)
    if rc != 0:
        raise RuntimeError(f"cm_host_write_index failed ({rc})")
    return idx


class IndexFile:

    def __init__(self, path: str, n_threads: int = 8, genome_only: bool = False, raw: bool = False):
        self.L = load()
        self.h = C.c_void_p()
        self.genome_only = genome_only
        self.raw = raw
        kmer, full, nrec = C.c_int32(0), C.c_int32(0), C.c_uint32(0)
        rc = self.L.cm_host_open_index(path.encode(), C.byref(self.h), C.byref(kmer), C.byref(full), C.byref(nrec))
        if rc != 0:
            raise RuntimeError(f"cm_host_open_index failed ({rc}): {path}")
        self.kmer, self.full, self.n_records, self.n_threads = kmer.value, full.value > 0, nrec.value, n_threads
        self.table_less = full.value < 0
        self._cur = None
        if self.table_less and not genome_only:
            self.close()
            raise RuntimeError(f"{path} is a packed FASTA: it has no k-mer table, open it with genome_only=True")

    def __iter__(self):
        return self

    def _drop(self):
        if self._cur is not None:
            self.L.cm_host_free_loaded_contig(C.byref(self._cur))
            self._cur = None

    def __next__(self):
        self._drop()
        iv, loaded = IndexView(), C.c_int(0)
        if self.raw:
            rw = IndexRaw()
            rc = self.L.cm_host_next_contig_raw(self.h, self.n_threads, C.byref(rw), C.byref(loaded))
            if rc != 0:
                raise RuntimeError(f"cm_host_next_contig_raw failed ({rc})")
            if not loaded.value:
                raise StopIteration
            return rw
        if self.genome_only:
            rc = self.L.cm_host_next_contig_genome(self.h, C.byref(iv), C.byref(loaded))
        else:
            rc = self.L.cm_host_next_contig(self.h, self.n_threads, C.byref(iv), C.byref(loaded))
        if rc != 0:
            raise RuntimeError(f"cm_host_next_contig failed ({rc})")
        if not loaded.value:
            raise StopIteration
        self._cur = iv
        return iv

    def close(self):
        self._drop()
        if self.h:
            self.L.cm_host_close_index(self.h)
            self.h = C.c_void_p()


def chr_array(chr_table):
    arr = (ChrInfo * max(len(chr_table), 1))()
    for i, (name, contig, start, ln) in enumerate(chr_table):
        arr[i] = ChrInfo(name.encode() if isinstance(name, str) else name, contig, start, ln)
    return arr


class ParsedBatch:

    def __init__(self, fb: FastqBatch):
# ... 49 lines not shown
    st = CircStats()
    rc = L.cm_circ_call(C.byref(params), window, n_con, views, host_index.annots, chrs, len(chr_table), C.byref(sorted_batch.fb),
                        candidates_path.encode(), report_path.encode(), C.byref(st))
    if rc != 0:
        raise RuntimeError(f"cm_circ_call failed ({rc})")
    return st


def run_circ(index_path, gtf, out_prefix, last_round, params=None, n_threads=4, index_info=None, window=0):
    L = load()
    a = CircArgs(index_path.encode(), (index_info or index_path + ".info").encode(), gtf.encode(), out_prefix.encode(),
                 params if params is not None else default_params(kmer=0), last_round, window, n_threads, 0)
    st = CircStats()
    err = C.create_string_buffer(1024)
    rc = L.cm_circ_run(C.byref(a), C.byref(st), err, len(err))
    if rc != 0:
        raise RuntimeError(f"cm_circ_run failed ({rc}): {err.value.decode()}")
    return st


def run_mapping(index_path, gtf, fastq1, fastq2, out_prefix, params=None, report=1, n_threads=4, batch_pairs=0, index_info=None, rank=0, world=1):
    L = load()
    a = MappingArgs(index_path.encode(), (index_info or index_path + ".info").encode(), gtf.encode(), fastq1.encode(), fastq2.encode(),
                    out_prefix.encode(), params if params is not None else default_params(), report, n_threads, batch_pairs, rank, world)
    st = MappingStats()
    err = C.create_string_buffer(1024)
    rc = L.cm_mapping_run(C.byref(a), C.byref(st), err, len(err))
    if rc != 0:
        raise RuntimeError(f"cm_mapping_run failed ({rc}): {err.value.decode()}")
    return st


def merge_parts(out_prefix, rounds, world, report=1):
    rc = load().cm_merge_parts(out_prefix.encode(), rounds, world, report)
    if rc != 0:
        raise RuntimeError(f"cm_merge_parts failed ({rc})")


class FastqReader:

    def __init__(self, r1: str, r2: str, chr_table=(), max_ed: int = 4, rank: int = 0, world: int = 1, n_threads: int = 0):
        self.L = load()
        self._chrs = chr_array(list(chr_table))
        self.h = C.c_void_p()
        first, count = C.c_uint64(0), C.c_uint64(0)
        if world == 1:
            rc = self.L.cm_fastq_open(r1.encode(), r2.encode(), self._chrs, len(chr_table), max_ed, C.byref(self.h))
        else:
            rc = self.L.cm_fastq_open_shard(r1.encode(), r2.encode(), self._chrs, len(chr_table), max_ed, rank, world, n_threads, C.byref(self.h),
                                            C.byref(first), C.byref(count))
        if rc != 0:
            raise RuntimeError(f"cm_fastq_open failed ({rc})")
        self.first_pair, self.n_pairs = first.value, (count.value if world > 1 else None)

    def next_batch(self, max_pairs: int):
        fb = FastqBatch()
        rc = self.L.cm_fastq_next(self.h, max_pairs, C.byref(fb))
        if rc != 0:
            raise RuntimeError(f"cm_fastq_next failed ({rc}): malformed FASTQ")
        return ParsedBatch(fb) if fb.reads.n_pairs else None

    def close(self):
        if self.h:
            self.L.cm_fastq_close(self.h)
            self.h = C.c_void_p()


class RecordWriter:

    def __init__(self, path1: str, path2=None, chr_table=()):
        self.L = load()
        self._chrs = chr_array(list(chr_table))
        self.h = C.c_void_p()
        rc = self.L.cm_writer_open(path1.encode(), path2.encode() if path2 else None, self._chrs, len(chr_table), C.byref(self.h))
        if rc != 0:
            raise RuntimeError(f"cm_writer_open failed ({rc})")

    def _call(self, fn, batch: ParsedBatch, states: np.ndarray, sel):
        st = np.ascontiguousarray(states)
        sp, ns = None, 0
        if sel is not None:
            sel = np.ascontiguousarray(sel, dtype=np.uint64)
            sp, ns = sel.ctypes.data, len(sel)
        rc = fn(self.h, C.byref(batch.fb), st.ctypes.data, sp, ns)
        if rc != 0:
            raise RuntimeError(f"writer failed ({rc})")

    def write_remain(self, batch, states, sel=None):
        self._call(self.L.cm_write_remain, batch, states, sel)

    def write_pam(self, batch, states, sel=None):
        self._call(self.L.cm_write_pam, batch, states, sel)

    def write_sam_header(self):
        if self.L.cm_write_sam_header(self.h) != 0:
            raise RuntimeError("cm_write_sam_header failed")

    def write_sam(self, batch, states, sel=None):
        self._call(self.L.cm_write_sam, batch, states, sel)

    def close(self):
        if self.h:
            rc = self.L.cm_writer_flush(self.h)
            self.L.cm_writer_close(self.h)
            self.h = C.c_void_p()
            if rc != 0:
                raise RuntimeError(f"writing failed ({rc}): output file is incomplete")


class HotPath:

    def __init__(self, params: Params):
        self.L = load()
        self.params = params
        self.h = C.c_void_p()
        rc = self.L.cm_create(C.byref(params), C.byref(self.h))
        if rc != 0:
            raise RuntimeError(f"cm_create failed ({rc}): no usable HIP device / bad params")
        self.n = 0
        self._pinned = []

    def _chk(self, rc, what):
        if rc != 0:
            raise RuntimeError(f"{what} failed ({rc}): {self.L.cm_last_error(self.h).decode()}")

    def load_contig(self, slot, iv: IndexView, av: AnnotView = None):
        self._chk(self.L.cm_load_contig(self.h, slot, C.byref(iv)), "cm_load_contig")
        if av is not None:
            self._chk(self.L.cm_load_annotation(self.h, slot, C.byref(av)), "cm_load_annotation")

    def load_contig_raw(self, slot, raw: IndexRaw, av: AnnotView = None):
        self._chk(self.L.cm_load_contig_raw(self.h, slot, C.byref(raw)), "cm_load_contig_raw")
        if av is not None:
            self._chk(self.L.cm_load_annotation(self.h, slot, C.byref(av)), "cm_load_annotation")

    def build_contig(self, slot, contig_num, genome: np.ndarray, av: AnnotView = None) -> BuildStats:
        g = np.ascontiguousarray(genome, dtype=np.uint8)
        st = BuildStats()
        self._chk(self.L.cm_build_contig(self.h, slot, contig_num, ptr(g, u8p) if g.size else None, g.size, C.byref(st)), "cm_build_contig")
        if av is not None:
            self._chk(self.L.cm_load_annotation(self.h, slot, C.byref(av)), "cm_load_annotation")
        return st

    def index_arrays(self, slot):
        n = C.c_uint64(0)
        self._chk(self.L.cm_index_download(self.h, slot, None, None, None, 0, C.byref(n)), "cm_index_download")
        off = np.empty((1 << 28) + 1, np.uint32)
        cks = np.empty(n.value, np.uint16)
        pos = np.empty(n.value, np.uint32)
        self._chk(self.L.cm_index_download(self.h, slot, off.ctypes.data, cks.ctypes.data if n.value else None, pos.ctypes.data if n.value else None,
                                           n.value, C.byref(n)), "cm_index_download")
        return off, cks, pos

    def upload(self, batch: ReadBatch, prior: np.ndarray = None):
        self.n = batch.n
        p = prior.ctypes.data if prior is not None else None
        self._chk(self.L.cm_reads_upload(self.h, C.byref(batch.c), p), "cm_reads_upload")

    def stage(self, batch: ReadBatch, prior: np.ndarray = None):
        self._staged_n = batch.n
        p = prior.ctypes.data if prior is not None else None
        self._chk(self.L.cm_reads_stage(self.h, C.byref(batch.c), p), "cm_reads_stage")

    def swap(self):
        self._chk(self.L.cm_reads_swap(self.h), "cm_reads_swap")
        self.n = self._staged_n

    def pinned_batch(self, seq1: np.ndarray, seq2: np.ndarray) -> "ReadBatch":
        n, L1 = seq1.shape
        L2 = seq2.shape[1]
        s1 = self.host_array(n * L1, np.uint8)
        s2 = self.host_array(n * L2, np.uint8)
        s1[:] = seq1.reshape(-1)
        s2[:] = seq2.reshape(-1)
        o1 = self.host_array(n + 1, np.uint64)
        o2 = self.host_array(n + 1, np.uint64)
        o1[:] = np.arange(n + 1, dtype=np.uint64) * L1
        o2[:] = np.arange(n + 1, dtype=np.uint64) * L2
        b = ReadBatch.__new__(ReadBatch)
        b.seq1, b.seq2, b.off1, b.off2, b.n = s1, s2, o1, o2, int(n)
        b.c = Reads(b.n, ptr(s1, u8p), ptr(o1, u64p), ptr(s2, u8p), ptr(o2, u64p))
        return b

    def map_round(self, slot, is_last):
        self._chk(self.L.cm_map_round(self.h, slot, int(is_last)), "cm_map_round")

    def map_rounds(self, slots, last_is_final=True):
        arr = (C.c_int32 * len(slots))(*slots)
        self._chk(self.L.cm_map_rounds(self.h, arr, len(slots), int(last_is_final)), "cm_map_rounds")

    def sync(self):
        self._chk(self.L.cm_sync(self.h), "cm_sync")

    def reset(self):
        self._chk(self.L.cm_reads_reset(self.h), "cm_reads_reset")

    def collect_active(self, cap=None):
        cap = int(cap if cap is not None else max(self.n, 1))
        if getattr(self, "_col_cap", 0) < cap:
            self._col_idx = self.host_array(cap, np.uint64)
            self._col_st = self.host_array(cap, MAPPED_DTYPE)
            self._col_cap = cap
        n = C.c_uint64(0)
        self._chk(self.L.cm_collect_active(self.h, cap, self._col_idx.ctypes.data, self._col_st.ctypes.data, C.byref(n)), "cm_collect_active")
        return self._col_idx[:n.value], self._col_st[:n.value]

    def collect_records(self, index_base=0, cap=None):
        cap = int(cap if cap is not None else max(self.n, 1))
        if getattr(self, "_rec_cap", 0) < cap:
            self._rec = self.host_array(cap, RECORD_DTYPE)
            self._rec_cap = cap
        n = C.c_uint64(0)
        self._chk(self.L.cm_collect_records(self.h, int(index_base), cap, self._rec.ctypes.data, C.byref(n)), "cm_collect_records")
        return self._rec[:n.value]

    def collect_records_device(self, index_base, cap, dev_ptr):
        n = C.c_uint64(0)
        self._chk(self.L.cm_collect_records_device(self.h, int(index_base), int(cap), C.c_void_p(int(dev_ptr)), C.byref(n)),
                  "cm_collect_records_device")
        return int(n.value)

    def host_array(self, n, dtype):
        dt = np.dtype(dtype)
        p = C.c_void_p()
        self._chk(self.L.cm_host_alloc(self.h, max(int(n), 1) * dt.itemsize, C.byref(p)), "cm_host_alloc")
        self._pinned.append(p.value)
        buf = (C.c_uint8 * (max(int(n), 1) * dt.itemsize)).from_address(p.value)
        return np.frombuffer(buf, dtype=dt, count=int(n))

    def download(self):
        st = np.zeros(self.n, dtype=MAPPED_DTYPE)
        cat = np.zeros(self.n, dtype=np.int32)
        act = np.zeros(self.n, dtype=np.uint8)
        self._chk(self.L.cm_reads_download(self.h, st.ctypes.data, cat.ctypes.data, act.ctypes.data), "cm_reads_download")
        return st, cat, act

    def seeds(self, slot, n_slots_cap=24):
        cap = self.n * 4 * n_slots_cap
        a = np.zeros(cap, np.uint32)
        b = np.zeros(cap, np.uint32)
        c = np.zeros(cap, np.uint32)
        ns = C.c_uint32(0)
        self._chk(self.L.cm_seed_batch(self.h, slot, a.ctypes.data, b.ctypes.data, c.ctypes.data, cap, C.byref(ns)),
                  "cm_seed_batch")
        k = self.n * 4 * ns.value
        return a[:k], b[:k], c[:k], ns.value

    def chains(self, slot):
        ch = np.zeros(self.n * 4 * CM_BESTCHAINLIM, dtype=CHAIN_DTYPE)
        nc = np.zeros(self.n * 4, np.int32)
        hh = np.zeros(self.n * 4, np.int32)
        self._chk(self.L.cm_chain_batch(self.h, slot, ch.ctypes.data, nc.ctypes.data, hh.ctypes.data), "cm_chain_batch")
        return ch, nc, hh

    def prof(self, on=True):
        self._chk(self.L.cm_prof_enable(self.h, int(on)), "cm_prof_enable")

    def prof_reset(self):
        self._chk(self.L.cm_prof_reset(self.h), "cm_prof_reset")

    def prof_get(self):
        ms = (C.c_double * 8)()
        n = (C.c_uint64 * 8)()
        self._chk(self.L.cm_prof_get(self.h, ms, n), "cm_prof_get")
        cnt = (C.c_uint64 * 8)()
        self._chk(self.L.cm_prof_counters(self.h, cnt), "cm_prof_counters")
        return list(ms), list(n), list(cnt)

    def close(self):
        if self.h:
            self._col_idx = self._col_st = self._rec = None
            self._rec_cap = 0
            self._col_cap = 0
            for p in self._pinned:
                self.L.cm_host_free(self.h, p)
            self._pinned = []
            self.L.cm_destroy(self.h)
            self.h = C.c_void_p()

    def __del__(self):
        try:
            self.close()
        except Exception:
            pass
```

include/circminer_hot.h:

```cpp
#ifndef CIRCMINER_HOT_H
#define CIRCMINER_HOT_H

#include <stddef.h>
#include <stdint.h>

#ifdef __cplusplus
extern "C" {
#endif

enum {
    CM_CONCRD = 0, CM_DISCRD = 1, CM_CHIORF = 2, CM_CHIBSJ = 3, CM_CHI2BSJ = 4, CM_CONGEN = 5,
    CM_CHIFUS = 6, CM_CONGNM = 7, CM_OEA2 = 8, CM_CANDID = 9, CM_OEANCH = 10, CM_ORPHAN = 11,
    CM_NOPROC_MANYHIT = 12, CM_NOPROC_NOMATCH = 13
};

enum {
    CM_OK = 0,
    CM_EINVAL = -1,
    CM_ENODEV = -2,
    CM_ENOMEM = -3,
    CM_EHIP = -4,
    CM_ESTATE = -5,
    CM_ELIMIT = -6,
    CM_EIO = -7
};

#define CM_WINDOW_SIZE 14
#define CM_BESTCHAINLIM 30
#ifndef CM_MAX_CHAIN_FRAGS
#define CM_MAX_CHAIN_FRAGS 16
#endif
#define CM_MAX_SEEDS_PER_READ 24
#define CM_CONTIG_SIZE 1100000000u

typedef struct cm_params {
    int32_t kmer;
    int32_t seed_lim;
    int32_t max_read_len;
    int32_t scan_level;
    int32_t max_ed;
    int32_t max_sc;
    int32_t band;
    int32_t max_tlen;
    int32_t max_intron;
    int32_t max_chain_len;
    int32_t device;
    int32_t reserved;
} cm_params;

typedef struct cm_index_view {
    int32_t contig_num;
    uint32_t ref_len;
    const uint8_t *genome;
    const uint32_t *bucket_off;
    const uint16_t *checksum;
    const uint32_t *pos;
    uint64_t n_entries;
} cm_index_view;

typedef struct cm_annot_view {
    uint32_t n_iv;
    const uint32_t *iv_spos, *iv_epos;
    const uint32_t *iv_max_end, *iv_min_end, *iv_max_next_exon;
    const uint32_t *iv_seg_off;
    const uint32_t *iv_seg;
    uint32_t n_seg;
    const uint32_t *seg_start, *seg_end, *seg_next_exon_beg, *seg_gene_id;
    const uint32_t *seg_tid_off;
    const uint32_t *seg_tid;
    uint32_t n_trans;
    const int32_t *trans_start_ind;
    const uint32_t *t2s_off;
    const uint8_t *t2s;
    uint32_t n_gene;
    const uint32_t *gene_start, *gene_end;
    uint64_t n_bits;
    const uint64_t *near_border_bits;
    const uint64_t *intronic_bits;
    uint32_t n_chr;
    const uint32_t *chr_shift;
    const int32_t *chr_id;
    const uint32_t *iv_bucket;
    uint32_t iv_bucket_shift, n_iv_bucket;
    uint32_t n_giv;
    const uint32_t *giv_spos, *giv_epos, *giv_gene_off, *giv_gene;
} cm_annot_view;

typedef struct cm_mapped_read {
    uint32_t spos_r1, spos_r2, epos_r1, epos_r2;
    uint32_t qspos_r1, qspos_r2, qepos_r1, qepos_r2;
    uint32_t mlen_r1, mlen_r2;
    int32_t ed_r1, ed_r2;
    int32_t type;
    int32_t tlen;
    int32_t contig_num;
    int32_t chr_id;
    uint16_t junc_num;
    uint8_t r1_forward, r2_forward, gm_compatible, pad[3];
} cm_mapped_read;

typedef struct cm_chain {
    float score;
    uint32_t chain_len;
    uint32_t rpos[CM_MAX_CHAIN_FRAGS];
    int32_t qpos[CM_MAX_CHAIN_FRAGS];
} cm_chain;

typedef struct cm_ctx cm_ctx;

typedef struct cm_reads {
    uint64_t n_pairs;
    const uint8_t *seq1;
    const uint64_t *off1;
    const uint8_t *seq2;
    const uint64_t *off2;
} cm_reads;

int cm_create(const cm_params *p, cm_ctx **out);
void cm_destroy(cm_ctx *ctx);
const char *cm_last_error(const cm_ctx *ctx);

int cm_load_contig(cm_ctx *ctx, int slot, const cm_index_view *iv);
struct cm_index_raw;
int cm_load_contig_raw(cm_ctx *ctx, int slot, const struct cm_index_raw *raw);
int cm_load_annotation(cm_ctx *ctx, int slot, const cm_annot_view *av);
typedef struct cm_build_stats {
    uint64_t n_entries;
    uint32_t max_bucket;
    uint32_t reserved;
    uint64_t buckets_by_path[3];
    double ms_device;
} cm_build_stats;
int cm_build_contig(cm_ctx *ctx, int slot, int32_t contig_num, const uint8_t *genome, uint32_t ref_len,
                    cm_build_stats *stats );
int cm_index_download(cm_ctx *ctx, int slot, uint32_t *bucket_off, uint16_t *checksum, uint32_t *pos,
                      uint64_t cap_entries, uint64_t *n_entries);
int cm_unload_contig(cm_ctx *ctx, int slot);

int cm_reads_upload(cm_ctx *ctx, const cm_reads *reads, const cm_mapped_read *prior);

int cm_reads_stage(cm_ctx *ctx, const cm_reads *reads, const cm_mapped_read *prior);
int cm_reads_swap(cm_ctx *ctx);

int cm_map_round(cm_ctx *ctx, int slot, int is_last_round);

int cm_map_rounds(cm_ctx *ctx, const int *slots, int n_rounds, int last_is_final);

int cm_reads_download(cm_ctx *ctx, cm_mapped_read *out_state, int32_t *out_category, uint8_t *out_active);

int cm_map_batch(cm_ctx *ctx, int slot, int is_last_round, const cm_reads *reads,
                 const cm_mapped_read *prior, cm_mapped_read *out_state, int32_t *out_category);

int cm_sync(cm_ctx *ctx);

int cm_reads_reset(cm_ctx *ctx);

int cm_collect_active(cm_ctx *ctx, uint64_t cap, uint64_t *out_idx, cm_mapped_read *out_state, uint64_t *out_n);
typedef struct cm_record {
    uint64_t pair;
    cm_mapped_read state;
} cm_record;
int cm_collect_records(cm_ctx *ctx, uint64_t index_base, uint64_t cap, cm_record *out, uint64_t *out_n);
int cm_collect_records_device(cm_ctx *ctx, uint64_t index_base, uint64_t cap, void *d_out, uint64_t *out_n);

int cm_host_alloc(cm_ctx *ctx, uint64_t bytes, void **out);
int cm_host_register(cm_ctx *ctx, void *p, uint64_t bytes);
int cm_host_unregister(cm_ctx *ctx, void *p);
int cm_type_histogram(cm_ctx *ctx, uint64_t out[14]);
int cm_host_free(cm_ctx *ctx, void *p);

int cm_seed_batch(cm_ctx *ctx, int slot, uint32_t *out_start, uint32_t *out_cnt, uint32_t *out_raw,
                  uint32_t cap_probes, uint32_t *out_n_slots);
int cm_chain_batch(cm_ctx *ctx, int slot, cm_chain *out_chains, int32_t *out_nchain, int32_t *out_high);

int cm_prof_enable(cm_ctx *ctx, int on);
int cm_prof_reset(cm_ctx *ctx);
int cm_prof_get(cm_ctx *ctx, double ms[8], uint64_t launches[8]);
int cm_prof_counters(cm_ctx *ctx, uint64_t c[8]);

int cm_host_build_index(const uint8_t *genome, uint32_t ref_len, int32_t kmer, int32_t contig_num,
                        int n_threads, cm_index_view *out);
void cm_host_free_index(cm_index_view *iv);
int cm_host_index_stats(const cm_index_view *iv, int32_t seed_lim, int n_threads, uint64_t out[4]);

typedef struct cm_chr_info {
    const char *name;
    uint32_t contig_id;
    uint32_t start_pos;
    uint32_t len;
} cm_chr_info;
int cm_host_build_annotation(const char *gtf_path, const cm_chr_info *chrs, uint32_t n_chr,
                             const uint32_t *contig_len, uint32_t n_contigs, int32_t max_read_len,
                             cm_annot_view *out);
void cm_host_free_annotation(cm_annot_view *av, uint32_t n_contigs);
int cm_host_gene_overlap(const cm_annot_view *av, uint32_t pos, const uint32_t **genes, uint32_t *n_genes);

int cm_host_pack_genome(const char *fasta_path, const char *packed_fa_path, const char *index_info_path,
                        uint32_t contig_size);
int cm_host_read_index_info(const char *path, cm_chr_info **out, uint32_t *n);
void cm_host_free_index_info(cm_chr_info *chrs, uint32_t n);
int cm_host_write_index(const char *packed_fa_path, const char *index_path, int32_t kmer, int compact,
                        int n_threads);
typedef struct cm_index_file cm_index_file;
int cm_host_open_index(const char *index_path, cm_index_file **out, int32_t *kmer, int32_t *is_full,
                       uint32_t *n_records);
int cm_host_next_contig(cm_index_file *f, int n_threads, cm_index_view *out, int *loaded);
typedef struct cm_index_raw {
    int32_t contig_num;
    uint32_t ref_len;
    const uint8_t *genome;
    uint32_t n_buckets;
    const uint32_t *hv;
    const uint32_t *count14;
    const void *table;
    uint64_t table_slots;
} cm_index_raw;
int cm_host_next_contig_raw(cm_index_file *f, int n_threads, cm_index_raw *out, int *loaded);
int cm_host_next_contig_genome(cm_index_file *f, cm_index_view *out, int *loaded);
void cm_host_free_loaded_contig(cm_index_view *iv);
void cm_host_close_index(cm_index_file *f);

typedef struct cm_fastq_batch {
    cm_reads reads;
    const uint8_t *qual1, *qual2;
    const char *names1, *names2;
    const uint64_t *name_off1, *name_off2;
    const cm_mapped_read *prior;
} cm_fastq_batch;
typedef struct cm_fastq cm_fastq;
int cm_fastq_open(const char *r1_path, const char *r2_path, const cm_chr_info *chrs, uint32_t n_chr, int32_t max_ed,
                  cm_fastq **out);
int cm_fastq_open_shard(const char *r1_path, const char *r2_path, const cm_chr_info *chrs, uint32_t n_chr, int32_t max_ed,
                        int32_t rank, int32_t world, int n_threads, cm_fastq **out, uint64_t *first_pair, uint64_t *n_pairs);
int cm_fastq_next(cm_fastq *f, uint64_t max_pairs, cm_fastq_batch *out);
void cm_fastq_set_release_hook(cm_fastq *f, void (*fn)(void *user, const void *ptr, uint64_t bytes), void *user);
void cm_fastq_close(cm_fastq *f);

typedef struct cm_writer cm_writer;
int cm_writer_open(const char *path1, const char *path2, const cm_chr_info *chrs, uint32_t n_chr, cm_writer **out);
int cm_write_remain(cm_writer *w, const cm_fastq_batch *b, const cm_mapped_read *states, const uint64_t *sel, uint64_t n_sel);
int cm_write_remain_records(cm_writer *w, const cm_fastq_batch *batch, const cm_record *recs, uint64_t n);
int cm_write_pam(cm_writer *w, const cm_fastq_batch *b, const cm_mapped_read *states, const uint64_t *sel, uint64_t n_sel);
int cm_write_sam_header(cm_writer *w);
int cm_write_sam(cm_writer *w, const cm_fastq_batch *b, const cm_mapped_read *states, const uint64_t *sel, uint64_t n_sel);
int cm_writer_flush(cm_writer *w);
void cm_writer_close(cm_writer *w);

typedef struct cm_mapping_args {
    const char *index_path;
    const char *index_info_path;
    const char *gtf_path;
    const char *fastq1, *fastq2;
    const char *out_prefix;
    cm_params params;
    int32_t report;
    int32_t n_threads;
    uint64_t batch_pairs;
    int32_t rank, world;
} cm_mapping_args;
typedef struct cm_mapping_stats {
    uint64_t pairs, bsj_pairs;
    uint64_t by_type[14];
    int32_t rounds, reserved;
    double seconds_load, seconds_map;
    double seconds_parse, seconds_device, seconds_write;
} cm_mapping_stats;
int cm_mapping_run(const cm_mapping_args *args, cm_mapping_stats *stats, char *err, uint64_t err_cap);
int cm_merge_parts(const char *out_prefix, int32_t rounds, int32_t world, int32_t report);

int cm_sort_remain(const char *in_path, const char *out_path);
int cm_regional_table_build(const uint8_t *seq, uint32_t start, int32_t len, int32_t window_size, uint32_t **off, uint32_t **loc);
void cm_regional_table_free(uint32_t *off, uint32_t *loc);
typedef struct cm_circ_res {
    const char *chr, *rname;
    uint32_t spos, epos;
    int32_t type, reserved;
    const char *start_signal, *end_signal, *start_bp_ref, *end_bp_ref;
} cm_circ_res;
int cm_circ_report(const cm_circ_res *res, uint64_t n, const char *report_path);
typedef struct cm_circ_stats {
    uint64_t pairs, candidate_rows, calls;
    double seconds;
} cm_circ_stats;
int cm_circ_call(const cm_params *p, int32_t window_size, uint32_t n_contigs, const cm_index_view *contigs, const cm_annot_view *annots,
                 const cm_chr_info *chrs, uint32_t n_chr, const cm_fastq_batch *sorted, const char *candidates_path,
                 const char *report_path, cm_circ_stats *stats);
typedef struct cm_circ_args {
    const char *index_path, *index_info_path, *gtf_path, *out_prefix;
    cm_params params;
// ... 13 lines not shown
```

Baseline: 28.04 million.

## Precompute per-index-entry near-border bits and fold them into chain LDS loads

When a contig and its annotation load, a kernel now precomputes one bit per index entry saying whether that entry's position lies near an annotation border. The heavy chain kernel ORs this bit into bit 31 of each position as it stages it into LDS. The near-border test then reads and clears that bit instead of doing a random lookup into the near-border bitmap. The DP score/prev init loop also skips cells below n_pre. This trades an extra device buffer, load-time work and a download API for fewer scattered global reads in the hot loop, and assumes positions never use bit 31.

```diff
diff --git a/circminer_amd/_build.py b/circminer_amd/_build.py
--- a/circminer_amd/_build.py
+++ b/circminer_amd/_build.py
@@ -11,7 +11,7 @@
 SOURCES = ["cm_hot.hip", "cm_dispatch.cpp", "host_index.cpp", "host_annot.cpp", "host_index_io.cpp", "host_fastq.cpp", "host_mapping.cpp", "host_circ.cpp",
            "host_circ_call.cpp"]
 DEPS = SOURCES + sorted(f for f in os.listdir(CSRC) if f.endswith(".h")) + [os.path.join("..", "..", "include", "circminer_hot.h")]
-KERNEL_EXPORTS = ['cm_create', 'cm_destroy', 'cm_last_error', 'cm_load_contig', 'cm_load_contig_raw', 'cm_build_contig', 'cm_index_download', 'cm_load_annotation', 'cm_unload_contig', 'cm_reads_upload', 'cm_reads_stage', 'cm_reads_swap', 'cm_map_rounds', 'cm_map_round', 'cm_sync', 'cm_reads_reset', 'cm_collect_active', 'cm_collect_records', 'cm_collect_records_device', 'cm_host_alloc', 'cm_host_free', 'cm_host_register', 'cm_host_unregister', 'cm_type_histogram', 'cm_reads_download', 'cm_map_batch', 'cm_seed_batch', 'cm_chain_batch', 'cm_debug_lane_clk', 'cm_debug_counters', 'cm_prof_enable', 'cm_prof_reset', 'cm_prof_get', 'cm_prof_counters', 'cm_ctx', 'cm_chain']
+KERNEL_EXPORTS = ['cm_create', 'cm_destroy', 'cm_last_error', 'cm_load_contig', 'cm_load_contig_raw', 'cm_build_contig', 'cm_index_download', 'cm_near_entry_download', 'cm_load_annotation', 'cm_unload_contig', 'cm_reads_upload', 'cm_reads_stage', 'cm_reads_swap', 'cm_map_rounds', 'cm_map_round', 'cm_sync', 'cm_reads_reset', 'cm_collect_active', 'cm_collect_records', 'cm_collect_records_device', 'cm_host_alloc', 'cm_host_free', 'cm_host_register', 'cm_host_unregister', 'cm_type_histogram', 'cm_reads_download', 'cm_map_batch', 'cm_seed_batch', 'cm_chain_batch', 'cm_debug_lane_clk', 'cm_debug_counters', 'cm_prof_enable', 'cm_prof_reset', 'cm_prof_get', 'cm_prof_counters', 'cm_ctx', 'cm_chain']
 VARIANTS = (("k16", []), ("k24", ["-DCM_MAX_CHAIN_FRAGS=24"]))
 
 
diff --git a/circminer_amd/csrc/cm_dispatch.cpp b/circminer_amd/csrc/cm_dispatch.cpp
--- a/circminer_amd/csrc/cm_dispatch.cpp
+++ b/circminer_amd/csrc/cm_dispatch.cpp
@@ -29,6 +29,7 @@
 CM_VARIANTS(int, cm_load_contig_raw, (void *, int, const cm_index_raw *))
 CM_VARIANTS(int, cm_build_contig, (void *, int, int32_t, const uint8_t *, uint32_t, cm_build_stats *))
 CM_VARIANTS(int, cm_index_download, (void *, int, uint32_t *, uint16_t *, uint32_t *, uint64_t, uint64_t *))
+CM_VARIANTS(int, cm_near_entry_download, (void *, int, uint32_t *, uint64_t, uint64_t *))
 CM_VARIANTS(int, cm_host_register, (void *, void *, uint64_t))
 CM_VARIANTS(int, cm_host_unregister, (void *, void *))
 CM_VARIANTS(int, cm_type_histogram, (void *, uint64_t *))
@@ -92,6 +93,9 @@
 int cm_index_download(cm_ctx *ctx, int slot, uint32_t *bucket_off, uint16_t *checksum, uint32_t *pos, uint64_t cap, uint64_t *n) {
     return ctx ? GO(cm_index_download, slot, bucket_off, checksum, pos, cap, n) : CM_EINVAL;
 }
+int cm_near_entry_download(cm_ctx *ctx, int slot, uint32_t *bits, uint64_t cap_words, uint64_t *n) {
+    return ctx ? GO(cm_near_entry_download, slot, bits, cap_words, n) : CM_EINVAL;
+}
 int cm_host_register(cm_ctx *ctx, void *p, uint64_t bytes) { return ctx ? GO(cm_host_register, p, bytes) : CM_EINVAL; }
 int cm_host_unregister(cm_ctx *ctx, void *p) { return ctx ? GO(cm_host_unregister, p) : CM_EINVAL; }
 int cm_type_histogram(cm_ctx *ctx, uint64_t out[14]) { return ctx ? GO(cm_type_histogram, out) : CM_EINVAL; }
diff --git a/circminer_amd/csrc/cm_hot.hip b/circminer_amd/csrc/cm_hot.hip
--- a/circminer_amd/csrc/cm_hot.hip
+++ b/circminer_amd/csrc/cm_hot.hip
@@ -451,7 +451,7 @@
                                                     const unsigned long long *celloff, double *dp_score, int32_t *dp_prev, uint8_t *pool,
                                                     unsigned long long pool_bytes, unsigned long long *pool_cursor, cm_chain *chains, int32_t *nchain,
                                                     int *err, uint16_t *resid, const uint32_t *perm, const unsigned int *n_perm, unsigned int *next_problem,
-                                                    unsigned long long *counters) {
+                                                    unsigned long long *counters, const uint32_t *near_entry) {
     extern __shared__ uint32_t lds_words[];
     CM_L uint32_t *LP = (CM_L uint32_t *)lds_words;
     __shared__ HeavyBackTrack BT;
@@ -481,9 +481,17 @@
         const uint32_t ncell = base[kc];
         CM_G double *dps = (CM_G double *)(dp_score + celloff[r]);
         CM_G int32_t *dpp = (CM_G int32_t *)(dp_prev + celloff[r]);
-        for (int s = 0; s < kc; ++s)
-            for (uint32_t i = lane; i < cn[s]; i += 64) LP[base[s] + i] = c.X.pos[st[s] + i];
-        for (uint32_t x = lane; x < ncell; x += 64) {
+        for (int s = 0; s < kc; ++s) {
+            const bool with_bit = near_entry && s < kc - 1;
+            for (uint32_t i = lane; i < cn[s]; i += 64) {
+                const uint32_t e = st[s] + i;
+                uint32_t v = c.X.pos[e];
+                if (with_bit) v |= ((near_entry[e >> 5] >> (e & 31u)) & 1u) << 31;
+                LP[base[s] + i] = v;
+            }
+        }
+        const uint32_t n_pre = kc >= 1 ? base[kc - 1] : 0u;
+        for (uint32_t x = n_pre + lane; x < ncell; x += 64) {
             dps[x] = (double)kmer;
             dpp[x] = -1;
         }
@@ -492,7 +500,6 @@
         CM_L uint32_t *NB = LP + ncell;
         CM_L uint16_t *Q = (CM_L uint16_t *)(NB + 2 * ((ncell + 63) >> 6));
         {
-            const uint32_t n_pre = kc >= 1 ? base[kc - 1] : 0u;
             const unsigned long long lt = (1ull << lane) - 1ull;
             uint32_t qn = 0;
             auto look_up = [&](uint32_t cnt) {
@@ -513,7 +520,9 @@
 #pragma unroll
                 for (int u = 0; u < 4; ++u) {
                     const uint32_t x = x0 + 64 * u + lane;
-                    nr[u] = x < n_pre && cmc::bit_at(c.A.near_border_bits, c.A.n_bits, LP[x]);
+                    const uint32_t v = x < n_pre ? LP[x] : 0u;
+                    nr[u] = (v >> 31) != 0u;
+                    if (nr[u]) LP[x] = v & 0x7fffffffu;
                 }
 #pragma unroll
                 for (int u = 0; u < 4; ++u) {
@@ -1411,6 +1420,14 @@
     v.x = out[0]; v.y = out[1]; v.z = out[2]; v.w = out[3];
     ((uint4 *)desc)[hv] = v;
 }
+__global__ void __launch_bounds__(BLK) k_near_entry(const uint32_t *pos, uint64_t n_entries, const uint64_t *near_bits, uint64_t n_bits, uint32_t *out) {
+    const uint64_t e = (uint64_t)blockIdx.x * BLK + threadIdx.x;
+    const bool b = e < n_entries && cmc::bit_at((cmc::g_u64)near_bits, n_bits, pos[e]);
+    const unsigned long long m = __ballot(b);
+    const int lane = (int)(threadIdx.x & 63u);
+    if (lane == 0) out[e >> 5] = (uint32_t)m;
+    if (lane == 32) out[e >> 5] = (uint32_t)(m >> 32);
+}
 constexpr int S32_T = 1024, S32_E = 8, S32_B = S32_T * S32_E;
 __global__ void __launch_bounds__(S32_T) k_scan32_a(const uint32_t *in, uint64_t n, uint32_t *out, uint32_t *bsum, uint32_t add, int inclusive) {
     __shared__ uint32_t wsum[S32_T / 64];
@@ -1608,6 +1625,7 @@
     bool loaded = false, has_annot = false;
     uint64_t gen = 0;
     uint32_t *d_desc = nullptr;
+    uint32_t *d_near_entry = nullptr;
     bool chain_parallel_ok = false;
     cm_index_view X{};
     cmc::AnnotDev A{};
@@ -2013,7 +2031,7 @@
     return CM_OK;
 }
 
-int run_chain_tile(cm_ctx *ctx, const KCore &core, const ReadsDev &rd, uint64_t pair0, uint32_t n_tile, bool parallel_ok, const uint8_t *act,
+int run_chain_tile(cm_ctx *ctx, const KCore &core, const ReadsDev &rd, uint64_t pair0, uint32_t n_tile, const Slot &sl, const uint8_t *act,
                    const ChainRecs &rb, int s, const std::function<int()> &after_launch = {}) {
     const int S = ctx->n_seeds;
     const uint32_t n_prob = n_tile * 4u;
@@ -2049,7 +2067,7 @@
     const size_t lds_extra = ((size_t)max_cells / 64 + 2) * 8 + 640;
     const size_t heavy_lds = std::min<size_t>((size_t)S * (size_t)ctx->P.seed_lim * sizeof(uint32_t),
                                               ((size_t)max_cells * sizeof(uint32_t) + 2047) / 2048 * 2048 + 2048) + (lds_extra + 255) / 256 * 256;
-    const bool split = ranges.size() == 1 && parallel_ok && heavy_lds <= 152u * 1024u;
+    const bool split = ranges.size() == 1 && sl.chain_parallel_ok && heavy_lds <= 152u * 1024u;
     bool fresh = true;
     auto launch_group = [&](uint32_t a, uint32_t b, unsigned long long base, bool use_split) -> int {
         const uint32_t n = b - a;
@@ -2071,7 +2089,7 @@
             const uint32_t hb = n < 8192u ? n : 8192u;
             hipLaunchKernelGGL(k_chain_heavy, dim3(hb), dim3(64), heavy_lds, ctx->st.B2, core, rd, pair0, S, sb.sstart, sb.scnt, sb.celloff,
                                ctx->dp.score, ctx->dp.prev, ctx->dp.pool, ctx->dp.pool_bytes, ctx->pool_cursor(s), rb.chains, rb.nchain, ctx->d_err,
-                               rb.resid, sb.perm4, sb.cctr + CTR_BASE + CHAIN_LIGHT_CLS - 1, sb.cctr + 48, ctx->d_counters);
+                               rb.resid, sb.perm4, sb.cctr + CTR_BASE + CHAIN_LIGHT_CLS - 1, sb.cctr + 48, ctx->d_counters, (const uint32_t *)sl.d_near_entry);
             ++ctx->launches[6];
             }
             HIPCHK(ctx, hipEventRecord(ctx->ev.join, ctx->st.B2));
@@ -2245,6 +2263,28 @@
 
 const char *cm_last_error(const cm_ctx *ctx) { return ctx ? ctx->err.c_str() : "null context"; }
 
+static void drop_near_entry(cm_ctx *ctx, Slot &s) {
+    if (!s.d_near_entry) return;
+    auto it = std::find(s.ann_allocs.begin(), s.ann_allocs.end(), (void *)s.d_near_entry);
+    if (it != s.ann_allocs.end()) s.ann_allocs.erase(it);
+    report_hip(ctx, "hipFree", hipFree(s.d_near_entry));
+    s.d_near_entry = nullptr;
+}
+static int make_near_entry(cm_ctx *ctx, Slot &s) {
+    drop_near_entry(ctx, s);
+    if (!s.loaded || !s.has_annot) return CM_OK;
+    const uint64_t n = s.X.n_entries;
+    const uint64_t nblk = (n + BLK - 1) / BLK;
+    uint32_t *d = nullptr;
+    HIPCHK(ctx, hipMalloc((void **)&d, (size_t)(nblk ? nblk * (BLK / 32) : 1) * sizeof(uint32_t)));
+    s.ann_allocs.push_back(d);
+    s.d_near_entry = d;
+    if (nblk) hipLaunchKernelGGL(k_near_entry, dim3((unsigned)nblk), dim3(BLK), 0, ctx->st.B, s.X.pos, n, s.A.near_border_bits, s.A.n_bits, d);
+    HIPCHK(ctx, hipGetLastError());
+    HIPCHK(ctx, hipStreamSynchronize(ctx->st.B));
+    return CM_OK;
+}
+
 static int finish_contig(cm_ctx *ctx, Slot &s) {
     const size_t nb = ((size_t)1 << (2 * CM_WINDOW_SIZE)) + 1;
     s.d_desc = nullptr;
@@ -2262,7 +2302,7 @@
     }
     HIPCHK(ctx, hipStreamSynchronize(ctx->st.B));
     s.loaded = true;
-    return CM_OK;
+    return make_near_entry(ctx, s);
 }
 
 int cm_load_contig(cm_ctx *ctx, int slot, const cm_index_view *iv) {
@@ -2272,6 +2312,7 @@
     HIPCHK(ctx, hipSetDevice(ctx->P.device));
     Slot &s = ctx->slots[slot];
     free_all(ctx, s.idx_allocs);
+    drop_near_entry(ctx, s);
     s.d_desc = nullptr;
     s.loaded = false;
     ++s.gen;
@@ -2311,6 +2352,7 @@
     HIPCHK(ctx, hipSetDevice(ctx->P.device));
     Slot &s = ctx->slots[slot];
     free_all(ctx, s.idx_allocs);
+    drop_near_entry(ctx, s);
     s.d_desc = nullptr;
     s.loaded = false;
     ++s.gen;
@@ -2533,6 +2575,7 @@
     HIPCHK(ctx, hipSetDevice(ctx->P.device));
     Slot &s = ctx->slots[slot];
     free_all(ctx, s.idx_allocs);
+    drop_near_entry(ctx, s);
     s.d_desc = nullptr;
     s.loaded = false;
     ++s.gen;
@@ -2573,6 +2616,24 @@
     return CM_OK;
 }
 
+int cm_near_entry_download(cm_ctx *ctx, int slot, uint32_t *bits, uint64_t cap_words, uint64_t *n_entries) {
+    if (!ctx) return CM_EINVAL;
+    int rc;
+    if ((rc = check_slot(ctx, slot, false))) return rc;
+    const Slot &s = ctx->slots[slot];
+    const uint64_t n = s.X.n_entries, nw = (n + 31) / 32;
+    if (n_entries) *n_entries = n;
+    if (!bits) return CM_OK;
+    if (cap_words < nw) return fail(ctx, CM_ELIMIT, "slot %d holds %llu entries, the buffer %llu words", slot, (unsigned long long)n, (unsigned long long)cap_words);
+    HIPCHK(ctx, hipSetDevice(ctx->P.device));
+    if (!s.d_near_entry) memset(bits, 0, (size_t)nw * sizeof(uint32_t));
+    else if (nw) {
+        HIPCHK(ctx, hipMemcpyAsync(bits, s.d_near_entry, (size_t)nw * sizeof(uint32_t), hipMemcpyDeviceToHost, ctx->st.B));
+        HIPCHK(ctx, hipStreamSynchronize(ctx->st.B));
+    }
+    return CM_OK;
+}
+
 int cm_load_annotation(cm_ctx *ctx, int slot, const cm_annot_view *av) {
     if (!ctx || !av) return CM_EINVAL;
     if (slot < 0 || slot >= MAX_SLOTS) return fail(ctx, CM_EINVAL, "slot %d out of range", slot);
@@ -2580,6 +2641,7 @@
     HIPCHK(ctx, hipSetDevice(ctx->P.device));
     Slot &s = ctx->slots[slot];
     free_all(ctx, s.ann_allocs);
+    s.d_near_entry = nullptr;
     s.has_annot = false;
     ++s.gen;
     cmc::AnnotAosHost aos;
@@ -2618,7 +2680,7 @@
         s.chain_parallel_ok = ok;
     }
     s.has_annot = true;
-    return CM_OK;
+    return make_near_entry(ctx, s);
 }
 
 int cm_unload_contig(cm_ctx *ctx, int slot) {
@@ -2628,7 +2690,7 @@
     free_all(ctx, ctx->slots[slot].idx_allocs);
     free_all(ctx, ctx->slots[slot].ann_allocs);
     ctx->slots[slot].loaded = ctx->slots[slot].has_annot = false;
-    ctx->slots[slot].d_desc = nullptr;
+    ctx->slots[slot].d_desc = ctx->slots[slot].d_near_entry = nullptr;
     ++ctx->slots[slot].gen;
     return CM_OK;
 }
@@ -3208,7 +3270,7 @@
                 ctx->pair_pending[b] = false;
             }
             HIPCHK(ctx, hipEventRecord(ctx->ev.flags, ctx->st.B));
-            if ((rc = run_chain_tile(ctx, core, rd_cur, p0, nt, sl.chain_parallel_ok, act_prep, rb, i & 1, ahead))) return rc;
+            if ((rc = run_chain_tile(ctx, core, rd_cur, p0, nt, sl, act_prep, rb, i & 1, ahead))) return rc;
             HIPCHK(ctx, hipEventRecord(ctx->ev.prep[b], ctx->st.B));
         }
         const int is_last = (r == n_rounds - 1) ? (last_is_final != 0) : 0;
@@ -3237,7 +3299,7 @@
             HIPCHK(ctx, hipStreamWaitEvent(ctx->st.B, ctx->ev.seed[n_items & 1], 0));
             if ((rc = seed_classes(ctx, 0, nt, ctx->d_ones, n_items & 1, ctx->st.B, &rbn))) return rc;
         } else if ((rc = run_seed_tile(ctx, core, rd_next, 0, nt, ctx->d_ones, n_items & 1, ctx->st.B, &rbn))) return rc;
-        if ((rc = run_chain_tile(ctx, core, rd_next, 0, nt, sl.chain_parallel_ok, ctx->d_ones, rbn, n_items & 1))) return rc;
+        if ((rc = run_chain_tile(ctx, core, rd_next, 0, nt, sl, ctx->d_ones, rbn, n_items & 1))) return rc;
         HIPCHK(ctx, hipEventRecord(ctx->ev.prep[b], ctx->st.B));
         ctx->pre_launched = true;
         ctx->pre_slot = slots[0];
@@ -3492,7 +3554,7 @@
         HIPCHK(ctx, hipMemsetAsync(ctx->rec[0].chains, 0, (size_t)nt * 4 * CM_BESTCHAINLIM * sizeof(cm_chain), ctx->st.B));
         const ChainRecs &rb0 = ctx->rec[0];
         if ((rc = run_seed_tile(ctx, core, current_reads(ctx), p0, nt, ctx->d_active, 0, ctx->st.B, &rb0))) return rc;
-        if ((rc = run_chain_tile(ctx, core, current_reads(ctx), p0, nt, ctx->slots[slot].chain_parallel_ok, ctx->d_active, rb0, 0))) return rc;
+        if ((rc = run_chain_tile(ctx, core, current_reads(ctx), p0, nt, ctx->slots[slot], ctx->d_active, rb0, 0))) return rc;
         const size_t np = (size_t)nt * 4, o = (size_t)p0 * 4;
         HIPCHK(ctx, hipMemcpyAsync(out_chains + o * CM_BESTCHAINLIM, ctx->rec[0].chains, np * CM_BESTCHAINLIM * sizeof(cm_chain), hipMemcpyDeviceToHost,
                                    ctx->st.B));
diff --git a/circminer_amd/lib.py b/circminer_amd/lib.py
--- a/circminer_amd/lib.py
+++ b/circminer_amd/lib.py
@@ -178,6 +178,7 @@
         "cm_host_next_contig_raw": (C.c_int, [vp, C.c_int, pp(IndexRaw), pp(C.c_int)]),
         "cm_build_contig": (C.c_int, [vp, C.c_int, C.c_int32, u8p, C.c_uint32, pp(BuildStats)]),
         "cm_index_download": (C.c_int, [vp, C.c_int, vp, vp, vp, C.c_uint64, pp(C.c_uint64)]),
+        "cm_near_entry_download": (C.c_int, [vp, C.c_int, vp, C.c_uint64, pp(C.c_uint64)]),
         "cm_unload_contig": (C.c_int, [vp, C.c_int]),
         "cm_reads_upload": (C.c_int, [vp, pp(Reads), vp]),
         "cm_reads_stage": (C.c_int, [vp, pp(Reads), vp]),
@@ -265,7 +266,7 @@
                     "cm_host_write_index", "cm_host_open_index", "cm_host_next_contig", "cm_host_next_contig_genome", "cm_host_free_loaded_contig",
                     "cm_host_close_index", "cm_fastq_open", "cm_fastq_open_shard", "cm_merge_parts", "cm_fastq_next", "cm_fastq_set_release_hook", "cm_fastq_close", "cm_writer_open", "cm_write_remain",
                     "cm_write_pam", "cm_write_sam_header", "cm_write_sam", "cm_writer_flush", "cm_writer_close", "cm_mapping_run", "cm_sort_remain", "cm_circ_report", "cm_circ_call", "cm_circ_run", "cm_host_gene_overlap", "cm_regional_table_build", "cm_regional_table_free",
-                    "cm_build_contig", "cm_index_download"]
+                    "cm_build_contig", "cm_index_download", "cm_near_entry_download"]
 
 
 class HostIndex:
@@ -621,6 +622,13 @@
                                            n.value, C.byref(n)), "cm_index_download")
         return off, cks, pos
 
+    def near_entry_bits(self, slot):
+        n = C.c_uint64(0)
+        self._chk(self.L.cm_near_entry_download(self.h, slot, None, 0, C.byref(n)), "cm_near_entry_download")
+        w = np.zeros((n.value + 31) // 32, np.uint32)
+        self._chk(self.L.cm_near_entry_download(self.h, slot, w.ctypes.data if w.size else None, w.size, C.byref(n)), "cm_near_entry_download")
+        return np.unpackbits(w.view(np.uint8), bitorder="little")[:n.value].astype(bool)
+
     def upload(self, batch: ReadBatch, prior: np.ndarray = None):
         self.n = batch.n
         p = prior.ctypes.data if prior is not None else None
diff --git a/include/circminer_hot.h b/include/circminer_hot.h
--- a/include/circminer_hot.h
+++ b/include/circminer_hot.h
@@ -135,6 +135,7 @@
                     cm_build_stats *stats );
 int cm_index_download(cm_ctx *ctx, int slot, uint32_t *bucket_off, uint16_t *checksum, uint32_t *pos,
                       uint64_t cap_entries, uint64_t *n_entries);
+int cm_near_entry_download(cm_ctx *ctx, int slot, uint32_t *bits, uint64_t cap_words, uint64_t *n_entries);
 int cm_unload_contig(cm_ctx *ctx, int slot);
 
 int cm_reads_upload(cm_ctx *ctx, const cm_reads *reads, const cm_mapped_read *prior);
```

Measured after the change: 28.17 million, median of 6. Within noise of the previous version (+0.5%).
